# xiph/daala

Hardware: NVIDIA H100
Metric: encoder Mpixels/s on 4K YUV420 intra (higher is better)
Workload: dtype int32

## Files before the change

daala_b200/csrc/frame_transform.cu:

```cuda
#include <cuda.h>
#include <cuda_runtime.h>
#include <cudaTypedefs.h>
#include <stdint.h>
#include <stdio.h>
#include <string.h>

#include "gen/dct_lifting.cuh"
#include "lapped_filter.cuh"
#include "frame_transform.h"
#include "haar.cuh"

namespace daala_b200 {

#ifndef DAALA_XFORM_THREADS
#define DAALA_XFORM_THREADS 64
#endif
constexpr int kThreads = DAALA_XFORM_THREADS;
constexpr int kPostThreads = 128;
constexpr int kCtasPerSm = 512 / kThreads;
constexpr int kGridCap = 132 * 8;
constexpr int kMaxB = 64;
constexpr int kHalo = 2;
constexpr int kMaxT = kMaxB + 2 * kHalo;
constexpr int kMaxPitch = kMaxT + 1;

struct TmaMaps {
  CUtensorMap plane[3];
};

template <int XDEC> struct RawTile {
  static constexpr int B = kMaxB >> XDEC;
  static constexpr int rows = B + 2 * kHalo;
  static constexpr int lead = 16;
  static constexpr int width = ((lead + B + kHalo + 15) / 16) * 16;
  static constexpr int skip = lead - kHalo;
  static constexpr int bytes = rows * width;
};

__device__ __forceinline__ uint32_t smem_u32(const void* p) { return (uint32_t)__cvta_generic_to_shared(p); }

__device__ __forceinline__ void mbar_init(uint64_t* bar, int count) {
  asm volatile("mbarrier.init.shared::cta.b64 [%0], %1;" ::"r"(smem_u32(bar)), "r"(count));
  asm volatile("fence.mbarrier_init.release.cluster;" ::: "memory");
}

__device__ __forceinline__ void mbar_expect_tx(uint64_t* bar, uint32_t bytes) {
  asm volatile("mbarrier.arrive.expect_tx.shared::cta.b64 _, [%0], %1;" ::"r"(smem_u32(bar)), "r"(bytes) : "memory");
}

__device__ __forceinline__ void mbar_wait(uint64_t* bar, uint32_t phase) {
  uint32_t ok = 0;
  while (!ok) {
    asm volatile(
        "{ .reg .pred p; mbarrier.try_wait.parity.shared::cta.b64 p, [%1], %2; selp.u32 %0, 1, 0, p; }"
        : "=r"(ok) : "r"(smem_u32(bar)), "r"(phase) : "memory");
  }
}

__device__ __forceinline__ void tma_load_3d(void* dst, const CUtensorMap* map, int x, int y, int z, uint64_t* bar) {
  asm volatile(
      "cp.async.bulk.tensor.3d.shared::cluster.global.mbarrier::complete_tx::bytes [%0], [%1, {%2, %3, %4}], [%5];"
      ::"r"(smem_u32(dst)), "l"(map), "r"(x), "r"(y), "r"(z), "r"(smem_u32(bar)) : "memory");
}

template <int B_, int P_>
struct SbCtxT {
  static constexpr int B = B_;
  static constexpr int P = P_;
  static constexpr int ushift = (B_ == 64) ? 3 : 2;
  static constexpr int logB = (B_ == 64) ? 6 : 5;
  int x0, y0;
};

struct SbLists {
  unsigned short blk[256 + 64 + 16 + 4 + 1];
  unsigned short node[64 + 16 + 4 + 1];
  int nblk[5];
  int nnode[4];
  unsigned char wcnt[8][9];
};
__device__ __forceinline__ constexpr int blk_base(int c) { return c == 0 ? 0 : c == 1 ? 256 : c == 2 ? 320 : c == 3 ? 336 : 340; }
__device__ __forceinline__ constexpr int node_base(int l) { return (int)((0x54504000u >> (8 * l)) & 0xffu); }
constexpr unsigned short kGateH = 0x4000;
constexpr unsigned short kGateV = 0x8000;

template <int XDEC>
__device__ __forceinline__ void build_lists(SbLists& L, const unsigned char* bsize, int bstride, int sbx,
                                            int sby, int x0, int y0, int pic_w, int pic_h) {
  static_assert(kThreads >= 64, "one thread per 8x8-luma unit");
  constexpr int B = kMaxB >> XDEC;
  constexpr int USZ = 8 >> XDEC;
  const int t = threadIdx.x, lane = t & 31, w = t >> 5;
  const int bx = t & 7, by = (t >> 3) & 7;
  unsigned flags = 0;
  unsigned rank[9];
  if (t < 64) {
    const int obs = bsize[(sby * 8 + by) * bstride + sbx * 8 + bx];
    const int c = (obs > XDEC ? obs : XDEC) - XDEC;
    const unsigned lt = (1u << lane) - 1u;
    const int xy = bx | by;
#pragma unroll
    for (int cat = 0; cat < 9; cat++) {
      bool f;
      if (cat < 5) {
        const int a = XDEC ? (1 << cat) : (cat ? (1 << (cat - 1)) : 1);
        f = c == cat && !(xy & (a - 1));
      } else {
        const int l = cat - 5, S = 8 << l;
        const int a = XDEC ? (2 << l) : (1 << l);
        f = S <= B && !(xy & (a - 1)) && c < 1 + l;
      }
      const unsigned b = __ballot_sync(0xffffffffu, f);
      flags |= (unsigned)f << cat;
      rank[cat] = __popc(b & lt);
      if (lane == 0) L.wcnt[w][cat] = (unsigned char)__popc(b);
    }
  }
  __syncthreads();
  if (t < 64) {
    const unsigned short pos = (unsigned short)(((by * USZ) << 8) | (bx * USZ));
#pragma unroll
    for (int cat = 0; cat < 9; cat++) {
      const int n0 = L.wcnt[0][cat], n1 = L.wcnt[1][cat];
      const int at = (w ? n0 : 0) + (int)rank[cat];
      constexpr bool kQuad = XDEC == 0;
      if (t == 0) {
        if (cat < 5) L.nblk[cat] = (cat == 0 && kQuad) ? 4 * (n0 + n1) : n0 + n1;
        else L.nnode[cat - 5] = n0 + n1;
      }
      if (flags & (1u << cat)) {
        if (cat == 0 && kQuad) {
          L.blk[4 * at + 0] = pos;
          L.blk[4 * at + 1] = (unsigned short)(pos + 4);
          L.blk[4 * at + 2] = (unsigned short)(pos + (4 << 8));
          L.blk[4 * at + 3] = (unsigned short)(pos + (4 << 8) + 4);
        } else if (cat < 5) {
          L.blk[blk_base(cat) + at] = pos;
        } else {
          const int S = 8 << (cat - 5);
          unsigned short v = pos;
          if (x0 + bx * USZ + S <= pic_w) v |= kGateH;
          if (y0 + by * USZ + S <= pic_h) v |= kGateV;
          L.node[node_base(cat - 5) + at] = v;
        }
      }
    }
  }
  __syncthreads();
}

template <int C, bool kFwd, int P>
__device__ __forceinline__ void transform_pass(int* tile, const SbLists& L, bool along_columns) {
  constexpr int LN = C + 2;
  constexpr int N = 1 << LN;
  const int items = L.nblk[C] << LN;
  for (int item = threadIdx.x; item < items; item += kThreads) {
    const int pos = L.blk[blk_base(C) + (item >> LN)];
    const int k = item & (N - 1);
    const int px = (pos & 255) + (along_columns ? k : 0);
// ... 83 lines not shown
  int* sp = tile + row0 * P + col;
  int32_t* gp = g + (size_t)row0 * gstride + col;
#pragma unroll 8
  for (int r = row0; r < B; r += kRowsPerIter) {
    if (kToGlobal) {
      *reinterpret_cast<int4*>(gp) = make_int4(sp[0], sp[1], sp[2], sp[3]);
    } else {
      const int4 v = *reinterpret_cast<const int4*>(gp);
      sp[0] = v.x;
      sp[1] = v.y;
      sp[2] = v.z;
      sp[3] = v.w;
    }
    sp += kRowsPerIter * P;
    gp += (size_t)kRowsPerIter * gstride;
  }
}
__device__ __forceinline__ bool rows_aligned16(const void* p, long long stride_elems) {
  return ((reinterpret_cast<uintptr_t>(p) | (uintptr_t)(stride_elems * 4)) & 15u) == 0;
}

struct FrameMasks {
  const uint8_t* haar;
  const uint8_t* skip;
};

template <int XDEC, bool kTma>
__device__ __forceinline__ void forward_sb_body(const FrameXformParams& prm, const PlaneXform& pl,
                                                int* tile_s, SbLists& lists, const CUtensorMap* map,
                                                unsigned char* raw, uint64_t* bar, const FrameMasks& fm) {
  constexpr int B = kMaxB >> XDEC;
  constexpr int T = B + 2 * kHalo;
  constexpr int P = kMaxPitch;
  using Sb = SbCtxT<B, P>;
  const int sbx = blockIdx.x % prm.nhsb, sby = prm.sb_row0 + blockIdx.x / prm.nhsb;
  const int fr = blockIdx.z;
  if (fm.skip && fm.skip[fr]) return;
  const bool haar_dc = fm.haar ? fm.haar[fr] != 0 : prm.haar_dc != 0;
  Sb s;
  s.x0 = sbx * B;
  s.y0 = sby * B;
  const int pw = prm.nhsb * B, ph = prm.nvsb * B;
  if (kTma) {
    constexpr int RW = RawTile<XDEC>::width;
    if (threadIdx.x == 0) {
      mbar_init(bar, 1);
      mbar_expect_tx(bar, RawTile<XDEC>::bytes);
      tma_load_3d(raw, map, s.x0 - RawTile<XDEC>::lead, s.y0 - kHalo, fr, bar);
    }
    build_lists<XDEC>(lists, prm.bsize + fr * prm.bsize_frame_pitch, prm.bstride, sbx, sby, s.x0, s.y0,
                      prm.pic_w, prm.pic_h);
    mbar_wait(bar, 0);
    constexpr int kSkip = RawTile<XDEC>::skip;
    constexpr int kW0 = kSkip / 4;
    constexpr int kWords = (kSkip + T + 3) / 4 - kW0;
    for (int i = threadIdx.x; i < T * kWords; i += kThreads) {
      const int r = i / kWords, m = i - r * kWords;
      const unsigned w = *reinterpret_cast<const unsigned*>(raw + r * RW + 4 * (kW0 + m));
      const int c0 = 4 * (kW0 + m) - kSkip;
      int* t = tile_s + r * P + c0;
#pragma unroll
      for (int j = 0; j < 4; j++) {
        const int c = c0 + j;
        if (c >= 0 && c < T) t[j] = ((int)((w >> (8 * j)) & 255u) - 128) * 16;
      }
    }
  } else {
    build_lists<XDEC>(lists, prm.bsize + fr * prm.bsize_frame_pitch, prm.bstride, sbx, sby, s.x0, s.y0,
                      prm.pic_w, prm.pic_h);
    const uint8_t* src = pl.pixels + fr * pl.pixel_frame_pitch;
    for (int i = threadIdx.x; i < T * T; i += kThreads) {
      int r = i / T, c = i - r * T;
      int gx = s.x0 + c - kHalo, gy = s.y0 + r - kHalo;
      int v = 0;
      if (gx >= 0 && gx < pw && gy >= 0 && gy < ph) v = ((int)src[(size_t)gy * pl.pixel_stride + gx] - 128) * 16;
      tile_s[r * P + c] = v;
    }
  }
  __syncthreads();
  {
    const bool top = sby > 0, bottom = sby + 1 < prm.nvsb;
    for (int i = threadIdx.x; i < 2 * T; i += kThreads) {
      int e = i >= T, c = i - e * T;
      if (e == 0 ? top : bottom) lap4_inplace<false>(tile_s + (e ? B : 0) * P + c, P);
    }
    __syncthreads();
    const bool left = sbx > 0, right = sbx + 1 < prm.nhsb;
    for (int i = threadIdx.x; i < 2 * B; i += kThreads) {
      int r = i % B + kHalo, e = i / B;
      if (e == 0 ? left : right) lap4_inplace<false>(tile_s + r * P + (e ? B : 0), 1);
    }
    __syncthreads();
  }
  int* tile = tile_s + kHalo * P + kHalo;
#pragma unroll 1
  for (int l = Sb::logB - 3; l >= 0; l--) {
    if (lists.nnode[l] == 0) continue;
    split_filter_level<false, P>(tile, lists, l, true);
    __syncthreads();
    split_filter_level<false, P>(tile, lists, l, false);
    __syncthreads();
  }
#ifdef DAALA_DEBUG_LISTS
  if (threadIdx.x == 0 && XDEC == 1 && sbx == 1 && sby == 1 && blockIdx.y == 1) {
    printf("chroma lists: nblk %d %d %d %d %d nnode %d %d %d %d\n", lists.nblk[0], lists.nblk[1], lists.nblk[2],
           lists.nblk[3], lists.nblk[4], lists.nnode[0], lists.nnode[1], lists.nnode[2], lists.nnode[3]);
    for (int c = 0; c < 4; c++) for (int i = 0; i < lists.nblk[c]; i++) printf("blk c%d (%d,%d)\n", c, lists.blk[blk_base(c) + i] & 255, lists.blk[blk_base(c) + i] >> 8);
    for (int l = 0; l < 3; l++) for (int i = 0; i < lists.nnode[l]; i++) printf("node l%d (%d,%d) gates %x\n", l, lists.node[node_base(l) + i] & 255, (lists.node[node_base(l) + i] >> 8) & 63, lists.node[node_base(l) + i] >> 14);
  }
#endif
  transform_all_leaves<true, P>(tile, lists);
  if (haar_dc) {
#pragma unroll 1
    for (int l = 0; l <= Sb::logB - 3; l++) {
      if (lists.nnode[l] == 0) continue;
      haar_dc_level<false, P>(tile, lists, l);
      __syncthreads();
    }
  }
  int32_t* dst = pl.coeffs + fr * pl.coeff_frame_pitch + (size_t)s.y0 * pl.coeff_stride + s.x0;
  if (rows_aligned16(dst, pl.coeff_stride)) {
    tile_copy4<B, P, true>(tile, dst, pl.coeff_stride);
    return;
  }
  for (int i = threadIdx.x; i < B * B; i += kThreads) {
    int r = i / B, c = i % B;
    dst[(size_t)r * pl.coeff_stride + c] = tile[r * P + c];
  }
}

__global__ void __launch_bounds__(kThreads, kCtasPerSm)
k_forward_sb(const __grid_constant__ FrameXformParams prm, const __grid_constant__ FrameMasks fm) {
  __shared__ int tile_s[kMaxT * kMaxPitch];
  __shared__ SbLists lists;
  const PlaneXform& pl = prm.plane[blockIdx.y];
  if (pl.xdec == 0) forward_sb_body<0, false>(prm, pl, tile_s, lists, nullptr, nullptr, nullptr, fm);
  else forward_sb_body<1, false>(prm, pl, tile_s, lists, nullptr, nullptr, nullptr, fm);
}

__global__ void __launch_bounds__(kThreads, kCtasPerSm)
k_forward_sb_tma(const __grid_constant__ FrameXformParams prm, const __grid_constant__ CUtensorMap map0,
                 const __grid_constant__ CUtensorMap map1, const __grid_constant__ CUtensorMap map2,
                 const __grid_constant__ FrameMasks fm) {
  __shared__ int tile_s[kMaxT * kMaxPitch];
  __shared__ __align__(128) unsigned char raw[RawTile<0>::bytes];
  __shared__ __align__(8) uint64_t bar;
  __shared__ SbLists lists;
  const PlaneXform& pl = prm.plane[blockIdx.y];
  const CUtensorMap* map = blockIdx.y == 0 ? &map0 : (blockIdx.y == 1 ? &map1 : &map2);
  if (pl.xdec == 0) forward_sb_body<0, true>(prm, pl, tile_s, lists, map, raw, &bar, fm);
  else forward_sb_body<1, true>(prm, pl, tile_s, lists, map, raw, &bar, fm);
}

template <int XDEC>
__device__ __forceinline__ void inverse_sb_body(const FrameXformParams& prm, const PlaneXform& pl,
                                                int* tile, SbLists& lists) {
  constexpr int B = kMaxB >> XDEC;
  constexpr int P = kMaxPitch;
  using Sb = SbCtxT<B, P>;
  const int sbx = blockIdx.x % prm.nhsb, sby = prm.sb_row0 + blockIdx.x / prm.nhsb;
  const int fr = blockIdx.z;
  Sb s;
  s.x0 = sbx * B;
  s.y0 = sby * B;
  const int32_t* srcp = pl.coeffs + fr * pl.coeff_frame_pitch + (size_t)s.y0 * pl.coeff_stride + s.x0;
  if (rows_aligned16(srcp, pl.coeff_stride)) {
    tile_copy4<B, P, false>(tile, const_cast<int32_t*>(srcp), pl.coeff_stride);
  } else {
    for (int i = threadIdx.x; i < B * B; i += kThreads) {
      int r = i / B, c = i % B;
      tile[r * P + c] = srcp[(size_t)r * pl.coeff_stride + c];
    }
  }
  build_lists<XDEC>(lists, prm.bsize + fr * prm.bsize_frame_pitch, prm.bstride, sbx, sby, s.x0, s.y0,
                    prm.pic_w, prm.pic_h);
  if (prm.haar_dc) {
#pragma unroll 1
    for (int l = Sb::logB - 3; l >= 0; l--) {
      if (lists.nnode[l] == 0) continue;
      haar_dc_level<true, P>(tile, lists, l);
      __syncthreads();
    }
  }
  transform_all_leaves<false, P>(tile, lists);
#pragma unroll 1
  for (int l = 0; l <= Sb::logB - 3; l++) {
    if (lists.nnode[l] == 0) continue;
    split_filter_level<true, P>(tile, lists, l, false);
    __syncthreads();
    split_filter_level<true, P>(tile, lists, l, true);
    __syncthreads();
  }
  int32_t* dst = pl.lapped + fr * pl.lapped_frame_pitch + (size_t)s.y0 * pl.lapped_stride + s.x0;
  if (rows_aligned16(dst, pl.lapped_stride)) {
    tile_copy4<B, P, true>(tile, dst, pl.lapped_stride);
    return;
  }
  for (int i = threadIdx.x; i < B * B; i += kThreads) {
    int r = i / B, c = i % B;
    dst[(size_t)r * pl.lapped_stride + c] = tile[r * P + c];
  }
}

__global__ void __launch_bounds__(kThreads, kCtasPerSm)
k_inverse_sb(const __grid_constant__ FrameXformParams prm) {
  __shared__ int tile_s[kMaxB * kMaxPitch];
  __shared__ SbLists lists;
  const PlaneXform& pl = prm.plane[blockIdx.y];
  if (pl.xdec == 0) inverse_sb_body<0>(prm, pl, tile_s, lists);
  else inverse_sb_body<1>(prm, pl, tile_s, lists);
}

template <int XDEC>
__device__ __forceinline__ void sb_postfilter_store_body(const FrameXformParams& prm,
                                                         const PlaneXform& pl, int* tile_s) {
  constexpr int B = kMaxB >> XDEC;
  constexpr int T = B + 2 * kHalo;
  constexpr int P = T + 1;
  const int sbx = blockIdx.x % prm.nhsb, sby = prm.sb_row0 + blockIdx.x / prm.nhsb;
  const int fr = blockIdx.z;
  const int32_t* lap = pl.lapped + fr * pl.lapped_frame_pitch;
  const int x0 = sbx * B, y0 = sby * B;
  const int pw = prm.nhsb * B, ph = prm.nvsb * B;
  const int32_t* core = lap + (size_t)y0 * pl.lapped_stride + x0;
  if (rows_aligned16(core, pl.lapped_stride)) {
    tile_copy4<B, P, false, kPostThreads>(tile_s + kHalo * P + kHalo, const_cast<int32_t*>(core), pl.lapped_stride);
    for (int i = threadIdx.x; i < 4 * T + 4 * B; i += kPostThreads) {
      int r, c;
      if (i < 4 * T) {
        const int k = i / T;
        r = k < 2 ? k : B + k;
        c = i - k * T;
      } else {
        const int j = i - 4 * T, k = j / B;
        c = k < 2 ? k : B + k;
        r = j - k * B + kHalo;
      }
      const int gx = x0 + c - kHalo, gy = y0 + r - kHalo;
      int v = 0;
      if (gx >= 0 && gx < pw && gy >= 0 && gy < ph) v = lap[(size_t)gy * pl.lapped_stride + gx];
      tile_s[r * P + c] = v;
    }
  } else {
    for (int i = threadIdx.x; i < T * T; i += kPostThreads) {
      int r = i / T, c = i - r * T;
      int gx = x0 + c - kHalo, gy = y0 + r - kHalo;
      int v = 0;
      if (gx >= 0 && gx < pw && gy >= 0 && gy < ph) v = lap[(size_t)gy * pl.lapped_stride + gx];
      tile_s[r * P + c] = v;
    }
  }
  __syncthreads();
  const bool left = sbx > 0, right = sbx + 1 < prm.nhsb;
  for (int i = threadIdx.x; i < 2 * T; i += kPostThreads) {
    int e = i >= T, r = i - e * T;
    if (e == 0 ? left : right) lap4_inplace<true>(tile_s + r * P + (e ? B : 0), 1);
  }
  __syncthreads();
  const bool top = sby > 0, bottom = sby + 1 < prm.nvsb;
  for (int i = threadIdx.x; i < 2 * B; i += kPostThreads) {
    int c = i % B + kHalo, e = i / B;
    if (e == 0 ? top : bottom) lap4_inplace<true>(tile_s + (e ? B : 0) * P + c, P);
  }
  __syncthreads();
  if (prm.post16[blockIdx.y]) {
    int16_t* d16 = prm.post16[blockIdx.y] + fr * pl.pixel_out_frame_pitch + (size_t)y0 * pl.pixel_out_stride + x0;
    for (int i = threadIdx.x; i < B * B / 2; i += kPostThreads) {
      int r = i / (B / 2), c2 = (i % (B / 2)) * 2;
      const int* p = tile_s + (r + kHalo) * P + c2 + kHalo;
      const unsigned w = ((unsigned)p[0] & 0xffffu) | ((unsigned)p[1] << 16);
      *reinterpret_cast<unsigned*>(d16 + (size_t)r * pl.pixel_out_stride + c2) = w;
    }
    return;
  }
  uint8_t* dst = pl.pixels_out + fr * pl.pixel_out_frame_pitch + (size_t)y0 * pl.pixel_out_stride + x0;
  for (int i = threadIdx.x; i < B * B / 4; i += kPostThreads) {
    int r = i / (B / 4), c4 = (i % (B / 4)) * 4;
    const int* p = tile_s + (r + kHalo) * P + c4 + kHalo;
    unsigned w = 0;
#pragma unroll
    for (int k = 0; k < 4; k++) {
      int v = ((p[k] + 8) >> 4) + 128;
      v = v < 0 ? 0 : (v > 255 ? 255 : v);
      w |= (unsigned)v << (8 * k);
    }
    *reinterpret_cast<unsigned*>(dst + (size_t)r * pl.pixel_out_stride + c4) = w;
  }
}

__global__ void __launch_bounds__(kPostThreads)
k_sb_postfilter_store(const __grid_constant__ FrameXformParams prm) {
  __shared__ int tile_s[kMaxT * kMaxPitch];
  const PlaneXform& pl = prm.plane[blockIdx.y];
  if (pl.xdec == 0) sb_postfilter_store_body<0>(prm, pl, tile_s);
  else sb_postfilter_store_body<1>(prm, pl, tile_s);
}

template <bool kPost>
__global__ void k_plane_sb_edges(int32_t* c, int stride, int nhsb, int nvsb, int sbw, int sbh,
                                 bool vertical_taps) {
  const int w = nhsb * sbw, h = nvsb * sbh;
  const int along = vertical_taps ? w : h;
  const int edges = (vertical_taps ? nvsb : nhsb) - 1;
  const long total = (long)along * edges;
  for (long i = blockIdx.x * (long)blockDim.x + threadIdx.x; i < total;
       i += (long)gridDim.x * blockDim.x) {
    int a = (int)(i % along), e = (int)(i / along) + 1;
    if (vertical_taps) lap4_inplace<kPost>(c + (size_t)(e * sbh - 2) * stride + a, stride);
    else lap4_inplace<kPost>(c + (size_t)a * stride + e * sbw - 2, 1);
  }
}

template <int L>
__global__ void __launch_bounds__(64)
k_block_transform(int32_t* blocks, int mode) {
  constexpr int N = 1 << L;
  constexpr int P = N + 5;
  __shared__ int t[N * P];
  int32_t* blk = blocks + (size_t)blockIdx.x * N * N;
  for (int i = threadIdx.x; i < N * N; i += blockDim.x) t[(i / N) * P + (i % N)] = blk[i];
  __syncthreads();
  const bool fwd = (mode & 1) == 0;
  const int passes = mode < 2 ? 2 : 1;
  for (int pass = 0; pass < passes; pass++) {
    bool cols = mode < 2 ? (fwd ? pass == 0 : pass == 1) : false;
    if (threadIdx.x < N) {
      int* p = cols ? t + threadIdx.x : t + threadIdx.x * P;
      int stride = cols ? P : 1;
      int v[N];
#pragma unroll
      for (int k = 0; k < N; k++) v[k] = p[k * stride];
      if (fwd) Lifting<N>::fwd(v); else Lifting<N>::inv(v);
#pragma unroll
      for (int k = 0; k < N; k++) p[k * stride] = v[k];
    }
    __syncthreads();
  }
  for (int i = threadIdx.x; i < N * N; i += blockDim.x) blk[i] = t[(i / N) * P + (i % N)];
}

__global__ void k_filter4_batch(int32_t* v, long count, int post) {
  for (long i = blockIdx.x * (long)blockDim.x + threadIdx.x; i < count;
       i += (long)gridDim.x * blockDim.x) {
    if (post) lap4_inplace<true>(v + 4 * i, 1); else lap4_inplace<false>(v + 4 * i, 1);
  }
}

template <int N>
__global__ void k_lapfilter_batch(int32_t* v, long count, int post) {
  for (long i = blockIdx.x * (long)blockDim.x + threadIdx.x; i < count; i += (long)gridDim.x * blockDim.x) {
    int t[N];
#pragma unroll
    for (int k = 0; k < N; k++) t[k] = v[i * N + k];
    if (post) LapFilter<N>::post(t); else LapFilter<N>::pre(t);
#pragma unroll
    for (int k = 0; k < N; k++) v[i * N + k] = t[k];
  }
}

__global__ void k_split_filter_batch(int32_t* blocks, int n, int post, int hfilter, int vfilter) {
  int32_t* b = blocks + (size_t)blockIdx.x * n * n;
  for (int phase = 0; phase < 2; phase++) {
    bool vertical_taps = post ? phase == 1 : phase == 0;
    if (vertical_taps ? hfilter : vfilter) {
      for (int i = threadIdx.x; i < n; i += blockDim.x) {
        if (vertical_taps) {
          if (post) lap4_inplace<true>(b + (n / 2 - 2) * n + i, n); else lap4_inplace<false>(b + (n / 2 - 2) * n + i, n);
        } else {
          if (post) lap4_inplace<true>(b + i * n + n / 2 - 2, 1); else lap4_inplace<false>(b + i * n + n / 2 - 2, 1);
        }
      }
    }
    __syncthreads();
  }
}

}

using namespace daala_b200;

template <bool kInverse>
__global__ void __launch_bounds__(256) k_haar_blocks(int32_t* __restrict__ blocks, int ln) {
  __shared__ int t[64 * 64];
  const int n = 1 << ln;
  int32_t* g = blocks + (size_t)blockIdx.x * n * n;
  if (!kInverse) {
    for (int i = threadIdx.x; i < n * n; i += 256) t[i] = g[i];
    __syncthreads();
    haar_forward_levels<256>(t, g, n, ln);
  } else {
    haar_inverse_levels<256>(t, g, n, ln);
    for (int i = threadIdx.x; i < n * n; i += 256) g[i] = t[i];
  }
}

extern "C" {

static bool encode_input_maps(const FrameXformParams* prm, int nplanes, TmaMaps* maps) {
  static PFN_cuTensorMapEncodeTiled_v12000 encode = nullptr;
  static bool tried = false;
  if (!tried) {
    tried = true;
    void* fn = nullptr;
    cudaDriverEntryPointQueryResult q;
    if (cudaGetDriverEntryPoint("cuTensorMapEncodeTiled", &fn, cudaEnableDefault, &q) == cudaSuccess &&
        q == cudaDriverEntryPointSuccess)
      encode = (PFN_cuTensorMapEncodeTiled_v12000)fn;
  }
  if (!encode) return false;
  memset(maps, 0, sizeof(*maps));
  for (int p = 0; p < nplanes; p++) {
    const PlaneXform& pl = prm->plane[p];
    const int B = kMaxB >> pl.xdec;
    const cuuint64_t w = (cuuint64_t)prm->nhsb * B, h = (cuuint64_t)prm->nvsb * B;
    const cuuint64_t fpitch = prm->nframes > 1 ? (cuuint64_t)pl.pixel_frame_pitch : w * h;
    if (((uintptr_t)pl.pixels & 15) || (pl.pixel_stride & 15) || (fpitch & 15) || pl.pixel_stride <= 0) return false;
    cuuint64_t dims[3] = {w, h, (cuuint64_t)prm->nframes};
    cuuint64_t strides[2] = {(cuuint64_t)pl.pixel_stride, fpitch};
    cuuint32_t box[3] = {(cuuint32_t)(pl.xdec ? RawTile<1>::width : RawTile<0>::width),
                         (cuuint32_t)(B + 2 * kHalo), 1};
    cuuint32_t estr[3] = {1, 1, 1};
    CUresult r = encode(&maps->plane[p], CU_TENSOR_MAP_DATA_TYPE_UINT8, 3, (void*)pl.pixels, dims, strides, box,
                        estr, CU_TENSOR_MAP_INTERLEAVE_NONE, CU_TENSOR_MAP_SWIZZLE_NONE,
                        CU_TENSOR_MAP_L2_PROMOTION_L2_128B, CU_TENSOR_MAP_FLOAT_OOB_FILL_NONE);
    if (r != CUDA_SUCCESS) return false;
  }
  return true;
}

int daala_b200_launch_forward_masked(const FrameXformParams* prm, int nplanes, const uint8_t* haar_frames,
                                     const uint8_t* skip_frames, cudaStream_t stream) {
  dim3 grid(prm->nhsb * prm->sb_rows, nplanes, prm->nframes);
  const FrameMasks fm = {haar_frames, skip_frames};
  TmaMaps maps;
  if (encode_input_maps(prm, nplanes, &maps))
    k_forward_sb_tma<<<grid, kThreads, 0, stream>>>(*prm, maps.plane[0], maps.plane[1], maps.plane[2], fm);
  else k_forward_sb<<<grid, kThreads, 0, stream>>>(*prm, fm);
  return (int)cudaGetLastError();
}

int daala_b200_launch_forward(const FrameXformParams* prm, int nplanes, cudaStream_t stream) {
  return daala_b200_launch_forward_masked(prm, nplanes, nullptr, nullptr, stream);
}

int daala_b200_launch_forward_no_tma(const FrameXformParams* prm, int nplanes, cudaStream_t stream) {
  dim3 grid(prm->nhsb * prm->sb_rows, nplanes, prm->nframes);
  k_forward_sb<<<grid, kThreads, 0, stream>>>(*prm, FrameMasks{nullptr, nullptr});
  return (int)cudaGetLastError();
}

int daala_b200_launch_inverse(const FrameXformParams* prm, int nplanes, cudaStream_t stream) {
  dim3 grid(prm->nhsb * prm->sb_rows, nplanes, prm->nframes);
  k_inverse_sb<<<grid, kThreads, 0, stream>>>(*prm);
  k_sb_postfilter_store<<<grid, kPostThreads, 0, stream>>>(*prm);
  return (int)cudaGetLastError();
}

static FrameXformParams plane_range(const FrameXformParams* prm, int plane0) {
  FrameXformParams q = *prm;
  for (int p = 0; p + plane0 < 3; p++) {
    q.plane[p] = prm->plane[plane0 + p];
    q.post16[p] = prm->post16[plane0 + p];
  }
  return q;
}

int daala_b200_launch_inverse_lapped_only(const FrameXformParams* prm, int plane0, int nplanes, cudaStream_t stream) {
  if (plane0 < 0 || nplanes < 1 || plane0 + nplanes > 3) return (int)cudaErrorInvalidValue;
  dim3 grid(prm->nhsb * prm->sb_rows, nplanes, prm->nframes);
  k_inverse_sb<<<grid, kThreads, 0, stream>>>(plane_range(prm, plane0));
  return (int)cudaGetLastError();
}

int daala_b200_launch_sb_postfilter_store(const FrameXformParams* prm, int plane0, int nplanes, cudaStream_t stream) {
  if (plane0 < 0 || nplanes < 1 || plane0 + nplanes > 3) return (int)cudaErrorInvalidValue;
  dim3 grid(prm->nhsb * prm->sb_rows, nplanes, prm->nframes);
  k_sb_postfilter_store<<<grid, kPostThreads, 0, stream>>>(plane_range(prm, plane0));
  return (int)cudaGetLastError();
}

int daala_b200_launch_plane_sb_filter(int32_t* c, int stride, int nhsb, int nvsb, int xdec, int ydec,
                                      int post, cudaStream_t stream) {
  const int sbw = 64 >> xdec, sbh = 64 >> ydec;
  for (int phase = 0; phase < 2; phase++) {
    bool vertical_taps = post ? phase == 1 : phase == 0;
    long total = vertical_taps ? (long)nhsb * sbw * (nvsb - 1) : (long)nvsb * sbh * (nhsb - 1);
    if (total <= 0) continue;
    int blocks = (int)((total + 255) / 256);
    if (blocks > kGridCap) blocks = kGridCap;
    if (post) k_plane_sb_edges<true><<<blocks, 256, 0, stream>>>(c, stride, nhsb, nvsb, sbw, sbh, vertical_taps);
    else k_plane_sb_edges<false><<<blocks, 256, 0, stream>>>(c, stride, nhsb, nvsb, sbw, sbh, vertical_taps);
  }
  return (int)cudaGetLastError();
}

int daala_b200_launch_block_transform(int32_t* blocks, int count, int ln, int mode, cudaStream_t stream) {
  if (count <= 0) return 0;
  switch (ln) {
    case 2: k_block_transform<2><<<count, 64, 0, stream>>>(blocks, mode); break;
    case 3: k_block_transform<3><<<count, 64, 0, stream>>>(blocks, mode); break;
    case 4: k_block_transform<4><<<count, 64, 0, stream>>>(blocks, mode); break;
    case 5: k_block_transform<5><<<count, 64, 0, stream>>>(blocks, mode); break;
    case 6: k_block_transform<6><<<count, 64, 0, stream>>>(blocks, mode); break;
    default: return (int)cudaErrorInvalidValue;
  }
  return (int)cudaGetLastError();
}

int daala_b200_launch_haar_blocks(int32_t* blocks, int count, int ln, int inverse, cudaStream_t stream) {
  if (count <= 0) return 0;
  if (ln < 1 || ln > 6) return (int)cudaErrorInvalidValue;
  if (inverse) k_haar_blocks<true><<<count, 256, 0, stream>>>(blocks, ln);
  else k_haar_blocks<false><<<count, 256, 0, stream>>>(blocks, ln);
  return (int)cudaGetLastError();
}

int daala_b200_launch_filter4(int32_t* v, long count, int post, cudaStream_t stream) {
  if (count <= 0) return 0;
  int blocks = (int)((count + 255) / 256);
  if (blocks > kGridCap) blocks = kGridCap;
  k_filter4_batch<<<blocks, 256, 0, stream>>>(v, count, post);
  return (int)cudaGetLastError();
}

int daala_b200_launch_lapfilter(int32_t* v, long count, int n, int post, cudaStream_t stream) {
  if (count <= 0) return 0;
  int blocks = (int)((count + 127) / 128);
  if (blocks > kGridCap) blocks = kGridCap;
  if (n == 4) k_filter4_batch<<<blocks, 128, 0, stream>>>(v, count, post);
  else if (n == 8) k_lapfilter_batch<8><<<blocks, 128, 0, stream>>>(v, count, post);
  else if (n == 16) k_lapfilter_batch<16><<<blocks, 128, 0, stream>>>(v, count, post);
  else if (n == 32) k_lapfilter_batch<32><<<blocks, 128, 0, stream>>>(v, count, post);
  else return (int)cudaErrorInvalidValue;
  return (int)cudaGetLastError();
}

int daala_b200_launch_split_filter(int32_t* blocks, int count, int n, int post, int hfilter, int vfilter,
                                   cudaStream_t stream) {
  if (count <= 0) return 0;
  k_split_filter_batch<<<count, 64, 0, stream>>>(blocks, n, post, hfilter, vfilter);
  return (int)cudaGetLastError();
}

}
```

daala_b200/csrc/frame_transform.h:

```cpp
#pragma once
#include "daala_b200.h"

typedef daala_b200_plane PlaneXform;
typedef daala_b200_frame FrameXformParams;
```

daala_b200/csrc/kf_engine.cu:

```cuda
#include <cuda_runtime.h>
#include <math.h>
#include <stdint.h>
#include <stdio.h>
#include <stdlib.h>
#include <string.h>

#include <algorithm>
#include <cmath>
#include <new>
#include <vector>

#include "daala_b200.h"
#include "dering_search.h"
#include "late_skip.h"
#include "lossless.h"
#include "haar_dc.h"
#include "mc_batch.h"
#include "gen/coding_order.inc"
#include "pvq_math.cuh"
#include "pvq_warp.cuh"
#include "pvq_common.cuh"

namespace daala_b200 {
namespace kf {

using namespace daala_b200::pvq;

enum Cnt {
  kNLuma = 0, kNChroma, kLumaCoefs, kChromaCoefs,
  kNItemsL = 4,
  kNItemsC = 7,
  kTotalHi = 14,
  kNHeads = 15,
  kNHeads0 = 16,
  kError = 17,
  kDepsDone = 18,
  kMcBadRef = 19,
  kMcBeyond = 20,
  kHeadLoL = 32,
  kHeadHi = 96,
  kTailHi = 128,
  kDoneHi = 160,
  kHeadCh = 192,
  kWaiters = 224,
  kTraceN = 240,
  kCntWords = 256
};

constexpr int kTile = 1024;
constexpr int kHeadBins = 12288;

struct Lists {
  const uint8_t* bsize;
  int bstride;
  long long bsize_pitch;
  int F, UW, UH;
  int u_row0, u_rows;
  int ntiles;
  int4* tile_sum;
  int32_t* unit_lbase;
  int32_t* unit_loff;
  daala_b200_pvq_block* luma;
  daala_b200_pvq_block* chroma;
  int32_t* dep_top;
  int32_t* dep_left;
  int32_t* succ_bottom;
  int32_t* succ_right;
  uint32_t* items_l[3];
  uint32_t* items_c[3];
  uint32_t* heads;
  uint32_t* heads0;
  uint32_t* heads_raw;
  int32_t* head_bin;
  int32_t* head_hist;
  int32_t* head_cursor;
  int32_t* cnt;
  int max_luma, max_chroma;
  const uint8_t* ftype;
  int32_t* kcnt;
  uint32_t* kitems_l[3];
};

__device__ __forceinline__ int4 add4(int4 a, int4 b) { return make_int4(a.x + b.x, a.y + b.y, a.z + b.z, a.w + b.w); }

__device__ __forceinline__ int4 unit_counts(int b, int ux, int uy) {
  if (b == 0) return make_int4(4, 64, 1, 16);
  const int span = 1 << (b - 1);
  if ((ux & (span - 1)) | (uy & (span - 1))) return make_int4(0, 0, 0, 0);
  const int lc = b == 1 ? 64 : b == 2 ? 256 : 512;
  const int cc = b == 1 ? 16 : b == 2 ? 64 : b == 3 ? 256 : 512;
  return make_int4(1, lc, 1, cc);
}

__device__ __forceinline__ bool unit_of(const Lists& L, long long i, int* f, int* uy, int* ux, int* b) {
  const long long per = (long long)L.u_rows * L.UW;
  if (i >= per * L.F) return false;
  *f = (int)(i / per);
  const int r = (int)(i - (long long)*f * per);
  *uy = L.u_row0 + r / L.UW;
  *ux = r % L.UW;
  *b = L.bsize[*f * L.bsize_pitch + (long long)*uy * L.bstride + *ux];
  return true;
}

__global__ void __launch_bounds__(kTile) k_unit_tile_sums(const __grid_constant__ Lists L) {
  __shared__ int4 part[32];
  const long long i = (long long)blockIdx.x * kTile + threadIdx.x;
  int f, uy, ux, b;
  int4 v = make_int4(0, 0, 0, 0);
  if (unit_of(L, i, &f, &uy, &ux, &b)) v = unit_counts(b, ux, uy);
#pragma unroll
  for (int o = 16; o > 0; o >>= 1) {
    v.x += __shfl_xor_sync(0xffffffffu, v.x, o);
    v.y += __shfl_xor_sync(0xffffffffu, v.y, o);
    v.z += __shfl_xor_sync(0xffffffffu, v.z, o);
    v.w += __shfl_xor_sync(0xffffffffu, v.w, o);
  }
  if ((threadIdx.x & 31) == 0) part[threadIdx.x >> 5] = v;
  __syncthreads();
  if (threadIdx.x == 0) {
    int4 s = make_int4(0, 0, 0, 0);
    for (int w = 0; w < kTile / 32; w++) s = add4(s, part[w]);
    L.tile_sum[blockIdx.x] = s;
  }
}

__global__ void __launch_bounds__(1024) k_tile_scan(const __grid_constant__ Lists L) {
  __shared__ int4 part[1024];
  __shared__ int4 carry;
  const int t = threadIdx.x;
  if (t == 0) carry = make_int4(0, 0, 0, 0);
  __syncthreads();
  for (int base = 0; base < L.ntiles; base += 1024) {
    const int i = base + t;
    const int4 v = i < L.ntiles ? L.tile_sum[i] : make_int4(0, 0, 0, 0);
    part[t] = v;
    __syncthreads();
    for (int o = 1; o < 1024; o <<= 1) {
      const int4 a = t >= o ? part[t - o] : make_int4(0, 0, 0, 0);
      __syncthreads();
      part[t] = add4(part[t], a);
      __syncthreads();
    }
    const int4 incl = part[t], c = carry;
    if (i < L.ntiles) L.tile_sum[i] = make_int4(c.x + incl.x - v.x, c.y + incl.y - v.y, c.z + incl.z - v.z, c.w + incl.w - v.w);
    __syncthreads();
    if (t == 1023) carry = add4(c, incl);
    __syncthreads();
  }
  if (t == 0) {
    const int4 tot = carry;
    L.cnt[kNLuma] = tot.x;
    L.cnt[kLumaCoefs] = tot.y;
    L.cnt[kNChroma] = 2 * tot.z;
    L.cnt[kChromaCoefs] = 2 * tot.w;
    for (int c = 0; c < 3; c++) {
      L.cnt[kNItemsL + c] = 0;
      L.cnt[kNItemsC + c] = 0;
    }
    L.cnt[kTotalHi] = 0;
    L.cnt[kNHeads] = 0;
    L.cnt[kNHeads0] = 0;
    L.cnt[kDepsDone] = 0;
    if (L.kcnt != L.cnt) {
      L.kcnt[kNLuma] = 0;
      for (int c = 0; c < 3; c++) L.kcnt[kNItemsL + c] = 0;
      L.kcnt[kTotalHi] = 0;
      L.kcnt[kNHeads] = 0;
      L.kcnt[kNHeads0] = 0;
      L.kcnt[kDepsDone] = 0;
    }
    L.cnt[kError] = tot.x > L.max_luma || 2 * tot.z > L.max_chroma ? 1 : 0;
  }
}

__device__ __forceinline__ void put_block(daala_b200_pvq_block* dst, int coef_off, int x0, int y0, int bs, int pli,
                                          int xdec, int frame) {
  int32_t* w = reinterpret_cast<int32_t*>(dst);
  w[0] = coef_off;
  w[1] = (x0 & 0xffff) | (y0 << 16);
  w[2] = bs | (pli << 8) | (xdec << 16) | (frame << 24);
}

__global__ void __launch_bounds__(kTile) k_unit_emit(const __grid_constant__ Lists L) {
  __shared__ int4 wsum[32];
  const long long i = (long long)blockIdx.x * kTile + threadIdx.x;
  const int lane = threadIdx.x & 31, warp = threadIdx.x >> 5;
  int f = 0, uy = 0, ux = 0, b = 0;
  const bool valid = unit_of(L, i, &f, &uy, &ux, &b);
  const int4 v = valid ? unit_counts(b, ux, uy) : make_int4(0, 0, 0, 0);
  int4 s = v;
#pragma unroll
  for (int o = 1; o < 32; o <<= 1) {
    int4 a;
    a.x = __shfl_up_sync(0xffffffffu, s.x, o);
    a.y = __shfl_up_sync(0xffffffffu, s.y, o);
    a.z = __shfl_up_sync(0xffffffffu, s.z, o);
    a.w = __shfl_up_sync(0xffffffffu, s.w, o);
    if (lane >= o) s = add4(s, a);
  }
  if (lane == 31) wsum[warp] = s;
  __syncthreads();
  int4 pre = L.tile_sum[blockIdx.x];
  for (int w = 0; w < warp; w++) pre = add4(pre, wsum[w]);
  pre = make_int4(pre.x + s.x - v.x, pre.y + s.y - v.y, pre.z + s.z - v.z, pre.w + s.w - v.w);
  if (!valid) return;
  L.unit_lbase[((long long)f * L.UH + uy) * L.UW + ux] = pre.x;
  if (v.x == 0) return;
  if (pre.x + v.x > L.max_luma || 2 * (pre.z + v.z) > L.max_chroma) return;
  if (L.unit_loff) L.unit_loff[((long long)f * L.UH + uy) * L.UW + ux] = pre.y;
  if (b == 0) {
    for (int q = 0; q < 4; q++)
      put_block(L.luma + pre.x + q, pre.y + 16 * q, ux * 8 + (q & 1) * 4, uy * 8 + (q >> 1) * 4, 0, 0, 0, f);
  } else {
    put_block(L.luma + pre.x, pre.y, ux * 8, uy * 8, b, 0, 0, f);
  }
  const int cbs = (b > 1 ? b : 1) - 1;
  const int xd = 1 | (b == 0 ? 0x80 : 0);
  put_block(L.chroma + 2 * pre.z, 2 * pre.w, ux * 4, uy * 4, cbs, 1, xd, f);
  put_block(L.chroma + 2 * pre.z + 1, 2 * pre.w + v.w, ux * 4, uy * 4, cbs, 2, xd, f);
}

__device__ __forceinline__ int band_class(int band) { return band < 3 ? 0 : band < 6 ? 1 : 2; }

__device__ __forceinline__ int append(uint32_t* list, int32_t* counter, bool pred, uint32_t v) {
  const unsigned m = __ballot_sync(__activemask(), pred);
  if (!pred) return -1;
  const int lane = threadIdx.x & 31, leader = __ffs(m) - 1;
  int base = 0;
  if (lane == leader) base = atomicAdd(counter, __popc(m));
  base = __shfl_sync(m, base, leader);
  const int pos = base + __popc(m & ((1u << lane) - 1u));
  list[pos] = v;
  return pos;
}

__device__ __forceinline__ int count_key(int32_t* ctr, int key) {
  const unsigned same = __match_any_sync(__activemask(), key);
  const int lane = threadIdx.x & 31, leader = __ffs(same) - 1;
  int base = 0;
  if (lane == leader) base = atomicAdd(&ctr[key], __popc(same));
  return __shfl_sync(same, base, leader) + __popc(same & ((1u << lane) - 1u));
}

constexpr int kChainCost0 = 7, kChainCost1 = 9, kChainCost2 = 18;
__device__ __forceinline__ int weight_bin(int len, int band) {
  const int c = band_class(band);
  const int w = len * (c == 0 ? kChainCost0 : c == 1 ? kChainCost1 : kChainCost2);
  return kHeadBins - 1 - min(w, kHeadBins - 1);
}

__device__ int chain_length(const Lists& L, const uint8_t* map, int x0, int y0, int bs, bool down) {
  const int nn = 4 << bs, y_end = (L.u_row0 + L.u_rows) * 8, x_end = L.UW * 8;
  int len = 1;
  for (int x = x0 + (down ? 0 : nn), y = y0 + (down ? nn : 0); x < x_end && y < y_end;
       x += down ? 0 : nn, y += down ? nn : 0, len++) {
    if (map[(long long)(y >> 3) * L.bstride + (x >> 3)] != bs) break;
    const int py = down ? y - 1 : y, px = down ? x : x - 1;
    if (map[(long long)(py >> 3) * L.bstride + (px >> 3)] != bs) break;
  }
  return len;
}

template <int kThreads>
__device__ __forceinline__ void scan_bins(int32_t* hist, int32_t* cursor) {
  __shared__ int part[kThreads];
  constexpr int kPer = kHeadBins / kThreads;
  const int t = threadIdx.x;
  int v[kPer], sum = 0;
#pragma unroll
  for (int i = 0; i < kPer; i++) {
    v[i] = __ldcg(hist + t * kPer + i);
    sum += v[i];
  }
  part[t] = sum;
  __syncthreads();
  for (int o = 1; o < kThreads; o <<= 1) {
    const int add = t >= o ? part[t - o] : 0;
    __syncthreads();
    part[t] += add;
    __syncthreads();
  }
  int run = part[t] - sum;
#pragma unroll
  for (int i = 0; i < kPer; i++) {
    hist[t * kPer + i] = run;
    cursor[t * kPer + i] = run;
    run += v[i];
  }
}

__global__ void __launch_bounds__(256) k_luma_deps(const __grid_constant__ Lists L) {
  const int n = min(L.cnt[kNLuma], L.max_luma);
  const int nth = gridDim.x * blockDim.x;
  for (int base = blockIdx.x * blockDim.x; base < n; base += nth) {
    const int blk = base + threadIdx.x;
    const bool in = blk < n && (!L.ftype || L.ftype[L.luma[blk].frame]);
    if (L.ftype) {
      const int nk = __popc(__ballot_sync(0xffffffffu, in));
      if ((threadIdx.x & 31) == 0 && nk) atomicAdd(&L.kcnt[kNLuma], nk);
    }
    int bs = 0, top = -1, left = -1;
    if (in) {
      const daala_b200_pvq_block b = L.luma[blk];
      const int x0 = b.x0, y0 = b.y0, f = b.frame;
      bs = b.bs;
      const int nn = 4 << bs;
      const uint8_t* map = L.bsize + f * L.bsize_pitch;
      if (y0 - nn >= L.u_row0 * 8 && map[(long long)((y0 - 1) >> 3) * L.bstride + (x0 >> 3)] == bs) {
        const int ty = y0 - nn;
        top = L.unit_lbase[((long long)f * L.UH + (ty >> 3)) * L.UW + (x0 >> 3)] +
              (bs == 0 ? ((ty >> 2) & 1) * 2 + ((x0 >> 2) & 1) : 0);
      }
      if (x0 > 0 && map[(long long)(y0 >> 3) * L.bstride + ((x0 - 1) >> 3)] == bs) {
        const int lx = x0 - nn;
        left = L.unit_lbase[((long long)f * L.UH + (y0 >> 3)) * L.UW + (lx >> 3)] +
               (bs == 0 ? ((y0 >> 2) & 1) * 2 + ((lx >> 2) & 1) : 0);
      }
      L.dep_top[blk] = top;
      L.dep_left[blk] = left;
      if (top >= 0) L.succ_bottom[top] = blk;
      if (left >= 0) L.succ_right[left] = blk;
    }
    const int nb = in ? num_bands(bs) : 0;
    int len_down = 0, len_across = 0;
    if (nb > 1) {
      const daala_b200_pvq_block b = L.luma[blk];
      const uint8_t* map = L.bsize + b.frame * L.bsize_pitch;
      if (top < 0) len_down = chain_length(L, map, b.x0, b.y0, bs, true);
      if (left < 0) len_across = chain_length(L, map, b.x0, b.y0, bs, false);
    }
    int chain = 0;
    for (int band = 0; band < 9; band++) {
      const bool has = band < nb;
      const bool is_free = band == 3 || band == 6;
      const int r = band % 3;
      const bool waits = band == 0 ? (top >= 0 || left >= 0) : r == 1 ? top >= 0 : left >= 0;
      const uint32_t item = ((uint32_t)blk << 4) | band;
      if (band == 3 || band == 6) {
        append(L.kitems_l[band_class(band)], &L.kcnt[kNItemsL + band_class(band)], has, item);
      } else if (band == 0) {
        append(L.heads0, &L.kcnt[kNHeads0], has && !waits, item);
      } else {
        const int pos = append(L.heads_raw, &L.kcnt[kNHeads], has && !waits, item);
        if (pos >= 0) {
          const int bin = weight_bin(r == 1 ? len_down : len_across, band);
          L.head_bin[pos] = bin;
          count_key(L.head_hist, bin);
        }
      }
      chain += has && !is_free;
    }
#pragma unroll
    for (int o = 16; o > 0; o >>= 1) chain += __shfl_xor_sync(0xffffffffu, chain, o);
    if ((threadIdx.x & 31) == 0 && chain) atomicAdd(&L.kcnt[kTotalHi], chain);
  }
  __shared__ bool last;
  __threadfence();
  __syncthreads();
  if (threadIdx.x == 0) last = atomicAdd(&L.kcnt[kDepsDone], 1) == (int)gridDim.x - 1;
  __syncthreads();
  if (last) {
    __threadfence();
// ... 157 lines not shown
    } else if (kind == kGatherInter) {
      const int32_t* psrc = prm.pred_plane[b.pli] + b.frame * prm.plane_frame_pitch[b.pli] + (size_t)b.y0 * stride + b.x0;
      int32_t* vref = prm.ref + b.coef_off;
      for (int i = lane; i < len; i += 32) {
        const int at = i == 0 ? 0 : scan_to_raster(i, ln, stride);
        vin[i] = src[at];
        vref[i] = psrc[at];
      }
      if (kMixed && kKind == kGatherChroma && lane == 0) prm.res_flip[blk] = 0;
    } else {
      const int lo = S.cfl_loff[b.frame * (prm.plane_frame_pitch[b.pli] >> 4) + (long long)(b.y0 >> 2) * (stride >> 2) +
                                (b.x0 >> 2)];
      int32_t* vref = prm.ref + b.coef_off;
      const int qoff = prm.qm_stride + ((((1 << (2 * b.bs)) - 1) << 4) / 3);
      int32_t xy = 0;
      for (int i = lane; i < len; i += 32) {
        const int32_t vi = i == 0 ? src[0] : src[scan_to_raster(i, ln, stride)];
        const int32_t vr = cfl_ref<kHdc>(S, b, lo, i);
        vin[i] = vi;
        vref[i] = vr;
        if (i >= 1 && i < 16) {
          const int32_t rq = vr * prm.qm[qoff + i], inq = vi * prm.qm[qoff + i];
          xy += (int32_t)((rq * (int64_t)inq) >> ((kQmShift + 4) << 1));
        }
      }
#pragma unroll
      for (int o = 16; o > 0; o >>= 1) xy += __shfl_xor_sync(0xffffffffu, xy, o);
      const int flip = xy < 0;
      __syncwarp();
      if (flip) {
        const int end = band_start(num_bands(b.bs));
        for (int i = 1 + lane; i < end; i += 32) vref[i] = -vref[i];
      }
      if (lane == 0) prm.res_flip[blk] = flip;
    }
  }
}

constexpr int kPersistThreads = 32;
constexpr int kPersistCtas = 32;
static_assert(kPersistCtas * (kPersistThreads / 32 * kSnapEntries * (int)sizeof(int16_t) + 1024) <= 228 * 1024,
              "k_pvq_persist's shared scratch does not fit kPersistCtas CTAs per SM");
constexpr uint32_t kNoItem = 0xffffffffu;
constexpr uint32_t kExit = 0xfffffffeu;

__device__ __forceinline__ int ld_relaxed(const int32_t* p) {
  int v;
  asm volatile("ld.relaxed.gpu.global.s32 %0, [%1];" : "=r"(v) : "l"(p) : "memory");
  return v;
}

__device__ __forceinline__ void push_chain(const Stage& S, int blk, int band) {
  const int pos = atomicAdd(&S.cnt[kTailHi], 1) - S.cnt[kNHeads0];
  st_release((int*)&S.ring[pos], (int)(((uint32_t)blk << 4) | band));
}

__device__ __forceinline__ uint32_t next_item(const Stage& S, int lane, int* done, bool* waiter) {
  int slot = -1, head = -1, lo = -1, nheads0 = 0, fin = -1;
  if (lane == 0) {
    const int n2 = S.cnt[S.n_items_at + 2], n1 = S.cnt[S.n_items_at + 1], n0 = S.cnt[S.n_items_at];
    const int nlo = n0 + n1 + n2;
    nheads0 = S.cnt[kNHeads0];
    if (*done) {
      const int d = atomicAdd(&S.cnt[kDoneHi], *done) + *done;
      if (d == S.cnt[kNLuma]) {
        __threadfence();
        fin = ld_relaxed(&S.cnt[kTailHi]) - nheads0;
      }
    }
    if (ld_relaxed(&S.cnt[kHeadHi]) < ld_relaxed(&S.cnt[kTailHi])) slot = atomicAdd(&S.cnt[kHeadHi], 1);
    if (slot < 0 && ld_relaxed(&S.cnt[kHeadCh]) < S.cnt[kNHeads]) {
      const int h = atomicAdd(&S.cnt[kHeadCh], 1);
      if (h < S.cnt[kNHeads]) head = h;
    }
    if (slot < 0 && head < 0 && ld_relaxed(&S.cnt[S.head_lo_at]) < nlo) {
      const int l = atomicAdd(&S.cnt[S.head_lo_at], 1);
      if (l < nlo) lo = l;
    }
    if (slot < 0 && head < 0 && lo < 0) {
      if (!*waiter && atomicAdd(&S.cnt[kWaiters], 1) < S.max_waiters) *waiter = true;
      if (*waiter) slot = atomicAdd(&S.cnt[kHeadHi], 1);
    }
  }
  *done = 0;
  fin = __shfl_sync(0xffffffffu, fin, 0);
  if (fin >= 0) {
    const int nw = (gridDim.x * blockDim.x) >> 5;
#pragma unroll 1
    for (int i = lane; i <= nw; i += 32) st_release((int*)&S.ring[fin + i], (int)kExit);
  }
  head = __shfl_sync(0xffffffffu, head, 0);
  if (head >= 0) return S.heads[head];
  slot = __shfl_sync(0xffffffffu, slot, 0);
  lo = __shfl_sync(0xffffffffu, lo, 0);
  if (slot >= 0) {
    nheads0 = __shfl_sync(0xffffffffu, nheads0, 0);
    if (slot < nheads0) return S.heads0[slot];
    uint32_t v;
    while ((v = (uint32_t)ld_acquire((const int*)&S.ring[slot - nheads0])) == kNoItem) __nanosleep(500);
    return v == kExit ? kNoItem : v;
  }
  if (lo >= 0) {
    const int n2 = S.cnt[S.n_items_at + 2], n1 = S.cnt[S.n_items_at + 1];
    return lo < n2 ? S.items[2][lo] : lo < n2 + n1 ? S.items[1][lo - n2] : S.items[0][lo - n2 - n1];
  }
  return kNoItem;
}

__device__ __forceinline__ void intra_band_ref(const Stage& S, int blk, int band, int coef_off, int lane) {
  const daala_b200_pvq_params& prm = S.prm;
  const int start = band_start(band);
  const int bn = band_start(band + 1) - start;
  const int r = band % 3;
  int top = -1, left = -1;
  if (band == 0 || r == 1) top = S.dep_top[blk];
  if (band == 0 || r == 2) left = S.dep_left[blk];
  if (band == 3 || band == 6) top = left = -1;
  const int32_t* ot = top >= 0 ? prm.out + prm.blocks[top].coef_off : nullptr;
  const int32_t* ol = left >= 0 ? prm.out + prm.blocks[left].coef_off : nullptr;
  bool low_from_top = false;
  if (band == 0) {
    double g1 = 0, g2 = 0;
    if (ot) { double a = __ldcg(ot + 2), bb = __ldcg(ot + 5), c = __ldcg(ot + 9); g1 += a * a; g1 += bb * bb; g1 += c * c; }
    if (ol) { double a = __ldcg(ol + 1), bb = __ldcg(ol + 4), c = __ldcg(ol + 7); g2 += a * a; g2 += bb * bb; g2 += c * c; }
    low_from_top = g1 > g2;
  }
  int32_t* vref = prm.ref + coef_off;
  for (int i = start + lane; i < start + bn; i += 32) {
    int r2, c2;
    scan_rc(i, &r2, &c2);
    int32_t p = 0;
    if (r2 == 0 && c2 > 0 && ot && (c2 >= 4 || low_from_top)) p = __ldcg(ot + i);
    if (c2 == 0 && r2 > 0 && ol && (r2 >= 4 || !low_from_top)) p = __ldcg(ol + i);
    vref[i] = p;
  }
}

__device__ __forceinline__ void run_item(const Stage& S, uint32_t item, int lane, int16_t* snap) {
  const daala_b200_pvq_params& prm = S.prm;
  const int blk = (int)(item >> 4), band = (int)(item & 15);
  const daala_b200_pvq_block b = prm.blocks[blk];
  const int bs = b.bs, pli = b.pli;
  const int start = band_start(band);
  const int bn = band_start(band + 1) - start;
  const size_t off = (size_t)b.coef_off + start;
  intra_band_ref(S, blk, band, b.coef_off, lane);
  const int qidx = bs * (bs + 1) + (band + 1) - (band + 1) / 3;
  const int q = S.fq_bq[(b.frame * 3 + pli) * 32 + qidx];
  const int beta = (prm.use_masking && pli == 0 && bs > 0) ? kBeta15 : kBeta1;
  const int qoff = (b.xdec & 1 ? prm.qm_stride : 0) + ((((1 << (2 * bs)) - 1) << 4) / 3) + start;
  int itheta, max_theta, k;
  double skip_term;
  const int gain = quantise_band_warp<0>(lane, snap, S.rsqrt_tbl, prm.out + off, prm.in + off, prm.ref + off, bn, q,
                                         prm.y + off, &itheta, &max_theta, &k, beta, &skip_term, prm.is_keyframe, pli,
                                         prm.qm + qoff, prm.qm_inv + qoff, prm.pvq_norm_lambda);
  if (lane == 0) {
    const size_t r = (size_t)blk * 9 + band;
    prm.res_skip_term[r] = skip_term;
    short4 pk;
    pk.x = (short)gain; pk.y = (short)itheta; pk.z = (short)max_theta; pk.w = (short)k;
    reinterpret_cast<short4*>(S.res_pack)[r] = pk;
  }
}

struct ItemGeom {
  int blk, band, bn, q, beta, pli, qoff, is_keyframe;
  size_t off;
};
__device__ __forceinline__ ItemGeom item_geom(const Stage& S, uint32_t item) {
  const daala_b200_pvq_params& prm = S.prm;
  ItemGeom g;
  g.blk = (int)(item >> 4);
  g.band = (int)(item & 15);
  const daala_b200_pvq_block b = prm.blocks[g.blk];
  const int bs = b.bs;
  g.pli = b.pli;
  const int start = band_start(g.band);
  g.bn = band_start(g.band + 1) - start;
  g.off = (size_t)b.coef_off + start;
  const int qidx = bs * (bs + 1) + (g.band + 1) - (g.band + 1) / 3;
  g.q = S.fq_bq[(b.frame * 3 + g.pli) * 32 + qidx];
  g.beta = (prm.use_masking && g.pli == 0 && bs > 0) ? kBeta15 : kBeta1;
  g.qoff = (b.xdec & 1 ? prm.qm_stride : 0) + ((((1 << (2 * bs)) - 1) << 4) / 3) + start;
  g.is_keyframe = S.ftype ? S.ftype[b.frame] : prm.is_keyframe;
  return g;
}

template <int kPhase, int kMode>
__global__ void __launch_bounds__(128) k_pvq_split(const __grid_constant__ Stage S, int cls, int chunk) {
  const daala_b200_pvq_params& prm = S.prm;
  const int lane = threadIdx.x & 31;
  const int slots = S.sp_slots[cls];
  const int first = chunk * slots;
  const int count = min(S.cnt[S.n_items_at + cls] - first, slots);
  const int vs = cls == 2 ? 128 : 32;
  const int nwarps = (gridDim.x * blockDim.x) >> 5;
  for (int i = (blockIdx.x * blockDim.x + threadIdx.x) >> 5; i < count; i += nwarps) {
    const ItemGeom g = item_geom(S, S.items[cls][first + i]);
    int16_t* vec = S.sp_vec[cls] + (size_t)i * 3 * vs;
    int32_t* lanes = S.sp_lanes[cls] + (size_t)i * kCtxLaneWords * 16;
    int32_t* uni = S.sp_uni[cls] + (size_t)i * kCtxUniWords;
    int16_t* snap = S.sp_snap[cls] + (size_t)i * kMaxEvents * vs;
    const int32_t* r0 = prm.ref + g.off;
    BandCtx B;
    if (kPhase == 0) {
      band_setup<kMode>(lane, B, prm.in + g.off, r0, g.bn, g.q, g.beta, g.is_keyframe, g.pli, prm.qm + g.qoff,
                 prm.pvq_norm_lambda, S.rsqrt_tbl);
      band_ctx_store_setup(lane, B, g.bn, vec, vs, lanes, uni);
    } else if (kPhase == 1) {
      band_ctx_load_search(lane, B, g.bn, vec, vs, lanes);
      band_search<kMode>(lane, B, g.bn, snap, vs, S.rsqrt_tbl);
      band_ctx_store_search(lane, B, lanes);
    } else {
      band_ctx_load_finish(lane, B, g.bn, vec, vs, lanes, uni);
      int itheta, max_theta, k;
      double skip_term;
      const int gain = band_finish<kMode>(lane, B, snap, vs, prm.out + g.off, r0, g.bn, g.q, prm.y + g.off, &itheta, &max_theta, &k,
                                   g.beta, &skip_term, g.is_keyframe, g.pli, prm.qm_inv + g.qoff, prm.pvq_norm_lambda);
      if (lane == 0) {
        const size_t r = (size_t)g.blk * 9 + g.band;
        prm.res_skip_term[r] = skip_term;
        short4 pk;
        pk.x = (short)gain; pk.y = (short)itheta; pk.z = (short)max_theta; pk.w = (short)k;
        reinterpret_cast<short4*>(S.res_pack)[r] = pk;
      }
    }
  }
}

__global__ void __launch_bounds__(kPersistThreads, kPersistCtas) k_pvq_persist(const __grid_constant__ Stage S) {
  __shared__ __align__(16) int16_t snap_all[kPersistThreads / 32][kSnapEntries];
  const int lane = threadIdx.x & 31;
  int16_t* snap = snap_all[threadIdx.x >> 5];
  int done = 0;
  bool waiter = false;
  for (;;) {
    uint32_t item = next_item(S, lane, &done, &waiter);
    if (item == kNoItem) return;
#ifdef DAALA_B200_CHAIN_TRACE
    int kind = (item & 15) == 0 ? 0 : (item & 15) == 3 || (item & 15) == 6 ? 2 : 1;
#endif
    for (;;) {
      const int band = (int)(item & 15);
#ifdef DAALA_B200_CHAIN_TRACE
      const unsigned long long t0 = globaltimer();
#endif
      run_item(S, item, lane, snap);
#ifdef DAALA_B200_CHAIN_TRACE
      trace_item(S, item, kind, t0, lane);
      kind = 3;
#endif
      if (band == 3 || band == 6) break;
      done += band == 0;
      __threadfence();
      __syncwarp();
      uint32_t next = kNoItem;
      if (lane == 0) {
        const int blk = (int)(item >> 4);
        if (band == 0) {
          const int nb[2] = {S.succ_bottom[blk], S.succ_right[blk]};
          for (int i = 0; i < 2; i++) {
            if (nb[i] < 0) continue;
            const int need = (S.dep_top[nb[i]] >= 0) + (S.dep_left[nb[i]] >= 0);
            if (need == 2 && atomicAdd(&S.join0[nb[i]], 1) != 1) continue;
            if (next == kNoItem) {
              next = (uint32_t)nb[i] << 4;
            } else {
              __threadfence();
              push_chain(S, nb[i], 0);
            }
          }
        } else {
          const int nb = band % 3 == 1 ? S.succ_bottom[blk] : S.succ_right[blk];
          if (nb >= 0) next = ((uint32_t)nb << 4) | band;
        }
      }
      next = __shfl_sync(0xffffffffu, next, 0);
      if (next == kNoItem) break;
      __threadfence();
      item = next;
    }
  }
}

__global__ void k_fill_rsqrt(double* tbl) {
  const int i = blockIdx.x * blockDim.x + threadIdx.x;
  if (i < kTableDoubles) pvq_fill_rsqrt_table(tbl, i);
}

__global__ void k_begin_pvq(int32_t* cnt, uint32_t* ring = nullptr, int nwarps = 0) {
  if (ring && cnt[kNLuma] == 0)
    for (int i = threadIdx.x; i <= nwarps; i += blockDim.x) ring[i] = kExit;
  if (threadIdx.x == 0 && blockIdx.x == 0) {
    cnt[kHeadLoL] = 0;
    cnt[kHeadHi] = 0;
    cnt[kTailHi] = cnt[kNHeads0];
    cnt[kDoneHi] = 0;
    cnt[kHeadCh] = 0;
    cnt[kWaiters] = 0;
#ifdef DAALA_B200_CHAIN_TRACE
    cnt[kTraceN] = 0;
#endif
  }
}

template <bool kInter, bool kHdc = false, bool kMixed = false>
__global__ void __launch_bounds__(256) k_finish_scatter(const __grid_constant__ Stage S) {
  const daala_b200_pvq_params& prm = S.prm;
  const int n = min(S.cnt[S.n_blocks_at], S.max_blocks);
  const int lane = threadIdx.x & 31;
  const int nwarps = (gridDim.x * blockDim.x) >> 5;
  for (int blk = (blockIdx.x * blockDim.x + threadIdx.x) >> 5; blk < n; blk += nwarps) {
    const daala_b200_pvq_block b = prm.blocks[blk];
    const bool key = kMixed && S.ftype[b.frame];
    const bool inter = kMixed ? !key : kInter, hdc = kMixed ? key : kHdc;
    const int ln = b.bs + 2, nn = 1 << ln;
    const int len = ln >= 5 ? 512 : 1 << (2 * ln);
    const int stride = prm.plane_stride[b.pli];
    int32_t* dst = prm.coef_plane[b.pli] + b.frame * prm.plane_frame_pitch[b.pli] + (size_t)b.y0 * stride + b.x0;
    const int32_t* src = prm.out + b.coef_off;
    if (lane == 0) {
      const int nb = num_bands(b.bs);
      double sd = 0;
      for (int i = 0; i < nb; i++) sd += prm.res_skip_term[(size_t)blk * 9 + i];
      prm.res_skip_diff[blk] = sd;
      if (hdc) {
        prm.out[b.coef_off] = dst[0] = hdc_grid(S, b.frame, b.pli)[(long long)(b.y0 >> 2) * (stride >> 2) + (b.x0 >> 2)];
        if (kMixed) {
          prm.res_dc[blk] = 0;
          if (S.dc_resid) S.dc_resid[blk] = 0;
        }
      } else if (!inter) {
        prm.out[b.coef_off] = prm.in[b.coef_off];
      } else {
        const int dc_quant = S.fq_bq[(b.frame * 3 + b.pli) * 32 + b.bs * (b.bs + 1)];
        const int32_t r = prm.ref[b.coef_off], diff = prm.in[b.coef_off] - r;
        int qdc = 0;
        if (abs(diff) >= dc_quant * 141 / 256) {
          const int half = ((dc_quant + 1) >> 1) - 1;
          qdc = (diff + (diff < 0 ? -half : half)) / dc_quant;
        }
        prm.out[b.coef_off] = dst[0] = qdc * dc_quant + r;
        prm.res_dc[blk] = qdc;
        if (S.dc_resid) S.dc_resid[blk] = diff;
      }
    }
    if (ln >= 5) {
      const int32_t* mdp = inter ? prm.pred_plane[b.pli] + b.frame * prm.plane_frame_pitch[b.pli] + (size_t)b.y0 * stride + b.x0
                                 : nullptr;
      for (int i = lane; i < nn * nn; i += 32) {
        const size_t at = (size_t)(i >> ln) * stride + (i & (nn - 1));
        if (i) dst[at] = inter ? mdp[at] : 0;
      }
      __syncwarp();
    }
    for (int i = lane + 1; i < len; i += 32) dst[scan_to_raster(i, ln, stride)] = src[i];
    const int32_t* y = prm.y + b.coef_off;
    for (int i = lane; i < len; i += 32) prm.y16[b.coef_off + i] = i ? (int16_t)y[i] : (int16_t)0;
  }
}

__global__ void k_dering_thresholds(const uint8_t* __restrict__ level, int32_t* __restrict__ thr_luma,
                                    int32_t* __restrict__ thr_chroma, int n, const uint8_t* __restrict__ coded,
                                    uint8_t* __restrict__ applied, const int32_t* __restrict__ frame_tbl, int nsb) {
  const int i = blockIdx.x * blockDim.x + threadIdx.x;
  if (i >= n) return;
  int g = level[i] < 6 ? level[i] : 5;
  if (coded) {
    if (!coded[i]) g = 0;
    applied[i] = (uint8_t)g;
  }
  const int32_t* t = frame_tbl + (size_t)(i / nsb) * 12;
  thr_luma[i] = t[g];
  thr_chroma[i] = t[6 + g];
}

struct Fin {
  const daala_b200_pvq_block* blocks[2];
  const uint8_t* skip[2];
  const int32_t* dc[2];
  const int32_t* cnt;
  int max_blocks[2];
  const int32_t* d[3];
  const int32_t* md[3];
  int32_t* out[3];
  long long plane_pitch[3];
  int plane_stride[3];
  uint8_t* bskip[3];
  long long skip_pitch[3];
  int skip_stride;
  uint8_t* coded;
  int nhsb, nvsb;
  const int32_t* fq_bq;
  const uint8_t* ftype;
};

__device__ __forceinline__ bool fin_block(const Fin& P, int i, int* list, int* blk) {
  const int nl = min(P.cnt[kNLuma], P.max_blocks[0]), nc = min(P.cnt[kNChroma], P.max_blocks[1]);
  if (i >= nl + nc) return false;
  *list = i >= nl;
  *blk = i >= nl ? i - nl : i;
  return true;
}

__global__ void __launch_bounds__(256) k_fin_patch(const __grid_constant__ Fin P) {
  const int lane = threadIdx.x & 31;
  const int nwarps = (gridDim.x * blockDim.x) >> 5;
  int list, blk;
  for (int i = (blockIdx.x * blockDim.x + threadIdx.x) >> 5; fin_block(P, i, &list, &blk); i += nwarps) {
    const daala_b200_pvq_block b = P.blocks[list][blk];
    const int ln = b.bs + 2, nn = 1 << ln;
    const int stride = P.plane_stride[b.pli];
    const size_t o = b.frame * P.plane_pitch[b.pli] + (size_t)b.y0 * stride + b.x0;
    const int32_t* src = (P.skip[list][blk] ? P.md[b.pli] : P.d[b.pli]) + o;
    const int32_t* mdp = P.md[b.pli] + o;
    int32_t* dst = P.out[b.pli] + o;
    if (P.ftype && P.ftype[b.frame]) {
      for (int k = lane; k < nn * nn; k += 32) {
        const size_t at = (size_t)(k >> ln) * stride + (k & (nn - 1));
        dst[at] = P.d[b.pli][o + at];
      }
      continue;
    }
    const int dc_quant = P.fq_bq[(b.frame * 3 + b.pli) * 32 + b.bs * (b.bs + 1)];
    const int32_t dc0 = mdp[0] + P.dc[list][blk] * dc_quant;
    for (int k = lane; k < nn * nn; k += 32) {
      const size_t at = (size_t)(k >> ln) * stride + (k & (nn - 1));
      dst[at] = k ? src[at] : dc0;
    }
  }
}

__global__ void __launch_bounds__(256) k_fin_skip_map(const __grid_constant__ Fin P) {
  const int lane = threadIdx.x & 31;
  const int nwarps = (gridDim.x * blockDim.x) >> 5;
  int list, blk;
  for (int i = (blockIdx.x * blockDim.x + threadIdx.x) >> 5; fin_block(P, i, &list, &blk); i += nwarps) {
    const daala_b200_pvq_block b = P.blocks[list][blk];
    const uint8_t s = P.skip[list][blk] && P.dc[list][blk] == 0 && !(P.ftype && P.ftype[b.frame]);
    const int nu = 1 << b.bs;
    uint8_t* m = P.bskip[b.pli] + b.frame * P.skip_pitch[b.pli] + (size_t)(b.y0 >> 2) * P.skip_stride + (b.x0 >> 2);
    for (int k = lane; k < nu * nu; k += 32) m[(size_t)(k >> b.bs) * P.skip_stride + (k & (nu - 1))] = s;
    if (lane == 0 && b.pli == 0 && !s) P.coded[((size_t)b.frame * P.nvsb + (b.y0 >> 6)) * P.nhsb + (b.x0 >> 6)] = 1;
  }
}

struct PoolStore {
  const uint8_t* src[3];
  uint8_t* pool[3];
  long long plane_bytes[3];
  const int32_t* slot;
};

__global__ void __launch_bounds__(256) k_fin_pool_store(const __grid_constant__ PoolStore S) {
  const int f = blockIdx.y / 3, p = blockIdx.y - 3 * f;
  const int slot = S.slot[f];
  if (slot < 0) return;
  const long long n = S.plane_bytes[p] >> 4;
  const uint4* __restrict__ src = reinterpret_cast<const uint4*>(S.src[p] + f * S.plane_bytes[p]);
  uint4* __restrict__ dst = reinterpret_cast<uint4*>(S.pool[p] + slot * S.plane_bytes[p]);
  for (long long i = (long long)blockIdx.x * blockDim.x + threadIdx.x; i < n; i += (long long)gridDim.x * blockDim.x)
    dst[i] = src[i];
}

struct Sym {
  const uint8_t* bsize;
  int bstride;
  long long bsize_pitch;
  int F, nhsb, sb_rows, u_row0;
  int nsb;
  uint32_t* unit_rank;
  uint32_t* sb_cnt;
  int32_t* sb_base;
  uint32_t* order;
  longlong2* off;
  longlong2* tile;
  long long* tot;
  int ntiles, cap_blocks;
  long long cap_bands, cap_bytes;
  daala_b200_kf_sym_frame* index;
  daala_b200_kf_sym_block* blocks;
  short4* bands;
  uint8_t* pulses;
  const daala_b200_pvq_block* list[2];
  const short4* res[2];
  const int32_t* y[2];
  const double* skip_diff[2];
  const int32_t* flip;
  const int32_t* cnt;
  int max_luma, max_chroma;
  daala_b200_kf_sym_dc* dc;
  const int32_t* qdc[2];
  const int32_t* dc_resid[2];
  daala_b200_kf_late_skip* late_skip;
  const daala_b200_kf_late_skip* ls_block[2];
  daala_b200_kf_sym_hdc* hdc;
  const int32_t* hdc_index[3];
  int gw[3], gh[3];
};

__device__ __forceinline__ int sym_band_bytes(int band, short4 r) {
  if (r.w <= 0) return 0;
  const int n = band_start(band + 1) - band_start(band) - (r.y != -1);
  return r.w > 127 ? 2 * n : n;
}

__global__ void __launch_bounds__(256) k_sym_rank(const __grid_constant__ Sym S) {
  const int lane = threadIdx.x & 31;
  const int sb = (blockIdx.x * blockDim.x + threadIdx.x) >> 5;
  if (sb >= S.F * S.nsb) return;
  const int f = sb / S.nsb, r = sb % S.nsb;
  const int sby = r / S.nhsb, sbx = r % S.nhsb;
  const int uw = S.nhsb * 8;
  uint32_t v[2];
  long long at[2];
  for (int h = 0; h < 2; h++) {
    const int m = 2 * lane + h;
    const int dx = (m & 1) | ((m >> 1) & 2) | ((m >> 2) & 4);
    const int dy = ((m >> 1) & 1) | ((m >> 2) & 2) | ((m >> 3) & 4);
    const int ux = sbx * 8 + dx, uy = S.u_row0 + sby * 8 + dy;
    const int b = S.bsize[f * S.bsize_pitch + (long long)uy * S.bstride + ux];
    const int4 c = unit_counts(b, ux, uy);
    v[h] = (uint32_t)c.x | ((uint32_t)c.z << 16);
    at[h] = ((long long)f * S.sb_rows * 8 + (uy - S.u_row0)) * uw + ux;
  }
  const uint32_t s = v[0] + v[1];
  uint32_t inc = s;
#pragma unroll
  for (int o = 1; o < 32; o <<= 1) {
    const uint32_t a = __shfl_up_sync(0xffffffffu, inc, o);
    if (lane >= o) inc += a;
  }
  S.unit_rank[at[0]] = inc - s;
  S.unit_rank[at[1]] = inc - s + v[0];
  if (lane == 31) S.sb_cnt[sb] = inc;
}

__global__ void __launch_bounds__(1024) k_sym_sb_scan(const __grid_constant__ Sym S) {
  __shared__ int part[1024];
  __shared__ int carry;
  const int t = threadIdx.x;
  const int n = S.F * S.nsb;
  if (t == 0) carry = 0;
  __syncthreads();
  for (int base = 0; base < n; base += 1024) {
    const int i = base + t;
    const uint32_t c = i < n ? S.sb_cnt[i] : 0u;
    const int v = (int)(c & 0xffff) + 2 * (int)(c >> 16);
    part[t] = v;
    __syncthreads();
    for (int o = 1; o < 1024; o <<= 1) {
      const int a = t >= o ? part[t - o] : 0;
      __syncthreads();
      part[t] += a;
      __syncthreads();
    }
    const int incl = part[t], c0 = carry;
    if (i < n) S.sb_base[i] = c0 + incl - v;
    __syncthreads();
    if (t == 1023) carry = c0 + incl;
    __syncthreads();
  }
  if (t == 0) S.tot[0] = min(carry, S.cap_blocks);
}

__global__ void __launch_bounds__(256) k_sym_hdc(const __grid_constant__ Sym S) {
  const int lane = threadIdx.x & 31;
  const int item = (blockIdx.x * blockDim.x + threadIdx.x) >> 5;
  if (item >= S.F * S.nsb * 3) return;
  const int sb = item / 3, pli = item - 3 * sb;
  const int f = sb / S.nsb, r = sb % S.nsb;
  const int sby = r / S.nhsb, sbx = r % S.nhsb;
  const int uw = S.nhsb * 8, xdec = pli ? 1 : 0;
  int b[2], ux[2], uy[2];
  for (int h = 0; h < 2; h++) {
    const int m = 2 * lane + h;
    ux[h] = sbx * 8 + ((m & 1) | ((m >> 1) & 2) | ((m >> 2) & 4));
    uy[h] = S.u_row0 + sby * 8 + (((m >> 1) & 1) | ((m >> 2) & 2) | ((m >> 3) & 4));
    b[h] = max((int)S.bsize[f * S.bsize_pitch + (long long)uy[h] * S.bstride + ux[h]], xdec);
  }
  const int b2 = __shfl_sync(0xffffffffu, b[0], lane & ~1);
  const int b3 = __shfl_sync(0xffffffffu, b[0], lane & ~7);
  const int b4 = __shfl_sync(0xffffffffu, b[0], 0);
  const bool s4 = b4 < 4, s3 = s4 && b3 < 3, s2 = s3 && b2 < 2;
  int mask[2];
  for (int h = 0; h < 2; h++) {
    const int m = 2 * lane + h;
    mask[h] = (m == 0 && s4 ? 1 : 0) | ((m & 15) == 0 && s3 ? 2 : 0) | ((m & 3) == 0 && s2 ? 4 : 0) |
              (s2 && b[h] < 1 ? 8 : 0);
  }
  const int n = __popc(mask[0]) + __popc(mask[1]);
  int inc = n;
#pragma unroll
  for (int o = 1; o < 32; o <<= 1) {
    const int a = __shfl_up_sync(0xffffffffu, inc, o);
    if (lane >= o) inc += a;
  }
  const uint32_t sc = S.sb_cnt[sb];
  const int plane_off = pli ? (int)(sc & 0xffff) + (pli - 1) * (int)(sc >> 16) : 0;
  const long long base = (long long)S.sb_base[sb] + plane_off;
  const long long first = S.sb_base[f * S.nsb];
  const int32_t* grid = S.hdc_index[pli] + (long long)f * S.gw[pli] * S.gh[pli];
  const int gsh = pli ? 0 : 1;
  if (lane == 0 && base < S.cap_blocks) {
    daala_b200_kf_sym_hdc d;
    d.value = grid[(long long)(uy[0] << gsh) * S.gw[pli] + (ux[0] << gsh)];
    d.block = (uint32_t)(base - first);
    d.pli = (uint8_t)pli;
    d.bsi = 4;
    d.child = 0;
    d.reserved = 0;
    S.hdc[base] = d;
  }
  int k = inc - n;
  for (int h = 0; h < 2; h++) {
    if (!mask[h]) continue;
    const uint32_t rk = S.unit_rank[((long long)f * S.sb_rows * 8 + (uy[h] - S.u_row0)) * uw + ux[h]];
    const uint32_t block = (uint32_t)(base - first) + (pli ? rk >> 16 : rk & 0xffff);
    const int gx = ux[h] << gsh, gy = uy[h] << gsh;
    for (int bsi = 4; bsi >= 1; bsi--) {
      if (!(mask[h] & (1 << (4 - bsi)))) continue;
      const int half = 1 << (bsi - 1 - xdec);
      for (int c = 1; c <= 3; c++) {
        const long long slot = base + 1 + 3 * k + (c - 1);
        if (slot >= S.cap_blocks) break;
        daala_b200_kf_sym_hdc d;
        d.value = grid[(long long)(gy + (c >> 1) * half) * S.gw[pli] + gx + (c & 1) * half];
        d.block = block;
        d.pli = (uint8_t)pli;
        d.bsi = (uint8_t)(bsi - 1);
        d.child = (uint8_t)c;
        d.reserved = 0;
        S.hdc[slot] = d;
      }
      k++;
    }
  }
}

__global__ void __launch_bounds__(256) k_sym_place(const __grid_constant__ Sym S) {
  const int nl = min(S.cnt[kNLuma], S.max_luma), nc = min(S.cnt[kNChroma], S.max_chroma);
  const int uw = S.nhsb * 8;
  for (int i = blockIdx.x * blockDim.x + threadIdx.x; i < nl + nc; i += gridDim.x * blockDim.x) {
    const int ch = i >= nl;
    const int blk = ch ? i - nl : i;
    const daala_b200_pvq_block b = S.list[ch][blk];
    const int sh = ch ? 2 : 3;
    const int ux = b.x0 >> sh, uy = b.y0 >> sh;
    const int sb = b.frame * S.nsb + ((uy - S.u_row0) >> 3) * S.nhsb + (ux >> 3);
    const uint32_t rk = S.unit_rank[((long long)b.frame * S.sb_rows * 8 + (uy - S.u_row0)) * uw + ux];
    const uint32_t sc = S.sb_cnt[sb];
    int pos = S.sb_base[sb];
    if (!ch) pos += (int)(rk & 0xffff) + (b.bs == 0 ? ((b.y0 >> 2) & 1) * 2 + ((b.x0 >> 2) & 1) : 0);
    else pos += (int)(sc & 0xffff) + (b.pli - 1) * (int)(sc >> 16) + (int)(rk >> 16);
    if (pos >= S.cap_blocks) continue;
    S.order[pos] = (uint32_t)blk | (ch ? 0x80000000u : 0u);
    const short4* r = S.res[ch] + (size_t)blk * 9;
    const int nb = num_bands(b.bs);
    long long bytes = 0;
    for (int j = 0; j < nb; j++) bytes += sym_band_bytes(j, r[j]);
    S.off[pos] = make_longlong2(nb, bytes);
  }
}

__device__ __forceinline__ longlong2 add2(longlong2 a, longlong2 b) { return make_longlong2(a.x + b.x, a.y + b.y); }

__global__ void __launch_bounds__(kTile) k_sym_tile_sums(const __grid_constant__ Sym S) {
  __shared__ longlong2 part[32];
  const long long i = (long long)blockIdx.x * kTile + threadIdx.x;
  longlong2 v = i < S.tot[0] ? S.off[i] : make_longlong2(0, 0);
#pragma unroll
  for (int o = 16; o > 0; o >>= 1) {
    v.x += __shfl_xor_sync(0xffffffffu, v.x, o);
    v.y += __shfl_xor_sync(0xffffffffu, v.y, o);
  }
  if ((threadIdx.x & 31) == 0) part[threadIdx.x >> 5] = v;
  __syncthreads();
  if (threadIdx.x == 0) {
    longlong2 s = make_longlong2(0, 0);
    for (int w = 0; w < kTile / 32; w++) s = add2(s, part[w]);
    S.tile[blockIdx.x] = s;
  }
}

__global__ void __launch_bounds__(1024) k_sym_tile_scan(const __grid_constant__ Sym S) {
  __shared__ longlong2 part[1024];
  __shared__ longlong2 carry;
  const int t = threadIdx.x;
  if (t == 0) carry = make_longlong2(0, 0);
  __syncthreads();
  for (int base = 0; base < S.ntiles; base += 1024) {
    const int i = base + t;
    const longlong2 v = i < S.ntiles ? S.tile[i] : make_longlong2(0, 0);
    part[t] = v;
    __syncthreads();
    for (int o = 1; o < 1024; o <<= 1) {
      const longlong2 a = t >= o ? part[t - o] : make_longlong2(0, 0);
      __syncthreads();
      part[t] = add2(part[t], a);
      __syncthreads();
    }
    const longlong2 incl = part[t], c = carry;
    if (i < S.ntiles) S.tile[i] = make_longlong2(c.x + incl.x - v.x, c.y + incl.y - v.y);
    __syncthreads();
    if (t == 1023) carry = add2(c, incl);
    __syncthreads();
  }
  if (t == 0) {
    S.tot[1] = carry.x;
    S.tot[2] = carry.y;
  }
}

__global__ void __launch_bounds__(kTile) k_sym_offsets(const __grid_constant__ Sym S) {
  __shared__ longlong2 wsum[32];
  const long long i = (long long)blockIdx.x * kTile + threadIdx.x;
  const int lane = threadIdx.x & 31, warp = threadIdx.x >> 5;
  const bool valid = i < S.tot[0];
  const longlong2 v = valid ? S.off[i] : make_longlong2(0, 0);
  longlong2 s = v;
#pragma unroll
  for (int o = 1; o < 32; o <<= 1) {
    const long long ax = __shfl_up_sync(0xffffffffu, s.x, o), ay = __shfl_up_sync(0xffffffffu, s.y, o);
    if (lane >= o) s = make_longlong2(s.x + ax, s.y + ay);
  }
  if (lane == 31) wsum[warp] = s;
  __syncthreads();
  longlong2 pre = S.tile[blockIdx.x];
  for (int w = 0; w < warp; w++) pre = add2(pre, wsum[w]);
  if (valid) S.off[i] = make_longlong2(pre.x + s.x - v.x, pre.y + s.y - v.y);
}

template <bool kInter>
__global__ void __launch_bounds__(256) k_sym_pack(const __grid_constant__ Sym S) {
  const int lane = threadIdx.x & 31;
  const long long n = S.tot[0];
  const int nwarps = (gridDim.x * blockDim.x) >> 5;
  for (long long slot = (blockIdx.x * blockDim.x + threadIdx.x) >> 5; slot < n; slot += nwarps) {
    const uint32_t id = S.order[slot];
    const int ch = id >> 31, blk = (int)(id & 0x7fffffffu);
    const daala_b200_pvq_block b = S.list[ch][blk];
    const long long first = S.sb_base[b.frame * S.nsb];
    const longlong2 o = S.off[slot], o0 = first < n ? S.off[first] : o;
    const short4* r = S.res[ch] + (size_t)blk * 9;
    const int nb = num_bands(b.bs);
    int bytes = 0;
    for (int j = 0; j < nb; j++) bytes += sym_band_bytes(j, r[j]);
    if (o.x + nb > S.cap_bands || o.y + bytes > S.cap_bytes) continue;
    if (lane == 0) {
      daala_b200_kf_sym_block rec;
      rec.skip_diff = S.skip_diff[ch][blk];
      rec.pulse_off = (uint32_t)(o.y - o0.y);
      rec.band_off = (uint32_t)(o.x - o0.x);
      rec.x0 = b.x0;
      rec.y0 = b.y0;
      rec.bs = b.bs;
      rec.pli = b.pli;
      rec.flip = !kInter && ch ? (uint8_t)S.flip[blk] : 0;
      rec.reserved = 0;
      S.blocks[slot] = rec;
      if (kInter) {
        daala_b200_kf_sym_dc d;
        d.qdc = S.qdc[ch][blk];
        d.dc_resid = S.dc_resid[ch][blk];
        S.dc[slot] = d;
        if (S.late_skip) S.late_skip[slot] = S.ls_block[ch][blk];
      }
    }
    if (lane < nb) S.bands[o.x + lane] = r[lane];
    const int32_t* y = S.y[ch] + b.coef_off;
    uint8_t* dst = S.pulses + o.y;
    for (int j = 0; j < nb; j++) {
      const short4 q = r[j];
      const int len = sym_band_bytes(j, q);
      if (!len) continue;
      const int st = band_start(j);
      if (q.w > 127) {
        for (int t = lane; t < len / 2; t += 32) {
          const int v = y[st + t];
          dst[2 * t] = (uint8_t)(v & 0xff);
          dst[2 * t + 1] = (uint8_t)((v >> 8) & 0xff);
        }
      } else {
        for (int t = lane; t < len; t += 32) dst[t] = (uint8_t)(y[st + t] & 0xff);
      }
      dst += len;
    }
  }
}

__global__ void k_sym_index(const __grid_constant__ Sym S) {
  for (int f = threadIdx.x; f < S.F; f += blockDim.x) {
    const long long n = S.tot[0];
    const long long s0 = S.sb_base[f * S.nsb];
    const long long s1 = f + 1 < S.F ? S.sb_base[(f + 1) * S.nsb] : n;
    const longlong2 a = s0 < n ? S.off[s0] : make_longlong2(S.tot[1], S.tot[2]);
    const longlong2 e = s1 < n ? S.off[s1] : make_longlong2(S.tot[1], S.tot[2]);
    daala_b200_kf_sym_frame x;
    x.first_block = s0;
    x.n_blocks = s1 - s0;
    x.first_band = a.x;
    x.n_bands = e.x - a.x;
    x.first_byte = a.y;
    x.n_bytes = e.y - a.y;
    S.index[f] = x;
  }
}

constexpr int kSymSegs = 7;
struct SymCopy {
  const uint8_t* src[kSymSegs];
  uint8_t* dst[kSymSegs];
  long long unit[kSymSegs];
  long long cap[kSymSegs];
  long long index_bytes;
  const long long* tot;
};

__global__ void __launch_bounds__(256) k_sym_copy(const __grid_constant__ SymCopy C) {
  const long long tid = (long long)blockIdx.x * blockDim.x + threadIdx.x;
  const long long nth = (long long)gridDim.x * blockDim.x;
  for (int seg = 0; seg < kSymSegs; seg++) {
    if (!C.dst[seg]) continue;
    const long long want = seg == 0 ? C.index_bytes : C.tot[seg >= 4 ? 0 : seg - 1] * C.unit[seg];
    const long long len = want < C.cap[seg] ? want : C.cap[seg];
    const uint8_t* s = C.src[seg];
    uint8_t* d = C.dst[seg];
    long long done = 0;
    if ((((uintptr_t)s | (uintptr_t)d) & 15) == 0) {
      const long long n16 = len >> 4;
      for (long long i = tid; i < n16; i += nth)
        reinterpret_cast<uint4*>(d)[i] = reinterpret_cast<const uint4*>(s)[i];
      done = n16 << 4;
    }
    for (long long i = done + tid; i < len; i += nth) d[i] = s[i];
  }
}

struct Unstream {
  const uint32_t* order;
  const long long* tot;
  const uint8_t* skip;
  const int32_t* dc;
  uint8_t* fin_skip[2];
  int32_t* fin_dc[2];
  const int32_t* form;
};

__global__ void __launch_bounds__(256) k_fin_unstream(const __grid_constant__ Unstream U) {
  if (!*U.form) return;
  const long long n = U.tot[0];
  for (long long slot = (long long)blockIdx.x * blockDim.x + threadIdx.x; slot < n;
       slot += (long long)gridDim.x * blockDim.x) {
    const uint32_t id = U.order[slot];
    const int ch = id >> 31, blk = (int)(id & 0x7fffffffu);
    U.fin_skip[ch][blk] = U.skip[slot];
    U.fin_dc[ch][blk] = U.dc[slot];
  }
}

}
}

using namespace daala_b200::kf;

extern "C" int daala_b200_launch_forward_masked(const daala_b200_frame* prm, int nplanes, const uint8_t* haar_frames,
                                                const uint8_t* skip_frames, cudaStream_t stream);
extern "C" int daala_b200_launch_inverse_lapped_only(const daala_b200_frame* prm, int plane0, int nplanes,
                                                     cudaStream_t stream);
extern "C" int daala_b200_launch_sb_postfilter_store(const daala_b200_frame* prm, int plane0, int nplanes,
                                                     cudaStream_t stream);

struct Dering {
  daala_b200_frame frame;
  const uint8_t* skip[3];
  long long skip_pitch[3];
  int skip_stride;
  uint8_t* level;
  const uint8_t* coded;
  uint8_t* applied;
  const int32_t* frame_tbl;
  int32_t* thr[2];
  int32_t* dir;
  bool search;
  daala_b200_dering_search_batch sb;
};

enum { kEvLists, kEvForward, kEvLumaBands, kEvLumaScatter, kEvChroma, kEvHaarDc, kEvLumaGather, kEvInterLuma, kNumEvents };

struct daala_b200_kf {
  daala_b200_kf_config cfg;
  int nhsb, nvsb, F;
  int plane_w[3], plane_h[3];
  cudaStream_t stream;
  bool own_stream;
  cudaStream_t side;
  cudaEvent_t ev[kNumEvents];
  cudaGraph_t graph;
  cudaGraphExec_t exec;
  bool captured;
  uint8_t* pixels[3];
  int32_t* coeffs[3];
  int32_t* lapped[3];
  uint8_t* pixels_out[3];
  uint8_t* pred_pixels[3];
  int32_t* pred_coeffs[3];
  uint8_t* bsize;
  int16_t *qm, *qm_inv;
  double* rsqrt_tbl;
  int16_t* sp_vec[3];
  int32_t* sp_lanes[3];
  int32_t* sp_uni[3];
  int16_t* sp_snap[3];
  int sp_slots[3];
  Dering dering;
  Lists lists;
  Stage luma, chroma;
  uint8_t* ftype;
  Stage luma_kf;
  Sym sym;
  daala_b200_frame frame;
  daala_b200_frame frame_fwd;
  daala_b200_frame frame_pred;
  uint8_t* ref_pixels[3];
  int32_t* ref_slot;
  daala_b200_mv_pt* mv_grid;
  int32_t* ref_slot_next;
  int32_t* mv1_grid;
  uint32_t* mc_leaves;
  int32_t* mc_nleaves;
  daala_b200_mc_batch mc;
  uint8_t* fin_skip[2];
  int32_t* fin_dc[2];
  int32_t* dc_resid[2];
  int32_t* fin_coeffs[3];
  uint8_t* fin_pixels[3];
  uint8_t* fin_bskip[3];
  uint8_t *fin_level, *fin_coded;
  Fin fin;
  cudaGraph_t fin_graph;
  cudaGraphExec_t fin_exec;
  bool fin_captured;
  int fin_dc_limit;
  daala_b200_kf_frame_quant* fq;
  int32_t* fq_tbl;
  std::vector<int32_t> fq_tbl_host;
  int32_t* fq_bq;
  std::vector<int32_t> fq_bq_host;
  int32_t* fin_slot_out;
  PoolStore store;
  uint8_t* fin_stream_skip;
  int32_t* fin_stream_dc;
  int32_t* fin_form;
  Unstream unstream;
  int32_t* d_orig[3];
  daala_b200_kf_late_skip* late_skip[2];
  daala_b200_late_skip_batch lsb;
  int16_t* ll_coeffs[3];
  int32_t* ll_blocks;
  int32_t* ll_dc;
  int32_t* ll_slot_out;
  daala_b200_lossless_batch ll;
  int32_t* hdc;
  int32_t* hdc_index[3];
  daala_b200_haar_dc_batch hdcb;
  std::vector<uint8_t> slot_filled;
  bool have_step;
  daala_b200_kf_totals last_tot;
  std::vector<void*> allocs;
  size_t bytes_allocated;
  size_t chain_cap;
  int sms;
  char err[256];
};

#define KF_CHECK(x)                                                                       \
  do {                                                                                    \
    cudaError_t e_ = (x);                                                                 \
    if (e_ != cudaSuccess) {                                                              \
      snprintf(kf->err, sizeof(kf->err), "%s: %s", #x, cudaGetErrorString(e_));           \
      return (int)e_;                                                                     \
    }                                                                                     \
  } while (0)

template <class T>
static cudaError_t dalloc(daala_b200_kf* kf, T** p, size_t n) {
  const size_t bytes = (n ? n : 1) * sizeof(T);
  cudaError_t e = cudaMalloc((void**)p, bytes);
  if (e == cudaSuccess) {
    kf->allocs.push_back(*p);
    kf->bytes_allocated += bytes;
    e = cudaMemset(*p, 0, bytes);
  }
  return e;
}

static int mc_alloc(daala_b200_kf* kf) {
  const int F = kf->F;
  daala_b200_mc_batch& B = kf->mc;
  const size_t nsb = (size_t)kf->nhsb * kf->nvsb;
  for (int p = 0; p < 3; p++) {
    KF_CHECK(dalloc(kf, &kf->ref_pixels[p], (size_t)kf->plane_w[p] * kf->plane_h[p] * kf->cfg.mc_refs));
    B.ref[p] = kf->ref_pixels[p];
    B.pred[p] = kf->pred_pixels[p];
    B.plane_w[p] = kf->plane_w[p];
    B.plane_h[p] = kf->plane_h[p];
  }
  KF_CHECK(dalloc(kf, &kf->ref_slot, (size_t)2 * F));
  KF_CHECK(dalloc(kf, &kf->mv_grid, (size_t)F * (kf->nvsb * 8 + 1) * (kf->nhsb * 8 + 1)));
  KF_CHECK(dalloc(kf, &kf->mc_leaves, (size_t)F * nsb * 64));
  KF_CHECK(dalloc(kf, &kf->mc_nleaves, (size_t)F * nsb));
  B.grid = kf->mv_grid;
  B.ref_slot = kf->ref_slot;
  B.leaves = kf->mc_leaves;
  B.nleaves = kf->mc_nleaves;
  B.F = F;
  B.nhsb = kf->nhsb;
  B.nvsb = kf->nvsb;
  B.nslots = kf->cfg.mc_refs;
  if (kf->cfg.mc_next) {
    KF_CHECK(dalloc(kf, &kf->ref_slot_next, (size_t)F));
    KF_CHECK(dalloc(kf, &kf->mv1_grid, (size_t)F * (kf->nvsb * 8 + 1) * (kf->nhsb * 8 + 1) * 2));
    B.ref_slot_next = kf->ref_slot_next;
    B.mv1 = kf->mv1_grid;
  }
  return 0;
}

static int ll_alloc(daala_b200_kf* kf) {
  const int F = kf->F;
  daala_b200_lossless_batch& B = kf->ll;
  memset(&B, 0, sizeof(B));
  for (int p = 0; p < 3; p++) {
    const size_t n = (size_t)kf->plane_w[p] * kf->plane_h[p] * F;
    KF_CHECK(dalloc(kf, &kf->pixels[p], n));
    KF_CHECK(dalloc(kf, &kf->pixels_out[p], n));
    KF_CHECK(dalloc(kf, &kf->ll_coeffs[p], n));
    if (kf->cfg.inter) KF_CHECK(dalloc(kf, &kf->pred_pixels[p], n));
    B.src[p] = kf->pixels[p];
    B.pred[p] = kf->pred_pixels[p];
    B.coeffs[p] = kf->ll_coeffs[p];
    B.out[p] = kf->pixels_out[p];
    B.plane_w[p] = kf->plane_w[p];
    B.plane_h[p] = kf->plane_h[p];
  }
  const size_t nrec = (size_t)F * kf->nhsb * kf->nvsb * 3;
  KF_CHECK(dalloc(kf, &kf->ll_blocks, nrec * 4));
  KF_CHECK(dalloc(kf, &kf->ll_dc, nrec));
  KF_CHECK(dalloc(kf, &kf->lists.cnt, (size_t)kCntWords));
  kf->mc.bad_ref = kf->lists.cnt + kMcBadRef;
  kf->mc.beyond = kf->lists.cnt + kMcBeyond;
  if (kf->cfg.inter_mc) {
    int rc = mc_alloc(kf);
    if (rc) return rc;
    KF_CHECK(dalloc(kf, &kf->ll_slot_out, (size_t)F));
    for (int p = 0; p < 3; p++) B.pool[p] = kf->ref_pixels[p];
    B.slot_out = kf->ll_slot_out;
  }
  B.blocks = kf->ll_blocks;
  B.dc = kf->ll_dc;
  B.F = F;
  B.nhsb = kf->nhsb;
  B.nvsb = kf->nvsb;
  B.pic_w = kf->cfg.pic_w;
  B.pic_h = kf->cfg.pic_h;
  KF_CHECK(cudaDeviceSynchronize());
  return 0;
}

static const char* fq_derive_host(daala_b200_kf* kf, const daala_b200_kf_frame_quant* rec, bool check, int* dc_limit) {
  if (!rec) return "frame_quant: the records ([nframes]) are required";
  const int F = kf->F;
  for (int f = 0; check && f < F; f++) {
    const daala_b200_kf_frame_quant& r = rec[f];
    if (r.q0 < 1 || r.q0 > DAALA_B200_KF_MAX_Q0) return "a record's q0 is outside [1, 8191]";
    if (r.coded_quantizer < 1 || r.coded_quantizer > 63) return "a record's coded_quantizer is outside [1, 63]";
    if (!std::isfinite(r.dering_lambda) || r.dering_lambda < 0) return "a record's dering_lambda is negative or not finite";
    for (int p = 0; p < 3; p++)
      for (int i = 0; i < 30; i++)
        if (r.pvq_qm_q4[p][i] < 1) return "a record's pvq_qm_q4 entry is 0";
  }
  *dc_limit = daala_b200_kf_frame_quant_derive(rec, F, reinterpret_cast<int32_t(*)[2][6]>(kf->fq_tbl_host.data()));
  for (int f = 0; f < F; f++)
    for (int p = 0; p < 3; p++)
      for (int i = 0; i < 30; i++)
        kf->fq_bq_host[(size_t)(f * 3 + p) * 32 + i] = std::max(1, (rec[f].q0 * rec[f].pvq_qm_q4[p][i]) >> 4);
  return nullptr;
}

static cudaError_t fq_copy(daala_b200_kf* kf, const daala_b200_kf_frame_quant* rec, cudaStream_t s) {
  const int F = kf->F;
  cudaError_t e = cudaMemcpyAsync(kf->fq, rec, sizeof(daala_b200_kf_frame_quant) * F, cudaMemcpyHostToDevice, s);
  if (!e) e = cudaMemcpyAsync(kf->fq_tbl, kf->fq_tbl_host.data(), sizeof(int32_t) * 12 * F, cudaMemcpyHostToDevice, s);
  if (!e) e = cudaMemcpyAsync(kf->fq_bq, kf->fq_bq_host.data(), sizeof(int32_t) * 96 * F, cudaMemcpyHostToDevice, s);
  return e;
}

static int kf_alloc(daala_b200_kf* kf) {
  if (kf->cfg.lossless) return ll_alloc(kf);
  const int F = kf->F;
  const bool inter = kf->cfg.inter != 0;
  const bool mixed = kf->cfg.frame_types != 0;
  if (mixed) KF_CHECK(dalloc(kf, &kf->ftype, (size_t)F));
  const long long luma_px = (long long)kf->plane_w[0] * kf->plane_h[0];
  for (int p = 0; p < 3; p++) {
    const size_t n = (size_t)kf->plane_w[p] * kf->plane_h[p] * F;
    KF_CHECK(dalloc(kf, &kf->pixels[p], n));
    KF_CHECK(dalloc(kf, &kf->coeffs[p], n));
    KF_CHECK(dalloc(kf, &kf->lapped[p], n));
    KF_CHECK(dalloc(kf, &kf->pixels_out[p], n));
    if (inter) {
      KF_CHECK(dalloc(kf, &kf->pred_pixels[p], n));
      KF_CHECK(dalloc(kf, &kf->pred_coeffs[p], n));
    }
  }
  const int UW = kf->nhsb * 8, UH = kf->nvsb * 8;
  KF_CHECK(dalloc(kf, &kf->bsize, (size_t)F * UW * UH));
  if (kf->cfg.inter_mc) {
    const int rc = mc_alloc(kf);
    if (rc) return rc;
    kf->mc.frame_type = kf->ftype;
  }
  KF_CHECK(dalloc(kf, &kf->fq, (size_t)F));
  KF_CHECK(dalloc(kf, &kf->fq_tbl, (size_t)F * 12));
  KF_CHECK(dalloc(kf, &kf->fq_bq, (size_t)F * 96));
  kf->fq_tbl_host.assign((size_t)F * 12, 0);
  kf->fq_bq_host.assign((size_t)F * 96, 1);
  KF_CHECK(dalloc(kf, &kf->qm, (size_t)2 * kf->cfg.qm_stride));
  KF_CHECK(dalloc(kf, &kf->qm_inv, (size_t)2 * kf->cfg.qm_stride));
  KF_CHECK(dalloc(kf, &kf->rsqrt_tbl, (size_t)kTableDoubles));
  KF_CHECK(cudaMemcpy(kf->qm, kf->cfg.qm, sizeof(int16_t) * 2 * kf->cfg.qm_stride, cudaMemcpyHostToDevice));
  KF_CHECK(cudaMemcpy(kf->qm_inv, kf->cfg.qm_inv, sizeof(int16_t) * 2 * kf->cfg.qm_stride, cudaMemcpyHostToDevice));

  Lists& L = kf->lists;
  memset(&L, 0, sizeof(L));
  L.bsize = kf->bsize;
  L.bstride = UW;
  L.bsize_pitch = (long long)UW * UH;
  L.F = F;
  L.UW = UW;
  L.UH = UH;
  L.u_row0 = kf->cfg.sb_row0 * 8;
  L.u_rows = kf->cfg.sb_rows * 8;
  const long long nunits = (long long)F * L.u_rows * UW;
  L.ntiles = (int)((nunits + kTile - 1) / kTile);
  const int div = kf->cfg.max_blocks_div > 0 ? kf->cfg.max_blocks_div : 1;
  L.max_luma = (int)(nunits * 4 / div) + 64;
  L.max_chroma = (int)(nunits * 2 / div) + 64;
  KF_CHECK(dalloc(kf, &L.tile_sum, (size_t)L.ntiles));
  KF_CHECK(dalloc(kf, &L.unit_lbase, (size_t)F * UW * UH));
  if (!inter || mixed) KF_CHECK(dalloc(kf, &L.unit_loff, (size_t)F * UW * UH));
  KF_CHECK(dalloc(kf, &L.luma, (size_t)L.max_luma));
  KF_CHECK(dalloc(kf, &L.chroma, (size_t)L.max_chroma));
  const size_t ndep = inter && !mixed ? 0 : (size_t)L.max_luma;
  const bool chains = ndep != 0;
  KF_CHECK(dalloc(kf, &L.dep_top, ndep));
  KF_CHECK(dalloc(kf, &L.dep_left, ndep));
  KF_CHECK(dalloc(kf, &L.succ_bottom, ndep));
  KF_CHECK(dalloc(kf, &L.succ_right, ndep));
  const size_t luma_shard_px = (size_t)F * L.u_rows * UW * 64;
  kf->chain_cap = luma_shard_px / 16 + 64 + (size_t)kf->sms * 64;
  const size_t cap_l0 = (size_t)L.max_luma * 3 < luma_shard_px / 16 ? (size_t)L.max_luma * 3 : luma_shard_px / 16;
  const size_t cap_l[3] = {inter ? cap_l0 + 64 : 64, luma_shard_px / 64 + 64, luma_shard_px / 256 + 64};
  const size_t cap_c[3] = {(size_t)L.max_chroma * 3 / 2 + 64, luma_shard_px / 4 * 2 * 3 / 64 + 64,
                           luma_shard_px / 4 * 2 * 3 / 256 + 64};
  for (int c = 0; c < 3; c++) {
    KF_CHECK(dalloc(kf, &L.items_l[c], cap_l[c]));
    KF_CHECK(dalloc(kf, &L.items_c[c], cap_c[c]));
    L.kitems_l[c] = L.items_l[c];
  }
  const size_t cap_k[3] = {64, cap_l[1], cap_l[2]};
  for (int c = 0; mixed && c < 3; c++) KF_CHECK(dalloc(kf, &L.kitems_l[c], cap_k[c]));
  {
    const int slots[3] = {1 << 19, 1 << 19, 3 << 15};
    for (int c = 0; c < 3; c++) {
      const int vs = c == 2 ? 128 : 32;
      kf->sp_slots[c] = slots[c];
      KF_CHECK(dalloc(kf, &kf->sp_vec[c], (size_t)slots[c] * 3 * vs));
      KF_CHECK(dalloc(kf, &kf->sp_lanes[c], (size_t)slots[c] * kCtxLaneWords * 16));
      KF_CHECK(dalloc(kf, &kf->sp_uni[c], (size_t)slots[c] * kCtxUniWords));
      KF_CHECK(dalloc(kf, &kf->sp_snap[c], (size_t)slots[c] * kMaxEvents * vs));
    }
  }
  {
    const int want = kf->cfg.persist_ctas_per_sm > 0 ? kf->cfg.persist_ctas_per_sm : kPersistCtas;
    int per_sm = 0;
    KF_CHECK(cudaFuncSetAttribute(k_pvq_persist, cudaFuncAttributePreferredSharedMemoryCarveout,
                                  cudaSharedmemCarveoutMaxShared));
    KF_CHECK(cudaOccupancyMaxActiveBlocksPerMultiprocessor(&per_sm, k_pvq_persist, kPersistThreads, 0));
    if (per_sm < want) {
      snprintf(kf->err, sizeof(kf->err), "k_pvq_persist: %d CTAs per SM resident, %d wanted", per_sm, want);
      return (int)cudaErrorLaunchOutOfResources;
    }
  }
  KF_CHECK(dalloc(kf, &L.heads, chains ? kf->chain_cap : 0));
  KF_CHECK(dalloc(kf, &L.heads_raw, chains ? kf->chain_cap : 0));
  KF_CHECK(dalloc(kf, &L.head_bin, chains ? kf->chain_cap : 0));
  KF_CHECK(dalloc(kf, &L.head_hist, chains ? (size_t)kHeadBins : 0));
  KF_CHECK(dalloc(kf, &L.head_cursor, chains ? (size_t)kHeadBins : 0));
  KF_CHECK(dalloc(kf, &L.heads0, ndep));
  KF_CHECK(dalloc(kf, &L.cnt, (size_t)kCntWords));
  L.kcnt = L.cnt;
  if (mixed) KF_CHECK(dalloc(kf, &L.kcnt, (size_t)kCntWords));
  L.ftype = kf->ftype;
  kf->mc.bad_ref = L.cnt + kMcBadRef;
  kf->mc.beyond = L.cnt + kMcBeyond;

  auto setup_stage = [&](Stage& S, bool chroma) -> int {
    memset(&S, 0, sizeof(S));
    daala_b200_pvq_params& p = S.prm;
    const size_t ncoef = chroma ? luma_shard_px / 2 + 1024 : luma_shard_px + 1024;
    const size_t nblk = chroma ? L.max_chroma : L.max_luma;
    p.blocks = chroma ? L.chroma : L.luma;
    KF_CHECK(dalloc(kf, &p.in, ncoef));
    KF_CHECK(dalloc(kf, &p.ref, ncoef));
    KF_CHECK(dalloc(kf, &p.out, ncoef));
    KF_CHECK(dalloc(kf, &p.y, ncoef));
    KF_CHECK(dalloc(kf, &p.y16, ncoef));
    KF_CHECK(dalloc(kf, &p.res_skip_term, nblk * 9));
    KF_CHECK(dalloc(kf, &p.res_skip_diff, nblk));
    KF_CHECK(dalloc(kf, &p.res_flip, nblk));
    KF_CHECK(dalloc(kf, &S.res_pack, nblk * 9 * 4));
    p.res_gain = p.res_theta = p.res_max_theta = p.res_k = nullptr;
    p.res_dc = nullptr;
    if (inter) KF_CHECK(dalloc(kf, &p.res_dc, nblk));
    p.qm = kf->qm;
    p.qm_inv = kf->qm_inv;
    for (int i = 0; i < 3; i++) {
      p.coef_plane[i] = kf->coeffs[i];
      p.pred_plane[i] = kf->pred_coeffs[i];
      p.plane_frame_pitch[i] = (long long)kf->plane_w[i] * kf->plane_h[i];
      p.plane_stride[i] = kf->plane_w[i];
    }
    p.qm_stride = kf->cfg.qm_stride;
    p.is_keyframe = inter ? 0 : 1;
    p.use_masking = kf->cfg.use_masking;
    p.pvq_norm_lambda = kf->cfg.pvq_norm_lambda;
    S.fq_bq = kf->fq_bq;
    for (int c = 0; c < 3; c++) S.items[c] = chroma ? L.items_c[c] : L.items_l[c];
    S.cnt = L.cnt;
    S.rsqrt_tbl = kf->rsqrt_tbl;
    for (int c = 0; c < 3; c++) {
      S.sp_vec[c] = kf->sp_vec[c];
      S.sp_lanes[c] = kf->sp_lanes[c];
      S.sp_uni[c] = kf->sp_uni[c];
      S.sp_snap[c] = kf->sp_snap[c];
      S.sp_slots[c] = kf->sp_slots[c];
      const size_t cap = chroma ? cap_c[c] : cap_l[c];
      S.sp_chunks[c] = kf->sp_slots[c] > 0 ? (int)((cap + kf->sp_slots[c] - 1) / kf->sp_slots[c]) : 0;
    }
    S.max_waiters = kf->sms * 8;
    S.n_items_at = chroma ? kNItemsC : kNItemsL;
    S.n_blocks_at = chroma ? kNChroma : kNLuma;
    S.max_blocks = (int)nblk;
#ifdef DAALA_B200_CHAIN_TRACE
    if (!chroma && !inter) {
      S.trace_cap = (int)(luma_shard_px / 16);
      KF_CHECK(dalloc(kf, &S.trace, (size_t)S.trace_cap));
    }
#endif
    if (!chroma) {
      S.head_lo_at = kHeadLoL;
      S.dep_top = L.dep_top;
      S.dep_left = L.dep_left;
      S.succ_bottom = L.succ_bottom;
      S.succ_right = L.succ_right;
      S.heads = L.heads;
      S.heads0 = L.heads0;
      KF_CHECK(dalloc(kf, &S.ring, chains ? kf->chain_cap : 0));
      KF_CHECK(dalloc(kf, &S.join0, ndep));
    }
    return 0;
  };
  int rc = setup_stage(kf->luma, false);
  if (rc) return rc;
  rc = setup_stage(kf->chroma, true);
  if (rc) return rc;
  kf->luma.ftype = kf->chroma.ftype = kf->ftype;
  if (!inter || mixed) {
    Stage& C = kf->chroma;
    C.cfl_in = kf->luma.prm.in;
    C.cfl_out = kf->luma.prm.out;
    C.cfl_loff = L.unit_loff;
  }
  if (kf->cfg.haar_dc_quant) {
    daala_b200_haar_dc_batch& H = kf->hdcb;
    memset(&H, 0, sizeof(H));
    const size_t g0 = (size_t)(kf->plane_w[0] >> 2) * (kf->plane_h[0] >> 2), g1 = (size_t)(kf->plane_w[1] >> 2) * (kf->plane_h[1] >> 2);
    KF_CHECK(dalloc(kf, &kf->hdc, (g0 + 2 * g1) * F));
    H.grid_frame_pitch = (long long)(g0 + 2 * g1);
    kf->luma.cfl_in = kf->chroma.cfl_in = kf->hdc;
    for (int p = 0; p < 3; p++) {
      KF_CHECK(dalloc(kf, &kf->hdc_index[p], (p ? g1 : g0) * F));
      H.coeffs[p] = kf->coeffs[p];
      H.dc[p] = kf->hdc + (p ? g0 + (p - 1) * g1 : 0);
      H.index[p] = kf->hdc_index[p];
      H.plane_w[p] = kf->plane_w[p];
      H.plane_h[p] = kf->plane_h[p];
    }
    H.bsize = kf->bsize;
    H.F = F;
    H.nhsb = kf->nhsb;
    H.nvsb = kf->nvsb;
    H.pvq_norm_lambda = kf->cfg.pvq_norm_lambda;
    H.fq_bq = kf->fq_bq;
    H.frame_type = kf->ftype;
  }
  if (mixed) {
    Stage& K = kf->luma_kf;
    K = kf->luma;
    K.prm.is_keyframe = 1;
    K.cnt = L.kcnt;
    for (int c = 0; c < 3; c++) K.items[c] = L.kitems_l[c];
    K.ftype = nullptr;
  }
  (void)luma_px;
  if (kf->cfg.inter_finish || kf->cfg.symbol_stream == 2)
    for (int c = 0; c < 2; c++) {
      Stage& S = c ? kf->chroma : kf->luma;
      KF_CHECK(dalloc(kf, &kf->dc_resid[c], (size_t)S.max_blocks));
      S.dc_resid = kf->dc_resid[c];
    }
  if (kf->cfg.symbol_stream) {
    Sym& Y = kf->sym;
    memset(&Y, 0, sizeof(Y));
    Y.bsize = kf->bsize;
    Y.bstride = UW;
    Y.bsize_pitch = (long long)UW * UH;
    Y.F = F;
    Y.nhsb = kf->nhsb;
    Y.sb_rows = kf->cfg.sb_rows;
    Y.u_row0 = L.u_row0;
    Y.nsb = kf->nhsb * kf->cfg.sb_rows;
    Y.cap_blocks = L.max_luma + L.max_chroma;
    Y.ntiles = (Y.cap_blocks + kTile - 1) / kTile;
    const size_t ncoef = (luma_shard_px + 1024) + (luma_shard_px / 2 + 1024);
    KF_CHECK(dalloc(kf, &Y.unit_rank, (size_t)F * L.u_rows * UW));
    KF_CHECK(dalloc(kf, &Y.sb_cnt, (size_t)F * Y.nsb));
    KF_CHECK(dalloc(kf, &Y.sb_base, (size_t)F * Y.nsb));
    KF_CHECK(dalloc(kf, &Y.order, (size_t)Y.cap_blocks));
    KF_CHECK(dalloc(kf, &Y.off, (size_t)Y.cap_blocks));
    KF_CHECK(dalloc(kf, &Y.tile, (size_t)Y.ntiles));
    KF_CHECK(dalloc(kf, &Y.tot, (size_t)4));
    KF_CHECK(dalloc(kf, &Y.index, (size_t)F));
    KF_CHECK(dalloc(kf, &Y.blocks, (size_t)Y.cap_blocks));
    Y.cap_bands = (long long)(ncoef / 16);
    Y.cap_bytes = (long long)(2 * ncoef);
    KF_CHECK(dalloc(kf, &Y.bands, ncoef / 16));
    KF_CHECK(dalloc(kf, &Y.pulses, 2 * ncoef));
    for (int c = 0; c < 2; c++) {
      const Stage& S = c ? kf->chroma : kf->luma;
      Y.list[c] = S.prm.blocks;
      Y.res[c] = reinterpret_cast<const short4*>(S.res_pack);
      Y.y[c] = S.prm.y;
      Y.skip_diff[c] = S.prm.res_skip_diff;
    }
    Y.flip = kf->chroma.prm.res_flip;
    Y.cnt = L.cnt;
    Y.max_luma = L.max_luma;
    Y.max_chroma = L.max_chroma;
    if (kf->cfg.symbol_stream == 2) {
      KF_CHECK(dalloc(kf, &Y.dc, (size_t)Y.cap_blocks));
      for (int c = 0; c < 2; c++) {
        Y.qdc[c] = (c ? kf->chroma : kf->luma).prm.res_dc;
        Y.dc_resid[c] = kf->dc_resid[c];
      }
    }
    if (kf->cfg.haar_dc_quant) {
      KF_CHECK(dalloc(kf, &Y.hdc, (size_t)Y.cap_blocks));
      for (int p = 0; p < 3; p++) {
        Y.hdc_index[p] = kf->hdc_index[p];
        Y.gw[p] = kf->plane_w[p] >> 2;
        Y.gh[p] = kf->plane_h[p] >> 2;
      }
    }
  }
  if (kf->cfg.late_skip) {
    daala_b200_late_skip_batch& B = kf->lsb;
    memset(&B, 0, sizeof(B));
    long long px = 0;
    for (int p = 0; p < 3; p++) {
      const size_t n = (size_t)kf->plane_w[p] * kf->plane_h[p] * F;
      KF_CHECK(dalloc(kf, &kf->d_orig[p], n));
      px += (long long)n;
      B.d_orig[p] = kf->d_orig[p];
      B.d[p] = kf->coeffs[p];
      B.md[p] = kf->pred_coeffs[p];
      B.plane_pitch[p] = (long long)kf->plane_w[p] * kf->plane_h[p];
      B.plane_stride[p] = kf->plane_w[p];
    }
    for (int c = 0; c < 2; c++) {
      const Stage& S = c ? kf->chroma : kf->luma;
      KF_CHECK(dalloc(kf, &kf->late_skip[c], (size_t)S.max_blocks));
      B.blocks[c] = S.prm.blocks;
      B.count[c] = L.cnt + S.n_blocks_at;
      B.max_blocks[c] = S.max_blocks;
      B.out[c] = kf->late_skip[c];
    }
    KF_CHECK(dalloc(kf, &B.cls_items, (size_t)daala_b200_late_skip_class_caps(px, B.cls_off, B.cls_cap)));
    KF_CHECK(dalloc(kf, &B.cls_n, (size_t)4));
    B.qm_is_flat = kf->cfg.qm_is_flat;
    B.use_activity_masking = kf->cfg.use_masking;
    B.fq = kf->fq;
    B.fq_bq = kf->fq_bq;
    if (kf->cfg.symbol_stream == 2) {
      Sym& Y = kf->sym;
      KF_CHECK(dalloc(kf, &Y.late_skip, (size_t)Y.cap_blocks));
      Y.ls_block[0] = kf->late_skip[0];
      Y.ls_block[1] = kf->late_skip[1];
    }
  }

  daala_b200_frame& f = kf->frame;
  memset(&f, 0, sizeof(f));
  for (int p = 0; p < 3; p++) {
    daala_b200_plane& pl = f.plane[p];
    pl.pixels = kf->pixels[p];
    pl.coeffs = kf->coeffs[p];
    pl.lapped = kf->lapped[p];
    pl.pixels_out = kf->pixels_out[p];
    pl.pixel_stride = pl.coeff_stride = pl.lapped_stride = pl.pixel_out_stride = kf->plane_w[p];
    pl.xdec = p ? 1 : 0;
    pl.pixel_frame_pitch = pl.coeff_frame_pitch = pl.lapped_frame_pitch = pl.pixel_out_frame_pitch =
        (long long)kf->plane_w[p] * kf->plane_h[p];
  }
  f.bsize = kf->bsize;
  f.bstride = UW;
  f.bsize_frame_pitch = (long long)UW * UH;
  f.nhsb = kf->nhsb;
  f.nvsb = kf->nvsb;
  f.pic_w = kf->cfg.pic_w;
  f.pic_h = kf->cfg.pic_h;
  f.haar_dc = inter || kf->cfg.haar_dc_quant ? 0 : 1;
  f.nframes = F;
  f.sb_row0 = kf->cfg.sb_row0;
  f.sb_rows = kf->cfg.sb_rows;
  kf->frame_pred = f;
  kf->frame_fwd = f;
  kf->frame_fwd.haar_dc = inter ? 0 : 1;
  for (int p = 0; p < 3; p++) {
    kf->frame_pred.plane[p].pixels = kf->pred_pixels[p];
    kf->frame_pred.plane[p].coeffs = kf->pred_coeffs[p];
  }
  if (kf->cfg.inter_finish) {
    const size_t nsb = (size_t)F * kf->nhsb * kf->nvsb;
    Fin& P = kf->fin;
    memset(&P, 0, sizeof(P));
    for (int c = 0; c < 2; c++) {
      const Stage& S = c ? kf->chroma : kf->luma;
      KF_CHECK(dalloc(kf, &kf->fin_skip[c], (size_t)S.max_blocks));
      KF_CHECK(dalloc(kf, &kf->fin_dc[c], (size_t)S.max_blocks));
      P.blocks[c] = S.prm.blocks;
      P.skip[c] = kf->fin_skip[c];
      P.dc[c] = kf->fin_dc[c];
      P.max_blocks[c] = S.max_blocks;
    }
    P.cnt = L.cnt;
    P.skip_stride = kf->nhsb * 16;
    for (int p = 0; p < 3; p++) {
      const size_t n = (size_t)kf->plane_w[p] * kf->plane_h[p] * F;
      KF_CHECK(dalloc(kf, &kf->fin_coeffs[p], n));
      KF_CHECK(dalloc(kf, &kf->fin_pixels[p], n));
      P.skip_pitch[p] = (long long)(kf->plane_h[p] / 4) * P.skip_stride;
      KF_CHECK(dalloc(kf, &kf->fin_bskip[p], (size_t)P.skip_pitch[p] * F));
      P.d[p] = kf->coeffs[p];
      P.md[p] = kf->pred_coeffs[p];
      P.out[p] = kf->fin_coeffs[p];
      P.plane_pitch[p] = (long long)kf->plane_w[p] * kf->plane_h[p];
      P.plane_stride[p] = kf->plane_w[p];
      P.bskip[p] = kf->fin_bskip[p];
    }
    KF_CHECK(dalloc(kf, &kf->fin_level, nsb));
    KF_CHECK(dalloc(kf, &kf->fin_coded, nsb));
    P.coded = kf->fin_coded;
    P.nhsb = kf->nhsb;
    P.nvsb = kf->nvsb;
    P.fq_bq = kf->fq_bq;
    P.ftype = kf->ftype;
    if (kf->cfg.inter_mc) {
      KF_CHECK(dalloc(kf, &kf->fin_slot_out, (size_t)F));
      PoolStore& W = kf->store;
      for (int p = 0; p < 3; p++) {
        W.src[p] = kf->fin_pixels[p];
        W.pool[p] = kf->ref_pixels[p];
        W.plane_bytes[p] = (long long)kf->plane_w[p] * kf->plane_h[p];
      }
      W.slot = kf->fin_slot_out;
    }
    if (kf->cfg.symbol_stream == 2) {
      Unstream& U = kf->unstream;
      KF_CHECK(dalloc(kf, &kf->fin_stream_skip, (size_t)kf->sym.cap_blocks));
      KF_CHECK(dalloc(kf, &kf->fin_stream_dc, (size_t)kf->sym.cap_blocks));
      KF_CHECK(dalloc(kf, &kf->fin_form, (size_t)1));
      U.order = kf->sym.order;
      U.tot = kf->sym.tot;
      U.skip = kf->fin_stream_skip;
      U.dc = kf->fin_stream_dc;
      for (int c = 0; c < 2; c++) {
        U.fin_skip[c] = kf->fin_skip[c];
        U.fin_dc[c] = kf->fin_dc[c];
      }
      U.form = kf->fin_form;
    }
  }
  const int dering = kf->cfg.dering ? kf->cfg.dering : kf->cfg.inter_finish;
  if (dering) {
    const size_t nsb = (size_t)F * kf->nhsb * kf->nvsb;
    Dering& D = kf->dering;
    D.frame = kf->frame;
    D.skip_stride = kf->nhsb * 16;
    uint8_t* zero_skip = nullptr;
    if (!kf->cfg.inter_finish) KF_CHECK(dalloc(kf, &zero_skip, nsb * 256 + 64));
    for (int p = 0; p < 3; p++) {
      KF_CHECK(dalloc(kf, &D.frame.post16[p], (size_t)kf->plane_w[p] * kf->plane_h[p] * F));
      if (kf->cfg.inter_finish) {
        D.frame.plane[p].coeffs = D.frame.plane[p].lapped = kf->fin_coeffs[p];
        D.frame.plane[p].pixels_out = kf->fin_pixels[p];
        D.skip[p] = kf->fin_bskip[p];
        D.skip_pitch[p] = kf->fin.skip_pitch[p];
      } else {
        D.skip[p] = zero_skip;
      }
    }
    KF_CHECK(dalloc(kf, &D.level, nsb));
    KF_CHECK(dalloc(kf, &D.thr[0], nsb));
    KF_CHECK(dalloc(kf, &D.thr[1], nsb));
    KF_CHECK(dalloc(kf, &D.dir, nsb * 64));
    D.coded = kf->fin_coded;
    D.applied = kf->fin_level;
    D.frame_tbl = kf->fq_tbl;
    D.search = dering == 2;
    if (D.search) {
      daala_b200_dering_search_batch& b = D.sb;
      b.etmp = D.frame.post16[0];
      b.src = kf->pixels[0];
      b.etmp_pitch = b.src_pitch = (long long)kf->plane_w[0] * kf->plane_h[0];
      b.etmp_stride = b.src_stride = kf->plane_w[0];
      b.nframes = F;
      b.nhsb = kf->nhsb;
      b.nvsb = kf->nvsb;
      b.qm_is_flat = kf->cfg.qm_is_flat;
      b.use_activity_masking = kf->cfg.use_masking;
      b.bskip = D.skip[0];
      b.skip_stride = D.skip_stride;
      b.skip_pitch = D.skip_pitch[0];
      b.coded = D.coded;
      b.is_keyframe = inter ? 0 : 1;
      b.frame_type = kf->ftype;
      KF_CHECK(dalloc(kf, &b.filt, (size_t)kf->plane_w[0] * kf->plane_h[0] * F));
      KF_CHECK(dalloc(kf, &b.orig, nsb * 4096));
      KF_CHECK(dalloc(kf, &b.cand, nsb * 4096));
      KF_CHECK(dalloc(kf, &b.dist, nsb * 6));
      b.dir = D.dir;
      b.levels = D.level;
      b.fq = kf->fq;
      b.frame_tbl = kf->fq_tbl;
      KF_CHECK(dalloc(kf, &b.cand_thr, nsb * 5));
    }
  }
  KF_CHECK(cudaDeviceSynchronize());
  k_fill_rsqrt<<<(kTableDoubles + 255) / 256, 256, 0, kf->stream>>>(kf->rsqrt_tbl);
  KF_CHECK(cudaGetLastError());
  std::vector<daala_b200_kf_frame_quant> rec((size_t)F);
  for (daala_b200_kf_frame_quant& r : rec) {
    r.q0 = kf->cfg.q0;
    r.coded_quantizer = kf->cfg.coded_quantizer;
    r.dering_lambda = kf->cfg.dering_lambda;
    memcpy(r.pvq_qm_q4, kf->cfg.pvq_qm_q4, sizeof(r.pvq_qm_q4));
  }
  fq_derive_host(kf, rec.data(), false, &kf->fin_dc_limit);
  KF_CHECK(fq_copy(kf, rec.data(), kf->stream));
  KF_CHECK(cudaStreamSynchronize(kf->stream));
  return 0;
}

static int enqueue_recon(const daala_b200_frame& frame, int p0, int n, cudaStream_t s) {
  const int rc = daala_b200_launch_inverse_lapped_only(&frame, p0, n, s);
  return rc ? rc : daala_b200_launch_sb_postfilter_store(&frame, p0, n, s);
}

static int enqueue_dering_plane(daala_b200_kf* kf, const Dering& D, int p, cudaStream_t s) {
  const int nsb = kf->nhsb * kf->nvsb;
  const long long per = (long long)kf->plane_w[p] * kf->plane_h[p];
  daala_b200_dering_params dp;
  memset(&dp, 0, sizeof(dp));
  dp.y = nullptr;
  dp.x = D.frame.post16[p];
  dp.dir = D.dir;
  dp.bskip = D.skip[p];
  dp.sb_threshold = D.thr[p ? 1 : 0];
  dp.ystride = dp.xstride = kf->plane_w[p];
  dp.dir_stride = kf->nhsb * 8;
  dp.skip_stride = D.skip_stride;
  dp.nhsb = kf->nhsb;
  dp.nvsb = kf->nvsb;
  dp.xdec = p ? 1 : 0;
  dp.pli = p;
  dp.overlap = 1;
  dp.coeff_shift = 4;
  dp.dir_format = D.search ? 2 : 0;
  return daala_b200_dering_plane_frames(&dp, kf->F, per, per, (long long)nsb * 64, nsb, D.skip_pitch[p],
                                        D.frame.plane[p].pixels_out, s);
}

static int enqueue_dering_luma(daala_b200_kf* kf, const Dering& D, cudaStream_t s) {
  if (D.search) {
    const int rc = daala_b200_dering_search_enqueue(&D.sb, s);
    if (rc) return rc;
  }
  const int nsb = kf->nhsb * kf->nvsb;
  k_dering_thresholds<<<(kf->F * nsb + 255) / 256, 256, 0, s>>>(D.level, D.thr[0], D.thr[1], kf->F * nsb, D.coded,
                                                                   D.applied, D.frame_tbl, nsb);
  return enqueue_dering_plane(kf, D, 0, s);
}

static int enqueue_dering(daala_b200_kf* kf, const Dering& D, cudaStream_t s) {
  int rc = enqueue_recon(D.frame, 0, 3, s);
  if (!rc) rc = enqueue_dering_luma(kf, D, s);
  for (int p = 1; !rc && p < 3; p++) rc = enqueue_dering_plane(kf, D, p, s);
  return rc;
}

static int dering_launches(const Dering& D, int parts) {
  return 2 * parts + (D.search ? 1 + 5 + 6 + 6 + 1 : 0) + 1 + 3;
}

static void enqueue_split(daala_b200_kf* kf, const Stage& S, cudaStream_t s) {
  const int grid = kf->sms * 16;
  for (int cls = 2; cls >= 0; cls--) {
    for (int chunk = 0; chunk < S.sp_chunks[cls]; chunk++) {
      if (cls == 2) {
        k_pvq_split<0, 2><<<grid, 128, 0, s>>>(S, cls, chunk);
        k_pvq_split<1, 2><<<grid, 128, 0, s>>>(S, cls, chunk);
        k_pvq_split<2, 2><<<grid, 128, 0, s>>>(S, cls, chunk);
      } else {
        k_pvq_split<0, 1><<<grid, 128, 0, s>>>(S, cls, chunk);
        k_pvq_split<1, 1><<<grid, 128, 0, s>>>(S, cls, chunk);
        k_pvq_split<2, 1><<<grid, 128, 0, s>>>(S, cls, chunk);
      }
    }
  }
}

template <bool kInter>
static void enqueue_sym(const Sym& Y, int wide, cudaStream_t s) {
  k_sym_rank<<<(Y.F * Y.nsb + 7) / 8, 256, 0, s>>>(Y);
  k_sym_sb_scan<<<1, 1024, 0, s>>>(Y);
  if (!kInter && Y.hdc) k_sym_hdc<<<(Y.F * Y.nsb * 3 + 7) / 8, 256, 0, s>>>(Y);
  k_sym_place<<<wide, 256, 0, s>>>(Y);
  k_sym_tile_sums<<<Y.ntiles, kTile, 0, s>>>(Y);
  k_sym_tile_scan<<<1, 1024, 0, s>>>(Y);
  k_sym_offsets<<<Y.ntiles, kTile, 0, s>>>(Y);
  k_sym_pack<kInter><<<wide, 256, 0, s>>>(Y);
  k_sym_index<<<1, 256, 0, s>>>(Y);
}

static int enqueue_mc(daala_b200_kf* kf, int phases, cudaStream_t s) {
  if (!kf->cfg.inter_mc) return 0;
  const int wide = kf->sms * 8;
  if (phases & DAALA_B200_KF_LISTS) {
    const cudaError_t e = cudaMemsetAsync(kf->lists.cnt + kMcBadRef, 0, 2 * sizeof(int32_t), s);
    if (e != cudaSuccess) return (int)e;
    const int rc = daala_b200_launch_mc_leaves(&kf->mc, wide, s);
    if (rc) return rc;
  }
  return phases & DAALA_B200_KF_FORWARD ? daala_b200_launch_mc_obmc(&kf->mc, wide, s) : 0;
}

#define STEP_TRY(x)           \
  do {                        \
    const int rc_ = (int)(x); \
    if (rc_) return rc_;      \
  } while (0)

static int enqueue_step(daala_b200_kf* kf, int phases) {
  const daala_b200_kf_config& cfg = kf->cfg;
  const bool key = !cfg.inter || cfg.frame_types, pb = cfg.inter != 0, mixed = cfg.frame_types != 0;
  const bool hdc = cfg.haar_dc_quant != 0, core = (phases & DAALA_B200_KF_SEARCH_ONLY) != 0;
  cudaStream_t s = kf->stream, c = phases == DAALA_B200_KF_ALL && kf->side ? kf->side : s;
  const Lists& L = kf->lists;
  const Stage& K = mixed ? kf->luma_kf : kf->luma;
  const uint8_t* ftype = mixed ? kf->ftype : nullptr;
  const int wide = kf->sms * 8;
  const int persist = kf->sms * (cfg.persist_ctas_per_sm > 0 ? cfg.persist_ctas_per_sm : kPersistCtas);
  auto record = [&](int e, cudaStream_t from) { return c == s ? cudaSuccess : cudaEventRecord(kf->ev[e], from); };
  auto wait = [&](int e, cudaStream_t to) { return c == s ? cudaSuccess : cudaStreamWaitEvent(to, kf->ev[e], 0); };
  auto join = [&](int e, cudaStream_t from, cudaStream_t to) {
    const cudaError_t r = record(e, from);
    return r != cudaSuccess ? r : wait(e, to);
  };

  STEP_TRY(join(kEvLists, s, c));
  STEP_TRY(enqueue_mc(kf, phases, c));
  if (phases & DAALA_B200_KF_FORWARD) {
    STEP_TRY(daala_b200_launch_forward_masked(&kf->frame_fwd, 3, ftype, nullptr, c));
    for (int p = 0; cfg.late_skip && p < 3; p++)
      STEP_TRY(cudaMemcpyAsync(kf->d_orig[p], kf->coeffs[p], sizeof(int32_t) * kf->plane_w[p] * kf->plane_h[p] * kf->F,
                               cudaMemcpyDeviceToDevice, c));
    if (pb) STEP_TRY(daala_b200_launch_forward_masked(&kf->frame_pred, 3, nullptr, ftype, c));
  }
  if (phases & DAALA_B200_KF_LISTS) {
    k_unit_tile_sums<<<L.ntiles, kTile, 0, s>>>(L);
    k_tile_scan<<<1, 1024, 0, s>>>(L);
    k_unit_emit<<<L.ntiles, kTile, 0, s>>>(L);
    if (key) {
      const size_t nl = (size_t)L.max_luma * sizeof(int32_t);
      STEP_TRY(cudaMemsetAsync(L.succ_bottom, 0xff, nl, s));
      STEP_TRY(cudaMemsetAsync(L.succ_right, 0xff, nl, s));
      STEP_TRY(cudaMemsetAsync(L.head_hist, 0, sizeof(int32_t) * kHeadBins, s));
      k_luma_deps<<<wide, 256, 0, s>>>(L);
    }
    if (pb) k_luma_items<<<wide, 256, 0, s>>>(L);
    k_chroma_items<<<wide, 256, 0, s>>>(L);
  }
  STEP_TRY(join(kEvForward, c, s));
  if (hdc && (phases & DAALA_B200_KF_FORWARD)) {
    STEP_TRY(daala_b200_launch_haar_dc(&kf->hdcb, c));
    STEP_TRY(record(kEvHaarDc, c));
  }

  if (phases & DAALA_B200_KF_PVQ_LUMA) {
    if (key) {
      STEP_TRY(cudaMemsetAsync(K.ring, 0xff, kf->chain_cap * sizeof(uint32_t), s));
      STEP_TRY(cudaMemsetAsync(K.join0, 0, (size_t)K.max_blocks * sizeof(int32_t), s));
      if (mixed) k_begin_pvq<<<1, 256, 0, s>>>(K.cnt, K.ring, persist * kPersistThreads / 32);
      else k_begin_pvq<<<1, 32, 0, s>>>(K.cnt);
    }
    if (!core && mixed) k_gather<kGatherLuma, false, true><<<wide, 256, 0, s>>>(kf->luma);
    else if (!core && pb) k_gather<kGatherInter><<<wide, 256, 0, s>>>(kf->luma);
    else if (!core) k_gather<kGatherLuma><<<wide, 256, 0, s>>>(kf->luma);
    if (pb) STEP_TRY(join(kEvLumaGather, s, c));
    if (key) k_pvq_persist<<<persist, kPersistThreads, 0, s>>>(K);
    if (pb) {
      enqueue_split(kf, kf->luma, c);
      STEP_TRY(record(kEvInterLuma, c));
    }
  }
  STEP_TRY(join(kEvLumaBands, s, c));
  if (phases & DAALA_B200_KF_PVQ_CHROMA) {
    if (!core && mixed) k_gather<kGatherChroma, true, true><<<wide, 256, 0, c>>>(kf->chroma);
    else if (!core && pb) k_gather<kGatherInter><<<wide, 256, 0, c>>>(kf->chroma);
    else if (!core && hdc) k_gather<kGatherChroma, true><<<wide, 256, 0, c>>>(kf->chroma);
    else if (!core) k_gather<kGatherChroma><<<wide, 256, 0, c>>>(kf->chroma);
    enqueue_split(kf, kf->chroma, c);
    if (!core && mixed) k_finish_scatter<false, true, true><<<wide, 256, 0, c>>>(kf->chroma);
    else if (!core && pb) k_finish_scatter<true><<<wide, 256, 0, c>>>(kf->chroma);
    else if (!core && hdc) k_finish_scatter<false, true><<<wide, 256, 0, c>>>(kf->chroma);
    else if (!core) k_finish_scatter<false><<<wide, 256, 0, c>>>(kf->chroma);
  }
  if (!core && (phases & DAALA_B200_KF_PVQ_LUMA)) {
    if (hdc) STEP_TRY(wait(kEvHaarDc, s));
    if (pb) STEP_TRY(wait(kEvInterLuma, s));
    const int grid = c != s ? kf->sms * 128 : wide;
    if (mixed) k_finish_scatter<false, true, true><<<grid, 256, 0, s>>>(kf->luma);
    else if (pb) k_finish_scatter<true><<<grid, 256, 0, s>>>(kf->luma);
    else if (hdc) k_finish_scatter<false, true><<<grid, 256, 0, s>>>(kf->luma);
    else k_finish_scatter<false><<<grid, 256, 0, s>>>(kf->luma);
  }
  if (!core && (phases & DAALA_B200_KF_PVQ_CHROMA) && (cfg.late_skip || cfg.symbol_stream)) {
    STEP_TRY(join(kEvLumaScatter, s, c));
    if (cfg.late_skip) STEP_TRY(daala_b200_late_skip_enqueue(&kf->lsb, kf->sms * 3, c));
    if (cfg.symbol_stream && pb) enqueue_sym<true>(kf->sym, wide, c);
    else if (cfg.symbol_stream) enqueue_sym<false>(kf->sym, wide, c);
  }

  if (phases & DAALA_B200_KF_INVERSE) {
    const daala_b200_frame& fr = cfg.dering ? kf->dering.frame : kf->frame;
    if (c != s) STEP_TRY(enqueue_recon(fr, 1, 2, c));
    STEP_TRY(enqueue_recon(fr, 0, c != s ? 1 : 3, s));
    if (cfg.dering) STEP_TRY(enqueue_dering_luma(kf, kf->dering, s));
    STEP_TRY(join(kEvChroma, c, s));
    for (int p = 1; cfg.dering && p < 3; p++) STEP_TRY(enqueue_dering_plane(kf, kf->dering, p, s));
  }
  return (int)cudaGetLastError();
}
#undef STEP_TRY

static int kf_enqueue_step_lossless(daala_b200_kf* kf, int phases) {
  if (phases != DAALA_B200_KF_ALL) {
    snprintf(kf->err, sizeof(kf->err), "a lossless step runs whole (DAALA_B200_KF_ALL)");
    return (int)cudaErrorInvalidValue;
  }
  const int rc = enqueue_mc(kf, phases, kf->stream);
  return rc ? rc : daala_b200_launch_lossless(&kf->ll, kf->stream);
}

static int kf_enqueue_finish(daala_b200_kf* kf) {
  cudaStream_t s = kf->stream;
  const int wide = kf->sms * 8;
  if (kf->fin_form) k_fin_unstream<<<wide, 256, 0, s>>>(kf->unstream);
  if (cudaMemsetAsync(kf->fin_coded, 0, (size_t)kf->F * kf->nhsb * kf->nvsb, s) != cudaSuccess)
    return (int)cudaGetLastError();
  k_fin_patch<<<wide, 256, 0, s>>>(kf->fin);
  k_fin_skip_map<<<wide, 256, 0, s>>>(kf->fin);
  const int rc = enqueue_dering(kf, kf->dering, s);
  if (rc) return rc;
  if (kf->fin_slot_out) k_fin_pool_store<<<dim3(wide > kf->F ? wide / kf->F : 1, 3 * kf->F), 256, 0, s>>>(kf->store);
  return (int)cudaGetLastError();
}

extern "C" {

static thread_local char g_create_err[256] = "null engine";

daala_b200_kf* daala_b200_kf_create(const daala_b200_kf_config* cfg) {
  snprintf(g_create_err, sizeof(g_create_err), "daala_b200_kf_create: invalid configuration");
  if (cfg && cfg->frame_types) {
    const char* why = cfg->frame_types != 1 ? "frame_types is 0 or 1"
                      : cfg->inter != 1 || cfg->frame_quant != 1 || cfg->haar_dc_quant != 1 ||
                                (cfg->inter_finish != 1 && cfg->inter_finish != 2)
                          ? "frame_types = 1 requires inter = 1, frame_quant = 1, haar_dc_quant = 1 and inter_finish 1 or 2"
                      : cfg->symbol_stream ? "frame_types is not defined with symbol_stream (keyframes and P frames have "
                                             "streams of different formats)"
                      : cfg->late_skip ? "frame_types is not defined with late_skip"
                      : cfg->lossless ? "frame_types is not defined with lossless"
                      : cfg->dering ? "frame_types is not defined with dering (keyframes are deringed in the finishing pass)"
                      : cfg->sb_rows > 0 ? "frame_types is not defined with a row shard (sb_rows > 0)" : nullptr;
    if (why) {
      snprintf(g_create_err, sizeof(g_create_err), "daala_b200_kf_create: %s", why);
      return nullptr;
    }
  }
  if (cfg && cfg->inter_mc && (cfg->inter_mc != 1 || cfg->inter != 1)) {
    snprintf(g_create_err, sizeof(g_create_err), "daala_b200_kf_create: inter_mc is 0 or 1, and 1 requires inter = 1");
    return nullptr;
  }
  if (cfg && cfg->mc_next && (cfg->mc_next != 1 || cfg->inter_mc != 1)) {
    snprintf(g_create_err, sizeof(g_create_err), "daala_b200_kf_create: mc_next is 0 or 1, and 1 requires inter_mc = 1");
    return nullptr;
  }
  if (cfg && cfg->inter_finish && (cfg->inter_finish < 0 || cfg->inter_finish > 2 || cfg->inter != 1)) {
    snprintf(g_create_err, sizeof(g_create_err),
             "daala_b200_kf_create: inter_finish is 0, 1 or 2, and 1 and 2 require inter = 1");
    return nullptr;
  }
  if (cfg && (cfg->symbol_stream < 0 || cfg->symbol_stream > 2 || (cfg->symbol_stream == 2 && cfg->inter != 1))) {
    snprintf(g_create_err, sizeof(g_create_err),
             "daala_b200_kf_create: symbol_stream is 0, 1 or 2, and 2 requires inter = 1 (a keyframe's DC goes through "
             "the Haar pyramid and has no scalar index)");
    return nullptr;
  }
  if (cfg && cfg->late_skip && (cfg->late_skip != 1 || cfg->inter != 1)) {
    snprintf(g_create_err, sizeof(g_create_err),
             "daala_b200_kf_create: late_skip is 0 or 1, and 1 requires inter = 1 (keyframes have no late skip)");
    return nullptr;
  }
  if (cfg && cfg->frame_quant && (cfg->frame_quant != 1 || cfg->inter != 1)) {
    snprintf(g_create_err, sizeof(g_create_err),
             "daala_b200_kf_create: frame_quant is 0 or 1, and 1 requires inter = 1 (keyframes: keyframe_quant = 1)");
    return nullptr;
  }
  if (cfg && cfg->keyframe_quant) {
    const char* with = cfg->keyframe_quant != 1 ? "a value other than 0 or 1"
                       : cfg->inter ? "inter (P and B frames take their records with frame_quant = 1)"
                       : cfg->lossless ? "lossless (every frame is at quantizer 0)"
                       : cfg->sb_rows > 0 ? "a row shard (sb_rows > 0)" : nullptr;
    if (with) {
      snprintf(g_create_err, sizeof(g_create_err), "daala_b200_kf_create: keyframe_quant is not defined with %s", with);
      return nullptr;
    }
  }
  if (cfg && cfg->lossless) {
    const char* with = cfg->lossless != 1 ? "a value other than 0 or 1"
                       : cfg->dering ? "dering (lossless frames skip deringing)"
                       : cfg->symbol_stream ? "symbol_stream (the stream is the PVQ symbols)"
                       : cfg->late_skip ? "late_skip"
                       : cfg->inter_finish ? "inter_finish"
                       : cfg->frame_quant ? "frame_quant (every frame is at quantizer 0)"
                       : cfg->sb_rows > 0 ? "a row shard (sb_rows > 0)" : nullptr;
    if (with) {
      snprintf(g_create_err, sizeof(g_create_err), "daala_b200_kf_create: lossless is not defined with %s", with);
      return nullptr;
    }
  }
  if (cfg && cfg->haar_dc_quant) {
    const char* with = cfg->haar_dc_quant != 1 ? "a value other than 0 or 1"
                       : cfg->inter && !cfg->frame_types ? "inter (P and B frames code a scalar DC per block)"
                       : cfg->lossless ? "lossless (its keyframe DCs are coded exactly)"
                       : cfg->sb_rows > 0 ? "a row shard (sb_rows > 0)" : nullptr;
    if (with) {
      snprintf(g_create_err, sizeof(g_create_err), "daala_b200_kf_create: haar_dc_quant is not defined with %s", with);
      return nullptr;
    }
  }
  if (cfg && !cfg->lossless && (cfg->q0 < 1 || cfg->q0 > DAALA_B200_KF_MAX_Q0)) {
    snprintf(g_create_err, sizeof(g_create_err), "daala_b200_kf_create: q0 is outside [1, %d] (lossless = 1 codes quantizer 0)",
             DAALA_B200_KF_MAX_Q0);
    return nullptr;
  }
  if (cfg && cfg->mc_refs < 0) {
    snprintf(g_create_err, sizeof(g_create_err), "daala_b200_kf_create: mc_refs < 0");
    return nullptr;
  }
  if (cfg && cfg->inter) {
    const char* with = cfg->inter != 1 ? "a value other than 0 or 1"
                       : cfg->dering ? "dering (the all-zero skip map of the deringing stage is a keyframe property)"
                       : cfg->symbol_stream == 1 ? "symbol_stream = 1 (its block record has no DC field; "
                                                   "symbol_stream = 2 is the P-frame stream)"
                       : cfg->sb_rows > 0 ? "a row shard (sb_rows > 0)" : nullptr;
    if (with) {
      snprintf(g_create_err, sizeof(g_create_err), "daala_b200_kf_create: inter is not defined with %s", with);
      return nullptr;
    }
  }
  if (!cfg || cfg->pic_w <= 0 || cfg->pic_h <= 0 || cfg->nframes <= 0 || cfg->nframes > 255 || !cfg->qm ||
      !cfg->qm_inv || cfg->qm_stride <= 0)
    return nullptr;
  daala_b200_kf* kf = new (std::nothrow) daala_b200_kf();
  if (!kf) return nullptr;
  kf->cfg = *cfg;
  kf->nhsb = (cfg->pic_w + 63) / 64;
  kf->nvsb = (cfg->pic_h + 63) / 64;
  kf->F = cfg->nframes;
  if (kf->cfg.inter_mc && kf->cfg.mc_refs == 0) kf->cfg.mc_refs = (kf->cfg.mc_next ? 3 : 2) * kf->F;
  if (!kf->cfg.inter_mc) kf->cfg.mc_refs = 0;
  kf->slot_filled.assign((size_t)kf->cfg.mc_refs, 0);
  if (kf->cfg.sb_rows <= 0) {
    kf->cfg.sb_row0 = 0;
    kf->cfg.sb_rows = kf->nvsb;
  }
  for (int p = 0; p < 3; p++) {
    kf->plane_w[p] = (kf->nhsb * 64) >> (p ? 1 : 0);
    kf->plane_h[p] = (kf->nvsb * 64) >> (p ? 1 : 0);
  }
  if ((long long)kf->plane_w[0] * kf->plane_h[0] * kf->F >= (1ll << 31)) {
// ... 670 lines not shown
```

daala_b200/csrc/pvq_warp.cuh:

```cuda
#pragma once
#include <math.h>
#include <stdint.h>

#include "pvq_math.cuh"

namespace daala_b200 {
namespace pvq {

constexpr unsigned kFull = 0xffffffffu;
constexpr int kMaxEvents = 14;
constexpr int kRsqrtEntries = 1 << 16;
constexpr int kLogEntries = 1 << 12;
constexpr int kTableDoubles = kRsqrtEntries + kLogEntries;

#ifndef DAALA_B200_PVQ_EXACT_BOUND
#define DAALA_B200_PVQ_EXACT_BOUND 4503599627370496.
#endif
#ifdef DAALA_B200_EMU_STATS
#define PVQ_WARP_STAT(i) (daala_b200_pvq_warp_stats[i]++)
#else
#define PVQ_WARP_STAT(i) ((void)0)
#endif

__device__ __forceinline__ int wsum(int v) { return __reduce_add_sync(kFull, v); }
// ... 511 lines not shown
#pragma unroll
    for (int e = 0; e < 4; e++)
      if (e * 32 + lane == m) r16[e] = (int16_t)(r16[e] + shr_round(gr * s, rshift));
    householder_apply_warp(lane, big, xr, x16, r16, n);
#pragma unroll
    for (int e = 0; e < 4; e++) {
      if (e && !big) break;
      const int t1 = __shfl_sync(kFull, xr[e], (lane + 1) & 31);
      const int t2 = e + 1 < 4 ? __shfl_sync(kFull, xr[e + 1 < 4 ? e + 1 : e], 0) : 0;
      const int nxt = lane == 31 ? t2 : t1;
      if (e * 32 + lane >= m) xr[e] = nxt;
    }
  }

  c_gain = 0; c_theta = -1; c_ts = 0; c_k = 0; c_cosd = 0; c_qcg = 0; c_qtheta = 0;
  c_sinprod = 0; c_lambda = 0; c_rate_ts = 0;
  bool c_valid = false;
  {
    const bool wref = lane < 12;
    const bool nref = lane == 12 || lane == 13;
    int i = 0, j = -1;
    if (wref && have_ref) {
      const int gain_bound = (cg - gain_offset) >> kCgainShift;
      i = (gain_bound - 1 > 1 ? gain_bound - 1 : 1) + (lane >> 2);
      c_valid = i <= gain_bound + 1;
      c_qcg = shl(i, kCgainShift) + gain_offset;
    } else if (nref && ((is_keyframe && pli == 0) || corr < .5 || cg < (int32_t)shl(2, kCgainShift))) {
      const int gain_bound = cg >> kCgainShift;
      i = (gain_bound > 1 ? gain_bound : 1) + (lane - 12);
      c_valid = i <= gain_bound + 1;
      c_qcg = shl(i, kCgainShift);
    }
    if (!c_valid) c_qcg = kCgainOne;
    if (wref) {
      c_ts = compute_max_theta(c_qcg, beta);
      int lo = (int)floor(.5 + nl_div(theta * theta_scale_1 * 2, M_PI) * c_ts) - 2;
      int hi = (int)ceil(nl_div(theta * theta_scale_1 * 2, M_PI) * c_ts);
      if (lo < 0) lo = 0;
      if (hi > c_ts - 1) hi = c_ts - 1;
      j = lo + (lane & 3);
      c_valid = c_valid && j <= hi;
    } else {
      c_ts = 0;
    }
    const long long tk = nl_theta_k(c_qcg, j, c_ts, !wref, n, beta);
    c_qtheta = (int32_t)(tk >> 32);
    c_k = (int)(uint32_t)tk;
    c_gain = i;
    c_theta = wref ? j : -1;
    c_cosd = nl_cos(theta - c_qtheta);
    const int sin_q = nl_cos(32768 - c_qtheta), sin_t = nl_cos(32768 - theta);
    double dist = gain_weight * (c_qcg - cg) * (c_qcg - cg);
    double g2 = c_qcg * (double)cg;
    if (wref) {
      const double dist_theta = 2 - 2. * c_cosd * trig_1;
      dist = dist + c_qcg * (double)cg * dist_theta;
      const double sin_theta = sin_t * trig_1;
      c_sinprod = sin_theta * sin_q * trig_1;
      g2 = g2 * c_sinprod;
    }
    dist *= cgain_2;
    g2 = g2 * cgain_2;
    c_alive = c_valid && !(wref ? dist > dist0 + 1.0 * pvq_norm_lambda && c_k != 0 : dist > dist0 && c_k != 0);
    c_lambda = nl_div(pvq_norm_lambda, 1e-30 + g2);
    c_rate_ts = c_ts < kLogEntries ? rsq[kRsqrtEntries + (c_ts > 0 ? c_ts : 1)]
                                   : .9 * (M_LOG2E * nl_log((double)c_ts));
  }
}

template <int kMode>
__device__ __forceinline__ void band_search(int lane, BandCtx& B, int n, int16_t* snap, int snap_stride,
                                            const double* rsq) {
  const bool big = kMode == 0 ? n > 32 : kMode == 2;
  const int (&x16)[4] = B.x16; const int (&xr)[4] = B.xr;
  const int &c_k = B.c_k, &c_alive = B.c_alive;
  const double &c_lambda = B.c_lambda;
  int &c_ev = B.c_ev;
  double &e_xy = B.e_xy, &e_yy = B.e_yy, &e_xx = B.e_xx;
  int &e_sum = B.e_sum, &e_k = B.e_k, &e_zero = B.e_zero;
  unsigned alive_w = __ballot_sync(kFull, c_alive && lane < 12);
  unsigned alive_n = __ballot_sync(kFull, c_alive && lane >= 12);

  int ya[4];
#pragma unroll
  for (int e = 0; e < 4; e++) ya[e] = 0;
  SearchVec sv;
  sv.nn = n;
  sv.xx = 0;
  int prev_k = 0, nev = 0;
  c_ev = -1;
  int phase = 0;
  e_xy = 0; e_yy = 0; e_xx = 0; e_sum = 0; e_k = 0; e_zero = 0;
  while (alive_w | alive_n) {
    unsigned grp;
    int kcur, leader;
    const bool noref_ev = alive_w == 0;
    if (!noref_ev) {
      const int key = (alive_w >> lane) & 1 ? (c_k << 4) | lane : 0x7fffffff;
      const int mn = wmin(key);
      kcur = mn >> 4;
      leader = mn & 15;
      grp = __ballot_sync(kFull, ((alive_w >> lane) & 1) && c_k == kcur);
      alive_w &= ~grp;
    } else {
      leader = __ffs(alive_n) - 1;
      grp = 1u << leader;
      alive_n &= ~grp;
      kcur = __shfl_sync(kFull, c_k, leader);
    }
    const int want = noref_ev ? 2 : 1;
    if (phase != want) {
      phase = want;
      prev_k = 0;
      int src[4];
#pragma unroll
      for (int e = 0; e < 4; e++) src[e] = noref_ev ? x16[e] : xr[e];
      if (big) search_init<4>(lane, sv, src, noref_ev ? n : n - 1);
      else search_init<1>(lane, sv, src, noref_ev ? n : n - 1);
    }
    double xy = 0, yy = 0;
    const bool zero_ev = !noref_ev && kcur == 0;
    if (zero_ev) {
#pragma unroll
      for (int e = 0; e < 4; e++) ya[e] = 0;
    } else {
      const double lambda = wfetch(c_lambda, leader);
      const int i = search_start(lane, sv, ya, kcur, prev_k, big, &xy, &yy);
      if (big) search_event<4>(lane, sv, ya, kcur, i, xy, yy, lambda, rsq, &xy, &yy);
      else search_event<1>(lane, sv, ya, kcur, i, xy, yy, lambda, rsq, &xy, &yy);
    }
    prev_k = kcur;
    int sj = 0;
#pragma unroll
    for (int e = 0; e < 4; e++) {
      if (e && !big) break;
      const int j = e * 32 + lane;
      if (j < sv.nn) sj += j * ya[e];
      if (j < n) snap[nev * snap_stride + j] = (int16_t)(j < sv.nn ? ya[e] : 0);
    }
    sj = wsum(sj);
    if (lane == nev) {
      e_xy = xy;
      e_yy = yy;
      e_xx = sv.xx;
      e_sum = sj;
      e_k = kcur;
      e_zero = zero_ev;
    }
    if ((grp >> lane) & 1) c_ev = nev;
    nev++;
  }
}

template <int kMode>
__device__ __forceinline__ int band_finish(int lane, const BandCtx& B, const int16_t* snap, int snap_stride, int32_t* out,
                                           const int32_t* r0, int n, int q0, int32_t* yout, int* itheta,
                                           int* max_theta, int* vk, int beta, double* skip_term, int is_keyframe,
                                           int pli, const int16_t* qm_inv, double pvq_norm_lambda) {
  const double gain_weight = 1.4;
  const double cgain_1 = 1. / kCgainOne;
  const double cgain_2 = cgain_1 * cgain_1;
  const double trig_1 = 1. / 32768;
  const bool big = kMode == 0 ? n > 32 : kMode == 2;
  const int cfl_enabled = is_keyframe && pli != 0;
  const int (&x16)[4] = B.x16; const int (&r16)[4] = B.r16; const int (&xr)[4] = B.xr;
  const int32_t cg = B.cg;
  int32_t g = B.g, gain_offset = B.gain_offset;
  const int icgr = B.icgr, m = B.m, s = B.s;
  double best_dist = B.best_dist, best_cost = B.best_cost;
  const double skip_dist = B.skip_dist;
  const int c_gain = B.c_gain, c_theta = B.c_theta, c_ts = B.c_ts, c_k = B.c_k, c_cosd = B.c_cosd, c_ev = B.c_ev;
  const int32_t c_qcg = B.c_qcg, c_qtheta = B.c_qtheta;
  const double c_sinprod = B.c_sinprod, c_rate_ts = B.c_rate_ts;
  const double e_xy = B.e_xy, e_yy = B.e_yy, e_xx = B.e_xx;
  const int e_sum = B.e_sum, e_k = B.e_k, e_zero = B.e_zero;
  int32_t theta = 0;
  double e_cos = 0, e_rate = 0;
  {
    const int kk = e_k > 0 ? e_k : 1;
    const double cd = nl_div(e_xy, 1e-100 + nl_sqrt(e_xx * e_yy));
    const double f = nl_div((double)e_sum, (double)(kk * n));
    const double t = nl_div(nl_log(n * 2 * (1 * f + .025)) * kk, (double)n);
    const double rate = (1 + .4 * f) * n * (M_LOG2E * nl_log(1 + (0 > t ? 0 : t))) + 3;
    e_cos = e_zero ? 0. : cd;
    e_rate = e_k == 0 ? 0. : rate;
  }
  double c_dist = 0, cost = 0;
  {
    const int src = c_ev >= 0 ? c_ev : 0;
    const double cos_dist = wfetch(e_cos, src);
    double rate = wfetch(e_rate, src);
    double dist;
    if (lane >= 12) {
      dist = gain_weight * (c_qcg - cg) * (c_qcg - cg) + c_qcg * (double)cg * (2 - 2 * cos_dist);
    } else {
      if (c_gain > 0 && c_theta >= 0) {
        rate += c_rate_ts;
        if (is_keyframe && pli == 0) rate += 6;
        if (c_gain == icgr) rate -= .5;
      }
      const double dist_theta = 2 - 2. * c_cosd * trig_1 + c_sinprod * (2 - 2 * cos_dist);
      dist = gain_weight * (c_qcg - cg) * (c_qcg - cg) + c_qcg * (double)cg * dist_theta;
    }
    dist *= cgain_2;
    c_dist = dist;
    cost = dist + pvq_norm_lambda * rate;
  }
  int best_lane = -1;
  {
    unsigned rem = __ballot_sync(kFull, c_ev >= 0);
    while (rem) {
      const int key = (rem >> lane) & 1 ? (c_ev << 5) | lane : 0x7fffffff;
      const int l = wmin(key) & 31;
      rem &= ~(1u << l);
      const double cl = wfetch(cost, l);
      if (l >= 12 ? cl <= best_cost : cl < best_cost) {
        best_cost = cl;
        best_lane = l;
      }
    }
  }

  int qg = 0, best_k = 0;
  int noref = is_keyframe ? 1 : 0;
  *itheta = is_keyframe ? -1 : 0;
  *max_theta = 0;
  int ybest[4];
#pragma unroll
  for (int e = 0; e < 4; e++) ybest[e] = 0;
  if (best_lane >= 0) {
    qg = __shfl_sync(kFull, c_gain, best_lane);
    best_k = __shfl_sync(kFull, c_k, best_lane);
    *itheta = __shfl_sync(kFull, c_theta, best_lane);
    *max_theta = __shfl_sync(kFull, c_ts, best_lane);
    theta = __shfl_sync(kFull, c_qtheta, best_lane);
    best_dist = wfetch(c_dist, best_lane);
    noref = best_lane >= 12;
    const int ev = __shfl_sync(kFull, c_ev, best_lane);
#pragma unroll
    for (int e = 0; e < 4; e++) {
      if (e && !big) break;
      const int j = e * 32 + lane;
      const int v = noref ? x16[e] : xr[e];
      const int a = j < n ? snap[ev * snap_stride + j] : 0;
      ybest[e] = j < (noref ? n : n - 1) ? (v < 0 ? -a : a) : 0;
    }
  }
  int skip = 0;
  if (noref) {
    if (qg == 0) skip = 1;
  } else {
    if (!is_keyframe && qg == 0) skip = icgr ? 1 : 2;
    if (qg == icgr && *itheta == 0 && !cfl_enabled) skip = 2;
  }
  int32_t res[4];
  if (skip) {
#pragma unroll
    for (int e = 0; e < 4; e++) res[e] = (skip == 2 && r0 && e * 32 + lane < n) ? r0[e * 32 + lane] : 0;
  } else {
    if (noref) gain_offset = 0;
    g = gain_expand(shl(qg, kCgainShift) + gain_offset, q0, beta);
    const int nn = n - !noref;
    int syy = 0;
#pragma unroll
    for (int e = 0; e < 4; e++) if (e * 32 + lane < nn) syy += ybest[e] * ybest[e];
    const int yy = wsum(syy);
    int gshift = ilog((uint32_t)g) - 14;
    if (gshift < 0) gshift = 0;
    int32_t scale;
    if (yy == 0) {
      scale = 0;
    } else {
      int rsh;
      const int16_t rs = rsqrt32(yy, &rsh);
      scale = vshr_round64(rs * (int64_t)g, rsh + gshift - 16);
    }
    const int qshift = kQmInvShift - gshift;
    int xs[4];
    if (noref) {
#pragma unroll
      for (int e = 0; e < 4; e++) xs[e] = mul16_32_q16(ybest[e], scale);
    } else {
      scale = round32(scale * (1. / 32768) * nl_cos(32768 - theta));
      int f[4];
#pragma unroll
      for (int e = 0; e < 4; e++) f[e] = e * 32 + lane < nn ? (int16_t)mul16_32_q16(ybest[e], scale) : 0;
      const int xm = (int16_t)floor(.5 + -s * (shr_round(g, gshift)) * (1. / 32768) * nl_cos(theta));
#pragma unroll
      for (int e = 0; e < 4; e++) {
        xs[e] = 0;
        if (e && !big) continue;
        const int t1 = __shfl_sync(kFull, f[e], (lane + 31) & 31);
        const int t2 = e > 0 ? __shfl_sync(kFull, f[e > 0 ? e - 1 : 0], 31) : 0;
        const int fprev = lane == 0 ? t2 : t1;
        const int j = e * 32 + lane;
        xs[e] = j < m ? f[e] : (j == m ? xm : fprev);
        if (j >= n) xs[e] = 0;
      }
      householder_apply_warp(lane, big, xs, xs, r16, n);
    }
#pragma unroll
    for (int e = 0; e < 4; e++) {
      const int j = e * 32 + lane;
      res[e] = j < n ? shr_round(xs[e] * qm_inv[j], qshift) : 0;
    }
  }
#pragma unroll
  for (int e = 0; e < 4; e++) {
    const int j = e * 32 + lane;
    if (j < n) {
      out[j] = res[e];
      yout[j] = ybest[e];
    }
  }
  *vk = best_k;
  *skip_term = skip_dist - best_dist;
  if (is_keyframe) return noref ? qg : (qg < icgr ? -2 * (qg - icgr) - 1 : (qg < 2 * icgr ? 2 * (qg - icgr) : qg - 1));
  {
    const int a = qg + 1, b = icgr + 1;
    return noref ? qg - 1 : (a < b ? -2 * (a - b) - 1 : (a < 2 * b ? 2 * (a - b) : a - 1));
  }
}

template <int kMode = 0>
__device__ __forceinline__ int quantise_band_warp(int lane, int16_t* snap, const double* rsq, int32_t* out, const int32_t* x0,
                                                  const int32_t* r0, int n, int q0, int32_t* yout, int* itheta,
                                                  int* max_theta, int* vk, int beta, double* skip_term, int is_keyframe,
                                                  int pli, const int16_t* qm, const int16_t* qm_inv,
                                                  double pvq_norm_lambda) {
  int16_t* vec = snap + kMaxEvents * kMaxN;
  int32_t* lanes = reinterpret_cast<int32_t*>(vec + 3 * kMaxN);
  int32_t* uni = lanes + kCtxLaneWords * 16;
  {
    BandCtx B;
    band_setup<kMode>(lane, B, x0, r0, n, q0, beta, is_keyframe, pli, qm, pvq_norm_lambda, rsq);
    ctx_sync();
    band_ctx_store_setup(lane, B, n, vec, kMaxN, lanes, uni);
  }
  ctx_sync();
  {
    BandCtx B;
    band_ctx_load_search(lane, B, n, vec, kMaxN, lanes);
    band_search<kMode>(lane, B, n, snap, kMaxN, rsq);
    band_ctx_store_search(lane, B, lanes);
  }
  ctx_sync();
  BandCtx B;
  band_ctx_load_finish(lane, B, n, vec, kMaxN, lanes, uni);
  return band_finish<kMode>(lane, B, snap, kMaxN, out, r0, n, q0, yout, itheta, max_theta, vk, beta, skip_term, is_keyframe, pli,
                     qm_inv, pvq_norm_lambda);
}

}
}
```

Measured before the change: 2470.

## Fuse coefficient scatter into inverse transform and reschedule list/forward streams

Result: faster. 2514 (median of 6 runs) (+1.7%).

```diff
diff --git a/daala_b200/csrc/frame_transform.cu b/daala_b200/csrc/frame_transform.cu
--- a/daala_b200/csrc/frame_transform.cu
+++ b/daala_b200/csrc/frame_transform.cu
@@ -5,6 +5,7 @@
 #include <stdio.h>
 #include <string.h>
 
+#include "gen/coding_order.inc"
 #include "gen/dct_lifting.cuh"
 #include "lapped_filter.cuh"
 #include "frame_transform.h"
@@ -394,9 +395,113 @@
   else forward_sb_body<1, true>(prm, pl, tile_s, lists, map, raw, &bar, fm);
 }
 
+struct SbUnitOffsets {
+  int off[64];
+};
+
+template <int P>
+__device__ __forceinline__ int coded_at(int i) {
+  const unsigned short* t = i < 16 ? kScan4 : i < 64 ? kScan8 : i < 256 ? kScan16 : kScan32;
+  const int first = i < 16 ? 1 : i < 64 ? 16 : i < 256 ? 64 : 256;
+  const int sh = i < 16 ? 2 : i < 64 ? 3 : i < 256 ? 4 : 5;
+  const int v = i ? t[i - first] : 0;
+  return (v >> sh) * P + (v & ((1 << sh) - 1));
+}
+
+constexpr int kCodedUnroll = 4;
+
+__device__ __forceinline__ int coded_unit_offset(const FrameXformParams& prm, const InverseCoded& C, int pli, int fr,
+                                                 int sbx, int sby, int t) {
+  const int units_w = prm.nhsb * 8;
+  const long long upitch = (long long)units_w * prm.nvsb * 8;
+  const int32_t* unit = (pli ? C.coff : C.loff) + fr * upitch;
+  return unit[(long long)(sby * 8 + (t >> 3)) * units_w + sbx * 8 + (t & 7)];
+}
+
+template <int XDEC, int B, int P>
+__device__ __forceinline__ void tile_from_coded(const PlaneXform& pl, const InverseCoded& C, int pli, int fr, int sbx,
+                                                int sby, int* tile, const SbLists& lists, const SbUnitOffsets& uo,
+                                                int32_t* dst) {
+  constexpr int USH = 3 - XDEC;
+  const long long stride = pl.coeff_stride, frame_pitch = pl.coeff_frame_pitch;
+  const int32_t* out = C.out[pli];
+  const bool inter = C.pred[pli] && !(C.ftype && C.ftype[fr]);
+  const int32_t* pred = inter ? C.pred[pli] + fr * frame_pitch + (size_t)sby * B * stride + (size_t)sbx * B : nullptr;
+  const bool pred4 = inter && rows_aligned16(pred, stride);
+#pragma unroll 1
+  for (int c = 3; c < 5; c++) {
+    const int ln = c + 2;
+    const int items = lists.nblk[c] << (2 * ln - 2);
+    for (int item = threadIdx.x; item < items; item += kThreads) {
+      const int pos = lists.blk[blk_base(c) + (item >> (2 * ln - 2))];
+      const int r = (pos >> 8) + ((item >> (ln - 2)) & ((1 << ln) - 1));
+      const int col = (pos & 255) + 4 * (item & ((1 << (ln - 2)) - 1));
+      int4 v = make_int4(0, 0, 0, 0);
+      if (pred4) {
+        v = *reinterpret_cast<const int4*>(pred + (size_t)r * stride + col);
+      } else if (inter) {
+        const int32_t* q = pred + (size_t)r * stride + col;
+        v = make_int4(q[0], q[1], q[2], q[3]);
+      }
+      int* t = tile + r * P + col;
+      t[0] = v.x;
+      t[1] = v.y;
+      t[2] = v.z;
+      t[3] = v.w;
+    }
+  }
+  __syncthreads();
+#pragma unroll 1
+  for (int c = 0; c < 5; c++) {
+    const int lg = (c < 3 ? 2 * c + 4 : 9) - 2;
+    const int len = 4 << lg;
+    const int items = lists.nblk[c] << lg;
+    for (int base = threadIdx.x; base < items; base += kCodedUnroll * kThreads) {
+      int4 v[kCodedUnroll];
+#pragma unroll
+      for (int u = 0; u < kCodedUnroll; u++) {
+        const int item = base + u * kThreads;
+        v[u] = make_int4(0, 0, 0, 0);
+        if (item < items) {
+          const int pos = lists.blk[blk_base(c) + (item >> lg)];
+          const int x = pos & 255, y = pos >> 8;
+          int off = uo.off[(y >> USH) * 8 + (x >> USH)];
+          if (XDEC == 0 && c == 0) off += 16 * (((y >> 1) & 2) | ((x >> 2) & 1));
+          if (pli == 2) off += len;
+          if (off >= 0 && off + len <= C.cap[pli])
+            v[u] = *reinterpret_cast<const int4*>(out + off + 4 * (item & ((1 << lg) - 1)));
+        }
+      }
+#pragma unroll
+      for (int u = 0; u < kCodedUnroll; u++) {
+        const int item = base + u * kThreads;
+        if (item < items) {
+          const int pos = lists.blk[blk_base(c) + (item >> lg)], i = 4 * (item & ((1 << lg) - 1));
+          int* t = tile + (pos >> 8) * P + (pos & 255);
+          t[coded_at<P>(i)] = v[u].x;
+          t[coded_at<P>(i + 1)] = v[u].y;
+          t[coded_at<P>(i + 2)] = v[u].z;
+          t[coded_at<P>(i + 3)] = v[u].w;
+        }
+      }
+    }
+  }
+  __syncthreads();
+  if (rows_aligned16(dst, stride)) {
+    tile_copy4<B, P, true>(tile, dst, stride);
+  } else {
+    for (int i = threadIdx.x; i < B * B; i += kThreads) {
+      int r = i / B, c = i % B;
+      dst[(size_t)r * stride + c] = tile[r * P + c];
+    }
+  }
+  __syncthreads();
+}
+
 template <int XDEC>
-__device__ __forceinline__ void inverse_sb_body(const FrameXformParams& prm, const PlaneXform& pl,
-                                                int* tile, SbLists& lists) {
+__device__ __forceinline__ void inverse_sb_body(const FrameXformParams& prm, const PlaneXform& pl, int pli,
+                                                const InverseCoded& coded, int* tile, SbLists& lists,
+                                                SbUnitOffsets& uo) {
   constexpr int B = kMaxB >> XDEC;
   constexpr int P = kMaxPitch;
   using Sb = SbCtxT<B, P>;
@@ -405,17 +510,26 @@
   Sb s;
   s.x0 = sbx * B;
   s.y0 = sby * B;
-  const int32_t* srcp = pl.coeffs + fr * pl.coeff_frame_pitch + (size_t)s.y0 * pl.coeff_stride + s.x0;
-  if (rows_aligned16(srcp, pl.coeff_stride)) {
-    tile_copy4<B, P, false>(tile, const_cast<int32_t*>(srcp), pl.coeff_stride);
+  int32_t* srcp = pl.coeffs + fr * pl.coeff_frame_pitch + (size_t)s.y0 * pl.coeff_stride + s.x0;
+  if (coded.out[pli]) {
+    const int t = threadIdx.x;
+    const int u = t < 64 ? coded_unit_offset(prm, coded, pli, fr, sbx, sby, t) : 0;
+    build_lists<XDEC>(lists, prm.bsize + fr * prm.bsize_frame_pitch, prm.bstride, sbx, sby, s.x0, s.y0,
+                      prm.pic_w, prm.pic_h);
+    if (t < 64) uo.off[t] = u;
+    tile_from_coded<XDEC, B, P>(pl, coded, pli, fr, sbx, sby, tile, lists, uo, srcp);
   } else {
-    for (int i = threadIdx.x; i < B * B; i += kThreads) {
-      int r = i / B, c = i % B;
-      tile[r * P + c] = srcp[(size_t)r * pl.coeff_stride + c];
-    }
-  }
-  build_lists<XDEC>(lists, prm.bsize + fr * prm.bsize_frame_pitch, prm.bstride, sbx, sby, s.x0, s.y0,
-                    prm.pic_w, prm.pic_h);
+    if (rows_aligned16(srcp, pl.coeff_stride)) {
+      tile_copy4<B, P, false>(tile, srcp, pl.coeff_stride);
+    } else {
+      for (int i = threadIdx.x; i < B * B; i += kThreads) {
+        int r = i / B, c = i % B;
+        tile[r * P + c] = srcp[(size_t)r * pl.coeff_stride + c];
+      }
+    }
+    build_lists<XDEC>(lists, prm.bsize + fr * prm.bsize_frame_pitch, prm.bstride, sbx, sby, s.x0, s.y0,
+                      prm.pic_w, prm.pic_h);
+  }
   if (prm.haar_dc) {
 #pragma unroll 1
     for (int l = Sb::logB - 3; l >= 0; l--) {
@@ -445,12 +559,13 @@
 }
 
 __global__ void __launch_bounds__(kThreads, kCtasPerSm)
-k_inverse_sb(const __grid_constant__ FrameXformParams prm) {
+k_inverse_sb(const __grid_constant__ FrameXformParams prm, const __grid_constant__ InverseCoded coded, int plane0) {
   __shared__ int tile_s[kMaxB * kMaxPitch];
   __shared__ SbLists lists;
+  __shared__ SbUnitOffsets uo;
   const PlaneXform& pl = prm.plane[blockIdx.y];
-  if (pl.xdec == 0) inverse_sb_body<0>(prm, pl, tile_s, lists);
-  else inverse_sb_body<1>(prm, pl, tile_s, lists);
+  if (pl.xdec == 0) inverse_sb_body<0>(prm, pl, plane0 + blockIdx.y, coded, tile_s, lists, uo);
+  else inverse_sb_body<1>(prm, pl, plane0 + blockIdx.y, coded, tile_s, lists, uo);
 }
 
 template <int XDEC>
@@ -693,7 +808,7 @@
 
 int daala_b200_launch_inverse(const FrameXformParams* prm, int nplanes, cudaStream_t stream) {
   dim3 grid(prm->nhsb * prm->sb_rows, nplanes, prm->nframes);
-  k_inverse_sb<<<grid, kThreads, 0, stream>>>(*prm);
+  k_inverse_sb<<<grid, kThreads, 0, stream>>>(*prm, InverseCoded{}, 0);
   k_sb_postfilter_store<<<grid, kPostThreads, 0, stream>>>(*prm);
   return (int)cudaGetLastError();
 }
@@ -707,11 +822,16 @@
   return q;
 }
 
-int daala_b200_launch_inverse_lapped_only(const FrameXformParams* prm, int plane0, int nplanes, cudaStream_t stream) {
+int daala_b200_launch_inverse_lapped_coded(const FrameXformParams* prm, const InverseCoded* coded, int plane0,
+                                           int nplanes, cudaStream_t stream) {
   if (plane0 < 0 || nplanes < 1 || plane0 + nplanes > 3) return (int)cudaErrorInvalidValue;
   dim3 grid(prm->nhsb * prm->sb_rows, nplanes, prm->nframes);
-  k_inverse_sb<<<grid, kThreads, 0, stream>>>(plane_range(prm, plane0));
-  return (int)cudaGetLastError();
+  k_inverse_sb<<<grid, kThreads, 0, stream>>>(plane_range(prm, plane0), coded ? *coded : InverseCoded{}, plane0);
+  return (int)cudaGetLastError();
+}
+
+int daala_b200_launch_inverse_lapped_only(const FrameXformParams* prm, int plane0, int nplanes, cudaStream_t stream) {
+  return daala_b200_launch_inverse_lapped_coded(prm, nullptr, plane0, nplanes, stream);
 }
 
 int daala_b200_launch_sb_postfilter_store(const FrameXformParams* prm, int plane0, int nplanes, cudaStream_t stream) {
diff --git a/daala_b200/csrc/frame_transform.h b/daala_b200/csrc/frame_transform.h
--- a/daala_b200/csrc/frame_transform.h
+++ b/daala_b200/csrc/frame_transform.h
@@ -1,5 +1,20 @@
 #pragma once
+#include <cuda_runtime.h>
+#include <stdint.h>
+
 #include "daala_b200.h"
 
 typedef daala_b200_plane PlaneXform;
 typedef daala_b200_frame FrameXformParams;
+
+struct InverseCoded {
+  const int32_t* out[3];
+  long long cap[3];
+  const int32_t* loff;
+  const int32_t* coff;
+  const int32_t* pred[3];
+  const uint8_t* ftype;
+};
+
+extern "C" int daala_b200_launch_inverse_lapped_coded(const FrameXformParams* prm, const InverseCoded* coded, int plane0,
+                                                      int nplanes, cudaStream_t stream);
diff --git a/daala_b200/csrc/kf_engine.cu b/daala_b200/csrc/kf_engine.cu
--- a/daala_b200/csrc/kf_engine.cu
+++ b/daala_b200/csrc/kf_engine.cu
@@ -12,6 +12,7 @@
 
 #include "daala_b200.h"
 #include "dering_search.h"
+#include "frame_transform.h"
 #include "late_skip.h"
 #include "lossless.h"
 #include "haar_dc.h"
@@ -60,6 +61,7 @@
   int4* tile_sum;
   int32_t* unit_lbase;
   int32_t* unit_loff;
+  int32_t* unit_coff;
   daala_b200_pvq_block* luma;
   daala_b200_pvq_block* chroma;
   int32_t* dep_top;
@@ -74,6 +76,7 @@
   int32_t* head_bin;
   int32_t* head_hist;
   int32_t* head_cursor;
+  int n_deps;
   int32_t* cnt;
   int max_luma, max_chroma;
   const uint8_t* ftype;
@@ -106,6 +109,12 @@
 __global__ void __launch_bounds__(kTile) k_unit_tile_sums(const __grid_constant__ Lists L) {
   __shared__ int4 part[32];
   const long long i = (long long)blockIdx.x * kTile + threadIdx.x;
+  const long long nthr = (long long)gridDim.x * kTile;
+  for (long long k = i; k < L.n_deps; k += nthr) {
+    L.succ_bottom[k] = -1;
+    L.succ_right[k] = -1;
+  }
+  for (long long k = i; L.n_deps && k < kHeadBins; k += nthr) L.head_hist[k] = 0;
   int f, uy, ux, b;
   int4 v = make_int4(0, 0, 0, 0);
   if (unit_of(L, i, &f, &uy, &ux, &b)) v = unit_counts(b, ux, uy);
@@ -208,7 +217,8 @@
   L.unit_lbase[((long long)f * L.UH + uy) * L.UW + ux] = pre.x;
   if (v.x == 0) return;
   if (pre.x + v.x > L.max_luma || 2 * (pre.z + v.z) > L.max_chroma) return;
-  if (L.unit_loff) L.unit_loff[((long long)f * L.UH + uy) * L.UW + ux] = pre.y;
+  L.unit_loff[((long long)f * L.UH + uy) * L.UW + ux] = pre.y;
+  L.unit_coff[((long long)f * L.UH + uy) * L.UW + ux] = 2 * pre.w;
   if (b == 0) {
     for (int q = 0; q < 4; q++)
       put_block(L.luma + pre.x + q, pre.y + 16 * q, ux * 8 + (q & 1) * 4, uy * 8 + (q >> 1) * 4, 0, 0, 0, f);
@@ -672,7 +682,7 @@
   int itheta, max_theta, k;
   double skip_term;
   const int gain = quantise_band_warp<0>(lane, snap, S.rsqrt_tbl, prm.out + off, prm.in + off, prm.ref + off, bn, q,
-                                         prm.y + off, &itheta, &max_theta, &k, beta, &skip_term, prm.is_keyframe, pli,
+                                         prm.y16 + off, &itheta, &max_theta, &k, beta, &skip_term, prm.is_keyframe, pli,
                                          prm.qm + qoff, prm.qm_inv + qoff, prm.pvq_norm_lambda);
   if (lane == 0) {
     const size_t r = (size_t)blk * 9 + band;
@@ -735,7 +745,7 @@
       band_ctx_load_finish(lane, B, g.bn, vec, vs, lanes, uni);
       int itheta, max_theta, k;
       double skip_term;
-      const int gain = band_finish<kMode>(lane, B, snap, vs, prm.out + g.off, r0, g.bn, g.q, prm.y + g.off, &itheta, &max_theta, &k,
+      const int gain = band_finish<kMode>(lane, B, snap, vs, prm.out + g.off, r0, g.bn, g.q, prm.y16 + g.off, &itheta, &max_theta, &k,
                                    g.beta, &skip_term, g.is_keyframe, g.pli, prm.qm_inv + g.qoff, prm.pvq_norm_lambda);
       if (lane == 0) {
         const size_t r = (size_t)g.blk * 9 + g.band;
@@ -825,58 +835,38 @@
 }
 
 template <bool kInter, bool kHdc = false, bool kMixed = false>
-__global__ void __launch_bounds__(256) k_finish_scatter(const __grid_constant__ Stage S) {
+__global__ void __launch_bounds__(256) k_block_scalars(const __grid_constant__ Stage S) {
   const daala_b200_pvq_params& prm = S.prm;
   const int n = min(S.cnt[S.n_blocks_at], S.max_blocks);
-  const int lane = threadIdx.x & 31;
-  const int nwarps = (gridDim.x * blockDim.x) >> 5;
-  for (int blk = (blockIdx.x * blockDim.x + threadIdx.x) >> 5; blk < n; blk += nwarps) {
+  for (int blk = blockIdx.x * blockDim.x + threadIdx.x; blk < n; blk += gridDim.x * blockDim.x) {
     const daala_b200_pvq_block b = prm.blocks[blk];
     const bool key = kMixed && S.ftype[b.frame];
     const bool inter = kMixed ? !key : kInter, hdc = kMixed ? key : kHdc;
-    const int ln = b.bs + 2, nn = 1 << ln;
-    const int len = ln >= 5 ? 512 : 1 << (2 * ln);
-    const int stride = prm.plane_stride[b.pli];
-    int32_t* dst = prm.coef_plane[b.pli] + b.frame * prm.plane_frame_pitch[b.pli] + (size_t)b.y0 * stride + b.x0;
-    const int32_t* src = prm.out + b.coef_off;
-    if (lane == 0) {
-      const int nb = num_bands(b.bs);
-      double sd = 0;
-      for (int i = 0; i < nb; i++) sd += prm.res_skip_term[(size_t)blk * 9 + i];
-      prm.res_skip_diff[blk] = sd;
-      if (hdc) {
-        prm.out[b.coef_off] = dst[0] = hdc_grid(S, b.frame, b.pli)[(long long)(b.y0 >> 2) * (stride >> 2) + (b.x0 >> 2)];
-        if (kMixed) {
-          prm.res_dc[blk] = 0;
-          if (S.dc_resid) S.dc_resid[blk] = 0;
-        }
-      } else if (!inter) {
-        prm.out[b.coef_off] = prm.in[b.coef_off];
-      } else {
-        const int dc_quant = S.fq_bq[(b.frame * 3 + b.pli) * 32 + b.bs * (b.bs + 1)];
-        const int32_t r = prm.ref[b.coef_off], diff = prm.in[b.coef_off] - r;
-        int qdc = 0;
-        if (abs(diff) >= dc_quant * 141 / 256) {
-          const int half = ((dc_quant + 1) >> 1) - 1;
-          qdc = (diff + (diff < 0 ? -half : half)) / dc_quant;
-        }
-        prm.out[b.coef_off] = dst[0] = qdc * dc_quant + r;
-        prm.res_dc[blk] = qdc;
-        if (S.dc_resid) S.dc_resid[blk] = diff;
+    const int nb = num_bands(b.bs);
+    double sd = 0;
+    for (int i = 0; i < nb; i++) sd += prm.res_skip_term[(size_t)blk * 9 + i];
+    prm.res_skip_diff[blk] = sd;
+    prm.y16[b.coef_off] = 0;
+    if (hdc) {
+      prm.out[b.coef_off] = hdc_grid(S, b.frame, b.pli)[(long long)(b.y0 >> 2) * (prm.plane_stride[b.pli] >> 2) + (b.x0 >> 2)];
+      if (kMixed) {
+        prm.res_dc[blk] = 0;
+        if (S.dc_resid) S.dc_resid[blk] = 0;
       }
-    }
-    if (ln >= 5) {
-      const int32_t* mdp = inter ? prm.pred_plane[b.pli] + b.frame * prm.plane_frame_pitch[b.pli] + (size_t)b.y0 * stride + b.x0
-                                 : nullptr;
-      for (int i = lane; i < nn * nn; i += 32) {
-        const size_t at = (size_t)(i >> ln) * stride + (i & (nn - 1));
-        if (i) dst[at] = inter ? mdp[at] : 0;
+    } else if (!inter) {
+      prm.out[b.coef_off] = prm.in[b.coef_off];
+    } else {
+      const int dc_quant = S.fq_bq[(b.frame * 3 + b.pli) * 32 + b.bs * (b.bs + 1)];
+      const int32_t r = prm.ref[b.coef_off], diff = prm.in[b.coef_off] - r;
+      int qdc = 0;
+      if (abs(diff) >= dc_quant * 141 / 256) {
+        const int half = ((dc_quant + 1) >> 1) - 1;
+        qdc = (diff + (diff < 0 ? -half : half)) / dc_quant;
       }
-      __syncwarp();
-    }
-    for (int i = lane + 1; i < len; i += 32) dst[scan_to_raster(i, ln, stride)] = src[i];
-    const int32_t* y = prm.y + b.coef_off;
-    for (int i = lane; i < len; i += 32) prm.y16[b.coef_off + i] = i ? (int16_t)y[i] : (int16_t)0;
+      prm.out[b.coef_off] = qdc * dc_quant + r;
+      prm.res_dc[blk] = qdc;
+      if (S.dc_resid) S.dc_resid[blk] = diff;
+    }
   }
 }
 
@@ -1004,7 +994,7 @@
   uint8_t* pulses;
   const daala_b200_pvq_block* list[2];
   const short4* res[2];
-  const int32_t* y[2];
+  const int16_t* y[2];
   const double* skip_diff[2];
   const int32_t* flip;
   const int32_t* cnt;
@@ -1288,7 +1278,7 @@
       }
     }
     if (lane < nb) S.bands[o.x + lane] = r[lane];
-    const int32_t* y = S.y[ch] + b.coef_off;
+    const int16_t* y = S.y[ch] + b.coef_off;
     uint8_t* dst = S.pulses + o.y;
     for (int j = 0; j < nb; j++) {
       const short4 q = r[j];
@@ -1386,8 +1376,6 @@
 
 extern "C" int daala_b200_launch_forward_masked(const daala_b200_frame* prm, int nplanes, const uint8_t* haar_frames,
                                                 const uint8_t* skip_frames, cudaStream_t stream);
-extern "C" int daala_b200_launch_inverse_lapped_only(const daala_b200_frame* prm, int plane0, int nplanes,
-                                                     cudaStream_t stream);
 extern "C" int daala_b200_launch_sb_postfilter_store(const daala_b200_frame* prm, int plane0, int nplanes,
                                                      cudaStream_t stream);
 
@@ -1406,7 +1394,7 @@
   daala_b200_dering_search_batch sb;
 };
 
-enum { kEvLists, kEvForward, kEvLumaBands, kEvLumaScatter, kEvChroma, kEvHaarDc, kEvLumaGather, kEvInterLuma, kNumEvents };
+enum { kEvFork, kEvLists, kEvForward, kEvLumaBands, kEvLumaScalars, kEvChroma, kEvHaarDc, kEvLumaGather, kEvInterLuma, kNumEvents };
 
 struct daala_b200_kf {
   daala_b200_kf_config cfg;
@@ -1442,6 +1430,7 @@
   daala_b200_frame frame;
   daala_b200_frame frame_fwd;
   daala_b200_frame frame_pred;
+  InverseCoded coded;
   uint8_t* ref_pixels[3];
   int32_t* ref_slot;
   daala_b200_mv_pt* mv_grid;
@@ -1669,7 +1658,8 @@
   L.max_chroma = (int)(nunits * 2 / div) + 64;
   KF_CHECK(dalloc(kf, &L.tile_sum, (size_t)L.ntiles));
   KF_CHECK(dalloc(kf, &L.unit_lbase, (size_t)F * UW * UH));
-  if (!inter || mixed) KF_CHECK(dalloc(kf, &L.unit_loff, (size_t)F * UW * UH));
+  KF_CHECK(dalloc(kf, &L.unit_loff, (size_t)F * UW * UH));
+  KF_CHECK(dalloc(kf, &L.unit_coff, (size_t)F * UW * UH));
   KF_CHECK(dalloc(kf, &L.luma, (size_t)L.max_luma));
   KF_CHECK(dalloc(kf, &L.chroma, (size_t)L.max_chroma));
   const size_t ndep = inter && !mixed ? 0 : (size_t)L.max_luma;
@@ -1718,6 +1708,7 @@
   KF_CHECK(dalloc(kf, &L.head_bin, chains ? kf->chain_cap : 0));
   KF_CHECK(dalloc(kf, &L.head_hist, chains ? (size_t)kHeadBins : 0));
   KF_CHECK(dalloc(kf, &L.head_cursor, chains ? (size_t)kHeadBins : 0));
+  L.n_deps = chains ? L.max_luma : 0;
   KF_CHECK(dalloc(kf, &L.heads0, ndep));
   KF_CHECK(dalloc(kf, &L.cnt, (size_t)kCntWords));
   L.kcnt = L.cnt;
@@ -1726,16 +1717,16 @@
   kf->mc.bad_ref = L.cnt + kMcBadRef;
   kf->mc.beyond = L.cnt + kMcBeyond;
 
+  const size_t ncoef_luma = luma_shard_px + 1024, ncoef_chroma = luma_shard_px / 2 + 1024;
   auto setup_stage = [&](Stage& S, bool chroma) -> int {
     memset(&S, 0, sizeof(S));
     daala_b200_pvq_params& p = S.prm;
-    const size_t ncoef = chroma ? luma_shard_px / 2 + 1024 : luma_shard_px + 1024;
+    const size_t ncoef = chroma ? ncoef_chroma : ncoef_luma;
     const size_t nblk = chroma ? L.max_chroma : L.max_luma;
     p.blocks = chroma ? L.chroma : L.luma;
     KF_CHECK(dalloc(kf, &p.in, ncoef));
     KF_CHECK(dalloc(kf, &p.ref, ncoef));
     KF_CHECK(dalloc(kf, &p.out, ncoef));
-    KF_CHECK(dalloc(kf, &p.y, ncoef));
     KF_CHECK(dalloc(kf, &p.y16, ncoef));
     KF_CHECK(dalloc(kf, &p.res_skip_term, nblk * 9));
     KF_CHECK(dalloc(kf, &p.res_skip_diff, nblk));
@@ -1797,6 +1788,18 @@
   rc = setup_stage(kf->chroma, true);
   if (rc) return rc;
   kf->luma.ftype = kf->chroma.ftype = kf->ftype;
+  {
+    InverseCoded& I = kf->coded;
+    memset(&I, 0, sizeof(I));
+    for (int p = 0; p < 3; p++) {
+      I.out[p] = (p ? kf->chroma : kf->luma).prm.out;
+      I.cap[p] = (long long)(p ? ncoef_chroma : ncoef_luma);
+      I.pred[p] = kf->pred_coeffs[p];
+    }
+    I.loff = L.unit_loff;
+    I.coff = L.unit_coff;
+    I.ftype = kf->ftype;
+  }
   if (!inter || mixed) {
     Stage& C = kf->chroma;
     C.cfl_in = kf->luma.prm.in;
@@ -1872,7 +1875,7 @@
       const Stage& S = c ? kf->chroma : kf->luma;
       Y.list[c] = S.prm.blocks;
       Y.res[c] = reinterpret_cast<const short4*>(S.res_pack);
-      Y.y[c] = S.prm.y;
+      Y.y[c] = S.prm.y16;
       Y.skip_diff[c] = S.prm.res_skip_diff;
     }
     Y.flip = kf->chroma.prm.res_flip;
@@ -2094,8 +2097,8 @@
   return 0;
 }
 
-static int enqueue_recon(const daala_b200_frame& frame, int p0, int n, cudaStream_t s) {
-  const int rc = daala_b200_launch_inverse_lapped_only(&frame, p0, n, s);
+static int enqueue_recon(const daala_b200_frame& frame, const InverseCoded* coded, int p0, int n, cudaStream_t s) {
+  const int rc = daala_b200_launch_inverse_lapped_coded(&frame, coded, p0, n, s);
   return rc ? rc : daala_b200_launch_sb_postfilter_store(&frame, p0, n, s);
 }
 
@@ -2135,7 +2138,7 @@
 }
 
 static int enqueue_dering(daala_b200_kf* kf, const Dering& D, cudaStream_t s) {
-  int rc = enqueue_recon(D.frame, 0, 3, s);
+  int rc = enqueue_recon(D.frame, nullptr, 0, 3, s);
   if (!rc) rc = enqueue_dering_luma(kf, D, s);
   for (int p = 1; !rc && p < 3; p++) rc = enqueue_dering_plane(kf, D, p, s);
   return rc;
@@ -2210,31 +2213,26 @@
     return r != cudaSuccess ? r : wait(e, to);
   };
 
-  STEP_TRY(join(kEvLists, s, c));
-  STEP_TRY(enqueue_mc(kf, phases, c));
+  STEP_TRY(join(kEvFork, s, c));
+  STEP_TRY(enqueue_mc(kf, phases, s));
   if (phases & DAALA_B200_KF_FORWARD) {
-    STEP_TRY(daala_b200_launch_forward_masked(&kf->frame_fwd, 3, ftype, nullptr, c));
+    STEP_TRY(daala_b200_launch_forward_masked(&kf->frame_fwd, 3, ftype, nullptr, s));
     for (int p = 0; cfg.late_skip && p < 3; p++)
       STEP_TRY(cudaMemcpyAsync(kf->d_orig[p], kf->coeffs[p], sizeof(int32_t) * kf->plane_w[p] * kf->plane_h[p] * kf->F,
-                               cudaMemcpyDeviceToDevice, c));
-    if (pb) STEP_TRY(daala_b200_launch_forward_masked(&kf->frame_pred, 3, nullptr, ftype, c));
+                               cudaMemcpyDeviceToDevice, s));
+    if (pb) STEP_TRY(daala_b200_launch_forward_masked(&kf->frame_pred, 3, nullptr, ftype, s));
   }
   if (phases & DAALA_B200_KF_LISTS) {
-    k_unit_tile_sums<<<L.ntiles, kTile, 0, s>>>(L);
-    k_tile_scan<<<1, 1024, 0, s>>>(L);
-    k_unit_emit<<<L.ntiles, kTile, 0, s>>>(L);
-    if (key) {
-      const size_t nl = (size_t)L.max_luma * sizeof(int32_t);
-      STEP_TRY(cudaMemsetAsync(L.succ_bottom, 0xff, nl, s));
-      STEP_TRY(cudaMemsetAsync(L.succ_right, 0xff, nl, s));
-      STEP_TRY(cudaMemsetAsync(L.head_hist, 0, sizeof(int32_t) * kHeadBins, s));
-      k_luma_deps<<<wide, 256, 0, s>>>(L);
-    }
-    if (pb) k_luma_items<<<wide, 256, 0, s>>>(L);
-    k_chroma_items<<<wide, 256, 0, s>>>(L);
-  }
-  STEP_TRY(join(kEvForward, c, s));
+    k_unit_tile_sums<<<L.ntiles, kTile, 0, c>>>(L);
+    k_tile_scan<<<1, 1024, 0, c>>>(L);
+    k_unit_emit<<<L.ntiles, kTile, 0, c>>>(L);
+    if (key) k_luma_deps<<<wide, 256, 0, c>>>(L);
+    if (pb) k_luma_items<<<wide, 256, 0, c>>>(L);
+    k_chroma_items<<<wide, 256, 0, c>>>(L);
+  }
+  STEP_TRY(join(kEvLists, c, s));
   if (hdc && (phases & DAALA_B200_KF_FORWARD)) {
+    STEP_TRY(join(kEvForward, s, c));
     STEP_TRY(daala_b200_launch_haar_dc(&kf->hdcb, c));
     STEP_TRY(record(kEvHaarDc, c));
   }
@@ -2263,34 +2261,37 @@
     else if (!core && hdc) k_gather<kGatherChroma, true><<<wide, 256, 0, c>>>(kf->chroma);
     else if (!core) k_gather<kGatherChroma><<<wide, 256, 0, c>>>(kf->chroma);
     enqueue_split(kf, kf->chroma, c);
-    if (!core && mixed) k_finish_scatter<false, true, true><<<wide, 256, 0, c>>>(kf->chroma);
-    else if (!core && pb) k_finish_scatter<true><<<wide, 256, 0, c>>>(kf->chroma);
-    else if (!core && hdc) k_finish_scatter<false, true><<<wide, 256, 0, c>>>(kf->chroma);
-    else if (!core) k_finish_scatter<false><<<wide, 256, 0, c>>>(kf->chroma);
+    if (!core && mixed) k_block_scalars<false, true, true><<<wide, 256, 0, c>>>(kf->chroma);
+    else if (!core && pb) k_block_scalars<true><<<wide, 256, 0, c>>>(kf->chroma);
+    else if (!core && hdc) k_block_scalars<false, true><<<wide, 256, 0, c>>>(kf->chroma);
+    else if (!core) k_block_scalars<false><<<wide, 256, 0, c>>>(kf->chroma);
   }
   if (!core && (phases & DAALA_B200_KF_PVQ_LUMA)) {
     if (hdc) STEP_TRY(wait(kEvHaarDc, s));
     if (pb) STEP_TRY(wait(kEvInterLuma, s));
     const int grid = c != s ? kf->sms * 128 : wide;
-    if (mixed) k_finish_scatter<false, true, true><<<grid, 256, 0, s>>>(kf->luma);
-    else if (pb) k_finish_scatter<true><<<grid, 256, 0, s>>>(kf->luma);
-    else if (hdc) k_finish_scatter<false, true><<<grid, 256, 0, s>>>(kf->luma);
-    else k_finish_scatter<false><<<grid, 256, 0, s>>>(kf->luma);
-  }
-  if (!core && (phases & DAALA_B200_KF_PVQ_CHROMA) && (cfg.late_skip || cfg.symbol_stream)) {
-    STEP_TRY(join(kEvLumaScatter, s, c));
-    if (cfg.late_skip) STEP_TRY(daala_b200_late_skip_enqueue(&kf->lsb, kf->sms * 3, c));
-    if (cfg.symbol_stream && pb) enqueue_sym<true>(kf->sym, wide, c);
-    else if (cfg.symbol_stream) enqueue_sym<false>(kf->sym, wide, c);
+    if (mixed) k_block_scalars<false, true, true><<<grid, 256, 0, s>>>(kf->luma);
+    else if (pb) k_block_scalars<true><<<grid, 256, 0, s>>>(kf->luma);
+    else if (hdc) k_block_scalars<false, true><<<grid, 256, 0, s>>>(kf->luma);
+    else k_block_scalars<false><<<grid, 256, 0, s>>>(kf->luma);
+  }
+  if (!core && (phases & DAALA_B200_KF_PVQ_CHROMA) && cfg.symbol_stream && !cfg.late_skip) {
+    STEP_TRY(join(kEvLumaScalars, s, c));
+    if (pb) enqueue_sym<true>(kf->sym, wide, c);
+    else enqueue_sym<false>(kf->sym, wide, c);
   }
 
   if (phases & DAALA_B200_KF_INVERSE) {
     const daala_b200_frame& fr = cfg.dering ? kf->dering.frame : kf->frame;
-    if (c != s) STEP_TRY(enqueue_recon(fr, 1, 2, c));
-    STEP_TRY(enqueue_recon(fr, 0, c != s ? 1 : 3, s));
+    if (c != s) STEP_TRY(enqueue_recon(fr, &kf->coded, 1, 2, c));
+    STEP_TRY(enqueue_recon(fr, &kf->coded, 0, c != s ? 1 : 3, s));
     if (cfg.dering) STEP_TRY(enqueue_dering_luma(kf, kf->dering, s));
     STEP_TRY(join(kEvChroma, c, s));
     for (int p = 1; cfg.dering && p < 3; p++) STEP_TRY(enqueue_dering_plane(kf, kf->dering, p, s));
+    if (cfg.late_skip) {
+      STEP_TRY(daala_b200_late_skip_enqueue(&kf->lsb, kf->sms * 3, s));
+      if (cfg.symbol_stream) enqueue_sym<true>(kf->sym, wide, s);
+    }
   }
   return (int)cudaGetLastError();
 }
diff --git a/daala_b200/csrc/pvq_warp.cuh b/daala_b200/csrc/pvq_warp.cuh
--- a/daala_b200/csrc/pvq_warp.cuh
+++ b/daala_b200/csrc/pvq_warp.cuh
@@ -687,9 +687,9 @@
   }
 }
 
-template <int kMode>
+template <int kMode, typename YOut>
 __device__ __forceinline__ int band_finish(int lane, const BandCtx& B, const int16_t* snap, int snap_stride, int32_t* out,
-                                           const int32_t* r0, int n, int q0, int32_t* yout, int* itheta,
+                                           const int32_t* r0, int n, int q0, YOut* yout, int* itheta,
                                            int* max_theta, int* vk, int beta, double* skip_term, int is_keyframe,
                                            int pli, const int16_t* qm_inv, double pvq_norm_lambda) {
   const double gain_weight = 1.4;
@@ -845,7 +845,7 @@
     const int j = e * 32 + lane;
     if (j < n) {
       out[j] = res[e];
-      yout[j] = ybest[e];
+      yout[j] = (YOut)ybest[e];
     }
   }
   *vk = best_k;
@@ -857,9 +857,9 @@
   }
 }
 
-template <int kMode = 0>
+template <int kMode = 0, typename YOut>
 __device__ __forceinline__ int quantise_band_warp(int lane, int16_t* snap, const double* rsq, int32_t* out, const int32_t* x0,
-                                                  const int32_t* r0, int n, int q0, int32_t* yout, int* itheta,
+                                                  const int32_t* r0, int n, int q0, YOut* yout, int* itheta,
                                                   int* max_theta, int* vk, int beta, double* skip_term, int is_keyframe,
                                                   int pli, const int16_t* qm, const int16_t* qm_inv,
                                                   double pvq_norm_lambda) {
```
